# saidwivedi/InteractVLM

Hardware: AMD Instinct MI355X
Metric: images/sec end-to-end contact inference (higher is better)
Workload: dtype f16

## Files before the change

### include/ivlm_hip.h

```cpp
#ifndef IVLM_HIP_H
#define IVLM_HIP_H

#include <stddef.h>
#include <stdint.h>

#ifdef __cplusplus
extern "C" {
#endif

#define IVLM_OK 0
#define IVLM_ERR_INVALID_ARG (-1)
#define IVLM_ERR_WORKSPACE (-2)
#define IVLM_ERR_LAUNCH (-3)
#define IVLM_ERR_UNSUPPORTED (-4)

#define IVLM_F32 0
#define IVLM_BF16 1
#define IVLM_BF16_SPLIT 2
#define IVLM_F16 4
#define IVLM_F16_SPLIT 5
#define IVLM_FP8 3

#define IVLM_GEMM_A_F32 1
#define IVLM_GEMM_RES_F32 2
#define IVLM_GEMM_A_SPLIT 4
#define IVLM_GEMM_OUT_SPLIT 8
#define IVLM_GEMM_F16 16
#define IVLM_GEMM_OUT_F16 32

#define IVLM_GEMM_W_PANEL 64

typedef void *ivlm_stream_t;

int ivlm_abi_version(void);
const char *ivlm_error_string(int code);
const char *ivlm_build_arch(void);
const char *ivlm_last_hip_error(void);

int ivlm_profile_launches(void *start_event, void *stop_event);


size_t ivlm_lift_plan_workspace_bytes(int V, int64_t HW, int Nv);
int ivlm_lift_plan_build(const int32_t *vid, const float *bary, int V, int64_t HW, int Nv,
                         int32_t *row_ptr, int32_t *ent_pix, float *ent_w, int64_t cap, int32_t *nnz_out,
                         void *workspace, size_t workspace_bytes, ivlm_stream_t stream);
int ivlm_lift_points_plan_build(const int32_t *pid, int V, int64_t HW, int Np, int32_t *row_ptr, int32_t *ent_pix, float *ent_w,
                                int64_t cap, int32_t *nnz_out, void *workspace, size_t workspace_bytes, ivlm_stream_t stream);
int ivlm_lift_stream_blocks_per_cu(int bpc);

int ivlm_lift_mesh_plan(const float *logits, const int32_t *row_ptr, const int32_t *ent_pix,
                        const float *ent_w, int B, int V, int64_t HW, int Nv, int mode, float param,
                        float *out, float *nviews, ivlm_stream_t stream);

int ivlm_lift_mesh_plan_lowres(const void *low, int dtype, int lh, int lw, int img, int in_h, int in_w, int oh, int ow,
                               const int32_t *row_ptr, const int32_t *ent_pix, const float *ent_w, int B, int V,
                               int Nv, int mode, float param, float *out, float *nviews, ivlm_stream_t stream);

size_t ivlm_lift_mesh_dense_workspace_bytes(int B, int V, int Nv);
int ivlm_lift_mesh_dense(const float *logits, const int32_t *vid, const float *bary, int B, int V,
                         int64_t HW, int Nv, int mode, float param, float *out, float *nviews,
                         void *workspace, size_t workspace_bytes, ivlm_stream_t stream);

size_t ivlm_lift_points_workspace_bytes(int B, int V, int Np);
int ivlm_lift_points(const float *probs, const int32_t *pid, int pid_batched, int B, int V, int64_t HW,
                     int Np, float *out, float *nviews, void *workspace, size_t workspace_bytes,
                     ivlm_stream_t stream);

int ivlm_postprocess_masks(const void *low, int dtype, int n, int h, int w, int img, int in_h, int in_w,
                           int oh, int ow, int apply_sigmoid, float *out, ivlm_stream_t stream);
int ivlm_uncertainty_mlp(const float *embeddings, int64_t rows, const void *w1, const void *b1, const void *w2, const void *b2,
                         const void *w3, const void *b3, float *out, ivlm_stream_t stream);
int ivlm_resize_bilinear(const float *src, int n, int h, int w, void *dst, int dst_dtype, int oh, int ow, ivlm_stream_t stream);

int ivlm_postprocess_masks_valid(const void *low, int dtype, int n, int h, int w, int img, int in_h, int in_w, int oh, int ow,
                                 const float *gt, float ignore_label, float *out, ivlm_stream_t stream);


int ivlm_gemm_bf16(const void *A, int64_t lda, const void *W, int64_t ldw, void *C, int64_t ldc,
                   const void *bias, const void *residual, int64_t ldr, int res_mod, int M, int N, int K,
                   int act, int out_f32, int batch, int64_t strideA, int64_t strideW, int64_t strideC,
                   int64_t strideR, const void *rms_w, float rms_eps, int flags, const int32_t *out_rows,
                   const int32_t *a_rows, ivlm_stream_t stream);

int ivlm_gemm_bf16_panel(const void *A, int64_t lda, int64_t a_kstep, const void *W, int64_t ldw, int64_t w_kstep, void *C,
                         int64_t ldc, int64_t c_panel, const void *bias, const void *residual, int64_t ldr, int M, int N, int K,
                         int act, int out_f32, int flags, const int32_t *out_rows, const int32_t *a_rows, ivlm_stream_t stream);

int ivlm_gemm_fp8(const void *A, int64_t lda, const void *W, int64_t ldw, void *C, int64_t ldc, const void *bias,
                  const void *residual, int64_t ldr, int M, int N, int K, int act, int out_kind, const float *scale_a,
                  const float *scale_w, const float *scale_out, int flags, const int32_t *out_rows, const int32_t *a_rows,
                  ivlm_stream_t stream);

int ivlm_gemv_fp8w(const float *x, const void *Wq, int64_t ldw, const float *scale_w, void *C, const void *bias,
                   const void *residual, int N, int K, int act, int out_f32, const void *rms_w, float rms_eps, int flags,
                   ivlm_stream_t stream);

size_t ivlm_gemm_splitk_workspace_bytes(int M, int N, int splits);
int ivlm_gemm_bf16_splitk(const void *A, int64_t lda, const void *W, int64_t ldw, void *C, int64_t ldc,
                          const void *bias, const void *residual, int64_t ldr, int res_mod, int M, int N, int K,
                          int act, int out_f32, int splits, void *workspace, size_t workspace_bytes, int flags,
                          ivlm_stream_t stream);
#define IVLM_SPLITK_COUNTERS 4096
int ivlm_gemm_bf16_splitk_fused(const void *A, int64_t lda, const void *W, int64_t ldw, void *C, int64_t ldc,
                                const void *bias, const void *residual, int64_t ldr, int res_mod, int M, int N, int K,
                                int act, int out_f32, int splits, void *workspace, size_t workspace_bytes, int32_t *counters,
                                int flags, ivlm_stream_t stream);
int ivlm_gemv_tuning(int max_blocks_per_cu, int rows2_min_n);
void ivlm_gemv1_tuning(int ksplit);
void ivlm_gemv1_lds_floor(int bytes);
int ivlm_gemv_mfma_min_m(int min_m);
void ivlm_skinny_tuning(int tiles_per_block);

int ivlm_gemm_nsplit(int on);
int ivlm_gemm_tile_override(int tile);
int ivlm_gemm_tile320(int on);
int ivlm_gemm_route_query(int entry, int M, int N, int K, int64_t lda, int64_t ldw, int64_t ldc, int64_t ldr, int64_t a_kstep,
                          int64_t w_kstep, int64_t c_panel, int act, int out_kind, int has_bias, int has_residual, int res_mod,
                          int batch, int flags, int has_out_rows, int has_a_rows, int splits, int32_t *records, int max_records);

int ivlm_layernorm(const void *x, int x_dtype, const void *w, const void *b, void *y, int y_dtype, int64_t rows, int cols,
                   float eps, int gelu_after, const int32_t *out_rows, const float *fp8_scale, ivlm_stream_t stream);
int ivlm_rmsnorm(const void *x, int x_dtype, const void *w, void *y, int y_dtype, int64_t rows, int cols, float eps,
                 ivlm_stream_t stream);

int ivlm_rmsnorm_fp8(const void *x, int x_dtype, const void *w, void *y, int64_t rows, int cols, float eps, const float *fp8_scale,
                     ivlm_stream_t stream);

int ivlm_attention_bf16(const void *q, const void *k, const void *v, void *o, const int64_t *strides_host, int B,
                        int H, int Sq, int Sk, int D, float scale, int causal, int q_pos0, const float *rel_h,
                        const float *rel_w, int rel_kh, int rel_kw, int kv_batch_div, int prescale_q,
                        ivlm_stream_t stream);
int ivlm_attention_f16(const void *q, const void *k, const void *v, void *o, const int64_t *strides_host, int B,
                       int H, int Sq, int Sk, int D, float scale, int causal, int q_pos0, const float *rel_h,
                       const float *rel_w, int rel_kh, int rel_kw, int kv_batch_div, int prescale_q,
                       ivlm_stream_t stream);
int ivlm_attention_f16_qsplit(const void *q, const void *q_lo, const void *k, const void *v, void *o, const int64_t *strides_host,
                              int B, int H, int Sq, int Sk, int D, float scale, const float *rel_h, const float *rel_w, int rel_kh,
                              int rel_kw, int level, ivlm_stream_t stream);
int ivlm_attention_bf16_split(const void *q, const void *q_lo, const void *k, const void *k_lo, const void *v, const void *v_lo,
                              void *o, void *o_lo, const int64_t *strides_host, int B, int H, int Sq, int Sk, int D, float scale,
                              int causal, int q_pos0, const float *rel_h, const float *rel_w, int rel_kh, int rel_kw,
                              int kv_batch_div, int prescale_q, ivlm_stream_t stream);
int ivlm_attention_f32(const float *q, const float *k, const float *v, float *o, const int64_t *strides_host, int B, int H,
                       int Sq, int Sk, int D, float scale, int kv_batch_div, ivlm_stream_t stream);
int ivlm_attention_pingpong(int mode);
int ivlm_attention_xcd_map(int on);
int ivlm_attention_window_kernel(int v2);

int ivlm_relpos_bias(const void *q, int64_t q_bs, int64_t q_hs, int64_t q_rs, const void *tab_h, const void *tab_w,
                     int B, int H, int SH, int SW, int D, float *rel_h, float *rel_w, ivlm_stream_t stream);
int ivlm_relpos_bias_split(const void *q, const void *q_lo, int64_t q_bs, int64_t q_hs, int64_t q_rs, const void *tab_h,
                           const void *tab_w, int B, int H, int SH, int SW, int D, float *rel_h, float *rel_w,
                           ivlm_stream_t stream);
int ivlm_relpos_gather(const void *G, int64_t g_head_stride, int npad, int B, int H, int SH, int SW, float *rel_h,
                       float *rel_w, ivlm_stream_t stream);
int ivlm_relpos_gather_f32(const void *G, int64_t g_head_stride, int npad, int B, int H, int SH, int SW, float *rel_h,
                           float *rel_w, ivlm_stream_t stream);

int ivlm_relpos_bias_f16(const void *q, const void *q_lo, int64_t q_bs, int64_t q_hs, int64_t q_rs, const void *cat16, int npad, int B,
                         int H, int SH, int SW, int D, float *G_ws, size_t g_bytes, float *rel_h, float *rel_w, ivlm_stream_t stream);

int ivlm_llama_decode_attn(const void *qkv, int io_dtype, void *kcache, void *vcache, int tmax, void *o, int H, int D, int pos,
                           const int32_t *pos_dev, float theta, float scale, const float *cos_tab, const float *sin_tab,
                           ivlm_stream_t stream);
int ivlm_llama_decode_attn_f16(const void *qkv, void *kcache, void *vcache, int tmax, void *o, int H, int D, int pos,
                               const int32_t *pos_dev, float theta, float scale, const float *cos_tab, const float *sin_tab,
                               ivlm_stream_t stream);
size_t ivlm_llama_decode_attn_splitkv_scratch_bytes(int H, int D);
int ivlm_llama_decode_attn_splitkv(const float *qkv, int cache_dtype, void *kcache, void *vcache, int tmax, float *o, int H, int D,
// ... 115 lines not shown
int ivlm_sam_encode_parity_f16mlp(const ivlm_sam_cfg *cfg, const ivlm_sam_head *head, const ivlm_sam_block *blocks_host,
                                  const ivlm_sam_mlp_f16 *mlp16_host, const void *images, int V, float *embeddings_out,
                                  void *workspace, size_t workspace_bytes, ivlm_stream_t stream);
typedef struct {
    const void *qkv_w16, *proj_w16, *lin1_w16, *lin2_w16, *qkv_b16, *rel_cat16;
} ivlm_sam_block_f16;
size_t ivlm_sam_encode_f16_workspace_bytes(const ivlm_sam_cfg *cfg, int V);
int ivlm_sam_encode_f16(const ivlm_sam_cfg *cfg, const ivlm_sam_head *head, const ivlm_sam_block *blocks_host,
                        const ivlm_sam_block_f16 *blocks16_host, const void *images, int V, float *embeddings_out, void *workspace,
                        size_t workspace_bytes, ivlm_stream_t stream);
int ivlm_bf16_to_f16(const void *src_bf16, void *dst_f16, int64_t n, ivlm_stream_t stream);

typedef struct {
    const void *w2, *b;
    int n, k;
} ivlm_lin;
typedef struct {
    ivlm_lin q, k, v, o;
} ivlm_dec_attn;
typedef struct {
    ivlm_dec_attn self_attn, t2i, i2t;
    const void *norm1_w, *norm1_b, *norm2_w, *norm2_b, *norm3_w, *norm3_b, *norm4_w, *norm4_b;
    ivlm_lin lin1, lin2;
} ivlm_dec_layer;
typedef struct {
    int C, heads, depth;
    const void *no_mask, *key_pe, *out_tokens;
    ivlm_dec_layer layers[4];
    ivlm_dec_attn final_attn;
    const void *norm_final_w, *norm_final_b, *up_ln_w, *up_ln_b;
    ivlm_lin up0, up1, hyper[3], iou[3];
} ivlm_sam_dec;
size_t ivlm_sam_decode_workspace_bytes(int V, int grid, int C, int n_text, int mlp_dim);
int ivlm_sam_decode(const ivlm_sam_dec *weights, int V, int grid, int n_text, const float *image_embeddings,
                    const float *text_embeds, float *low_res_out, float *iou_out, void *workspace, size_t workspace_bytes,
                    ivlm_stream_t stream);

int ivlm_gemm_splitk_choice(int M, int N, int K, int act, int has_rms);
int ivlm_stages_splitk_fused(int on);

int ivlm_gemv1_bf12(const float *x, const void *P, int64_t ldp, const void *E, int64_t lde, const int32_t *ebase,
                    const int32_t *patch_ptr, const int32_t *patch_col, const void *patch_val, void *C, const void *bias,
                    const void *residual, int N, int K, int act, int out_f32, const void *rms_w, float rms_eps, int flags,
                    ivlm_stream_t stream);
int ivlm_gemv1_bf12m(const float *x, const void *Pf, const void *Ef, const int32_t *ebase, const int32_t *patch_ptr,
                     const int32_t *patch_col, const void *patch_val, void *C, const void *bias, const void *residual, int N, int K,
                     int act, int out_f32, const void *rms_w, float rms_eps, int flags, ivlm_stream_t stream);
int ivlm_llama_decode_attn_parts(const float *qkv, int cache_dtype, void *kcache, void *vcache, int tmax, float *parts, int H, int D,
                                 int pos, const int32_t *pos_dev, float theta, float scale, const float *cos_tab, const float *sin_tab,
                                 ivlm_stream_t stream);
int ivlm_gemv1_bf12m_parts(const float *parts, int D, const void *Pf, const void *Ef, const int32_t *ebase, const int32_t *patch_ptr,
                           const int32_t *patch_col, const void *patch_val, void *C, const void *bias, const void *residual, int N, int K,
                           int act, int out_f32, int flags, ivlm_stream_t stream);
int ivlm_pack_bf12m_count(const void *w, int N_valid, int n_rows, int K, int32_t *ebase, int32_t *patch_ptr, ivlm_stream_t stream);
int ivlm_pack_bf12m_fill(const void *w, int N_valid, int n_rows, int K, const int32_t *ebase, const int32_t *patch_ptr, void *Pf, void *Ef,
                         int32_t *patch_col, void *patch_val, ivlm_stream_t stream);
int ivlm_gemv16_bf12m(const float *x, int64_t lda, int M, const void *Pf, const void *Ef, const int32_t *ebase,
                      const int32_t *patch_ptr, const int32_t *patch_col, const void *patch_val, void *C, int64_t ldc, const void *bias,
                      const void *residual, int64_t ldr, int N, int K, int act, int out_f32, const void *rms_w, float rms_eps, int flags,
                      ivlm_stream_t stream);
void ivlm_gemv16_bf12m_tuning(int tiles_per_block);
int ivlm_decode_parts_tuning(int ranges);
void ivlm_gemv1_bf12m_tuning(int wide_max_blocks);
int ivlm_gemv1_bf12m_staging(int form);
int ivlm_unpack_bf12(const void *P, int64_t ldp, const void *E, int64_t lde, const int32_t *ebase, const int32_t *patch_ptr,
                     const int32_t *patch_col, const void *patch_val, int N, int K, void *w_out, ivlm_stream_t stream);

int ivlm_argmax_f32(const float *x, int rows, int cols, int32_t *out, ivlm_stream_t stream);
int ivlm_argmax_f32_bump(const float *x, int rows, int cols, int32_t *out, int32_t *bump, ivlm_stream_t stream);

int ivlm_im2col_nchw(const void *x, void *out, int B, int C, int H, int W, int ks, int stride, int Kpad,
                     ivlm_stream_t stream);
int ivlm_im2col3x3_nhwc(const void *x, void *out, int B, int H, int W, int C, ivlm_stream_t stream);
int ivlm_im2col3x3_nhwc_strided(const void *x, int64_t ldx, void *out, int64_t ldo, int B, int H, int W, int C,
                                ivlm_stream_t stream);
int ivlm_gather_rows(void *dst, int dst_kind, int64_t ldd, const void *src, int src_dtype, int64_t lds, const int32_t *idx,
                     const void *add, int add_dtype, int64_t lda, int64_t rows, int cols, const float *fp8_scale,
                     ivlm_stream_t stream);
int ivlm_amax(const void *x, int dtype, int64_t n, float *out, ivlm_stream_t stream);
int ivlm_add_rows(void *out, int out_kind, const void *a, int a_dtype, const void *b, int b_dtype, int64_t rows, int cols,
                  int64_t b_rows, int op, ivlm_stream_t stream);
int ivlm_fill_rows(void *dst, int64_t ldd, const int32_t *idx, int64_t n_idx, const void *row, int cols,
                   ivlm_stream_t stream);
int ivlm_dense_pe(const void *gauss, void *pe, int pe_dtype, int h, int w, int F, ivlm_stream_t stream);
int ivlm_rope_kv(void *qkv, int64_t ld, int T, int H, int D, int pos0, float theta, void *kcache, void *vcache,
                 const float *cos_tab, const float *sin_tab, ivlm_stream_t stream);
int ivlm_rope_kv_f16(void *qkv, int64_t ld, int T, int H, int D, int pos0, float theta, void *kcache, void *vcache,
                     const float *cos_tab, const float *sin_tab, ivlm_stream_t stream);
int ivlm_rope_kv_split(void *qkv, int64_t ld, int T, int H, int D, int pos0, void *kcache, void *kcache_lo, void *vcache,
                       void *vcache_lo, const float *cos_tab, const float *sin_tab, ivlm_stream_t stream);
int ivlm_llama_attn_oproj(const float *qkv, void *kcache, void *vcache, int tmax, float *attn_scratch, const void *wo,
                          const float *x, float *x_out, int H, int D, float theta, float scale, const float *cos_tab,
                          const float *sin_tab, const int32_t *pos_dev, const int32_t *step_dev, int32_t *counter,
                          int32_t *status, ivlm_stream_t stream);
int ivlm_rope_table(float *cos_tab, float *sin_tab, int T, int D, float theta, ivlm_stream_t stream);
int ivlm_normalize_pad_u8(const uint8_t *src, int H, int W, int y0, int x0, int ch, int cw, const float *mean3_host,
                          const float *std3_host, void *out, int out_bf16, int OH, int OW, ivlm_stream_t stream);
int ivlm_mask_dot(const void *up, const void *hyper, int dtype, float *low, int B, int gh, int gw, int C,
                  ivlm_stream_t stream);
int ivlm_mask_dot_multi(const void *up, const void *hyper, int dtype, float *low, int B, int M, int gh, int gw, int C,
                        ivlm_stream_t stream);
int ivlm_prompt_embed(const float *coords, const int32_t *labels, const float *gauss, const float *table, float *out, int64_t R,
                      int F, int H, int W, ivlm_stream_t stream);
int ivlm_mask_downscale(const float *mask, const float *w0, const float *b0, const float *ln1_w, const float *ln1_b, const float *w3,
                        const float *b3, const float *ln2_w, const float *ln2_b, const float *w6, const float *b6, float *dense, int B,
                        int gh, int gw, int C, int mask_in_chans, float eps, ivlm_stream_t stream);

size_t ivlm_h_geo_workspace_bytes(int n);
int ivlm_h_geo_metric(const float *dist, const float *pred, const float *gt, int B, int n, float *out, void *workspace,
                      size_t workspace_bytes, ivlm_stream_t stream);
int ivlm_contact_prf(const float *gt, const float *pred, int B, int n, float thr, float *out, ivlm_stream_t stream);
int ivlm_spmv_csr(const int32_t *row_ptr, const int32_t *col, const float *val, const float *x, int B, int rows,
                  int cols, float *y, ivlm_stream_t stream);

int ivlm_contact_band_census(const float *p, int64_t ld, int B, int Nv, const float *thr, int J, float margin, int32_t *counts,
                             float *mindist, ivlm_stream_t stream);
size_t ivlm_mask_band_census_workspace_bytes(void);
int ivlm_mask_band_census(const float *logits, int V, int64_t HW, const int32_t *ent_pix, const int32_t *row_ptr, int n_rows,
                          float thr_p, float margin_p, int32_t *counts, void *workspace, size_t workspace_bytes,
                          ivlm_stream_t stream);

#define IVLM_SEG_GT_U8 0
#define IVLM_SEG_GT_I32 1
#define IVLM_SEG_GT_F32 2
size_t ivlm_seg_iou_workspace_bytes(int V);
int ivlm_seg_iou_counts(const float *pred, const void *gt, int gt_dtype, int V, int H, int W, int ignore_label, int32_t *out,
                        void *workspace, size_t workspace_bytes, ivlm_stream_t stream);
#define IVLM_AFFORD_MAX_N 4096
#define IVLM_AFFORD_MAX_T 64
int ivlm_afford_metrics(const float *gt, const float *pred, int B, int n, const float *thresholds, int T, float mae_div,
                        float *out, int32_t *valid, ivlm_stream_t stream);

#define IVLM_CONTACT_PAIR_CHAIN 512
size_t ivlm_contact_pair_workspace_bytes(int B, int N_o, int N_h);
int ivlm_contact_pair(const float *o, const float *h, const void *p, const void *q, int p_dtype, int B, int N_o, int N_h,
                      int64_t o_batch_stride, int64_t h_batch_stride, float *value_out, float *grad_o, float *grad_h,
                      void *workspace, size_t workspace_bytes, ivlm_stream_t stream);

#define IVLM_ICP_ESTIMATE_SCALE 1
#define IVLM_ICP_ALLOW_REFLECTION 2
#define IVLM_ICP_REQUERY 4
size_t ivlm_contact_icp_workspace_bytes(int B, int N_o);
int ivlm_contact_icp(const float *x, const float *y, const float *xn, const float *yn, const float *w, const float *init_R,
                     const float *init_T, const float *init_s, int B, int N_o, int N_h, int64_t x_batch_stride, int64_t y_batch_stride,
                     int64_t xn_batch_stride, int64_t yn_batch_stride, int64_t w_batch_stride, int max_iterations, float relative_rmse_thr,
                     int flags, float *R_out, float *T_out, float *s_out, float *rmse_out, int32_t *converged_out, int32_t *iterations_out,
                     int32_t *nn_idx_out, float *hist_R, float *hist_T, float *hist_s, void *workspace, size_t workspace_bytes,
                     ivlm_stream_t stream);

int ivlm_points_align(const float *X, const float *Y, const float *w, int B, int N, int64_t x_batch_stride, int64_t y_batch_stride,
                      int64_t w_batch_stride, int flags, float *R_out, float *T_out, float *s_out, void *workspace, size_t workspace_bytes,
                      ivlm_stream_t stream);

int ivlm_contact_nearest(const float *q, const float *t, int D, int B, int N_o, int N_h, int64_t q_batch_stride, int64_t t_batch_stride,
                         int32_t *idx_out, float *d2_out, ivlm_stream_t stream);

int ivlm_contact_normal_filter(const float *obj_normals, const float *human_normals, int N_o, int N_h, float c_pos, float c_neg,
                               int has_neg, uint8_t *keep_out, ivlm_stream_t stream);

#define IVLM_SILHOUETTE_CHAIN 32
#define IVLM_SILHOUETTE_POS_ULPS 12
#define IVLM_SILHOUETTE_REL_ULPS 6
#define IVLM_SILHOUETTE_EXP_ULPS 3
#define IVLM_SILHOUETTE_T_ULPS 8
size_t ivlm_soft_silhouette_workspace_bytes(int B, int N, int F, int H, int W);
int ivlm_soft_silhouette_forward(const float *verts, const int32_t *faces, int B, int N, int F, int H, int W, float fx, float fy,
// ... 140 lines not shown
```

### interactvlm_amd/csrc/elementwise.hip

```cpp
#include "kernels.h"

namespace ivlm {
namespace {

constexpr int kT = 256;

inline int grid_for(int64_t work_items, int max_blocks = 8192) {
    int64_t b = (work_items + kT - 1) / kT;
    if (b < 1) b = 1;
    return (int)(b < max_blocks ? b : max_blocks);
}

__global__ __launch_bounds__(kT) void im2col_nchw_kernel(const bf16_t* __restrict__ x, bf16_t* __restrict__ out, int B,
                                                         int C, int H, int W, int ks, int stride, int Kpad) {
    const int gh = (H - ks) / stride + 1, gw = (W - ks) / stride + 1;
    const int K = C * ks * ks;
    const int64_t total = (int64_t)B * gh * gw * (Kpad >> 3);
    for (int64_t i = (int64_t)blockIdx.x * kT + threadIdx.x; i < total; i += (int64_t)gridDim.x * kT) {
        const int c8 = (int)(i % (Kpad >> 3));
        const int64_t row = i / (Kpad >> 3);
        const int gx = (int)(row % gw), gy = (int)((row / gw) % gh), b = (int)(row / ((int64_t)gw * gh));
        bf16_t v[8];
#pragma unroll
        for (int e = 0; e < 8; ++e) {
// ... 38 lines not shown
        f[4] = __uint_as_float(u.z << 16); f[5] = __uint_as_float(u.z & 0xffff0000u);
        f[6] = __uint_as_float(u.w << 16); f[7] = __uint_as_float(u.w & 0xffff0000u);
    }
}
__device__ __forceinline__ uint2 pack_fp8x8(const float* f, float inv_scale) {
    float c[8];
#pragma unroll
    for (int j = 0; j < 8; ++j) c[j] = fminf(fmaxf(f[j] * inv_scale, -448.0f), 448.0f);
    uint32_t a = 0, b = 0;
    a = __builtin_amdgcn_cvt_pk_fp8_f32(c[0], c[1], a, false);
    a = __builtin_amdgcn_cvt_pk_fp8_f32(c[2], c[3], a, true);
    b = __builtin_amdgcn_cvt_pk_fp8_f32(c[4], c[5], b, false);
    b = __builtin_amdgcn_cvt_pk_fp8_f32(c[6], c[7], b, true);
    return make_uint2(a, b);
}

__device__ __forceinline__ void store8(void* base, int kind, int64_t elem, int cols, const float* f, float inv_scale = 1.0f) {
    if (kind == 3) {
        *reinterpret_cast<uint2*>(static_cast<uint8_t*>(base) + elem) = pack_fp8x8(f, inv_scale);
        return;
    }
    if (kind == 1) {
        float4* p = reinterpret_cast<float4*>(static_cast<float*>(base) + elem);
        p[0] = make_float4(f[0], f[1], f[2], f[3]);
        p[1] = make_float4(f[4], f[5], f[6], f[7]);
        return;
    }
    bf16_t* o = static_cast<bf16_t*>(base) + elem;
    *reinterpret_cast<uint4*>(o) = make_uint4(pack_bf16x2(f[0], f[1]), pack_bf16x2(f[2], f[3]), pack_bf16x2(f[4], f[5]),
                                              pack_bf16x2(f[6], f[7]));
    if (kind == 2) {
        float l[8];
#pragma unroll
        for (int j = 0; j < 8; ++j) l[j] = f[j] - bf16_to_f32(f32_to_bf16(f[j]));
        *reinterpret_cast<uint4*>(o + cols) = make_uint4(pack_bf16x2(l[0], l[1]), pack_bf16x2(l[2], l[3]),
                                                         pack_bf16x2(l[4], l[5]), pack_bf16x2(l[6], l[7]));
    }
}

__global__ __launch_bounds__(kT) void gather_rows_kernel(void* __restrict__ dst, int dst_kind, int64_t ldd,
                                                         const void* __restrict__ src, int src_kind, int64_t lds_,
                                                         const int32_t* __restrict__ idx, const void* __restrict__ add,
                                                         int add_kind, int64_t lda, int64_t rows, int cols,
                                                         const float* __restrict__ scale) {
    const int c8n = cols >> 3;
    const int64_t total = rows * c8n;
    const float inv_scale = scale ? 1.0f / *scale : 1.0f;
    for (int64_t i = (int64_t)blockIdx.x * kT + threadIdx.x; i < total; i += (int64_t)gridDim.x * kT) {
        const int c8 = (int)(i % c8n);
        const int64_t r = i / c8n;
        const int64_t s = idx ? (int64_t)idx[r] : r;
        float v[8] = {0.f, 0.f, 0.f, 0.f, 0.f, 0.f, 0.f, 0.f};
        if (s >= 0) load8(src, src_kind, s * lds_ + c8 * 8, v);
        if (add) {
            float a[8];
            load8(add, add_kind, r * lda + c8 * 8, a);
#pragma unroll
            for (int j = 0; j < 8; ++j) v[j] += a[j];
        }
        store8(dst, dst_kind, r * ldd + c8 * 8, cols, v, inv_scale);
    }
}

__global__ __launch_bounds__(kT) void amax_kernel(const void* __restrict__ x, int kind, int64_t n8, float* __restrict__ out) {
    float m = 0.0f;
    for (int64_t i = (int64_t)blockIdx.x * kT + threadIdx.x; i < n8; i += (int64_t)gridDim.x * kT) {
        float v[8];
        load8(x, kind, i * 8, v);
#pragma unroll
        for (int j = 0; j < 8; ++j) m = fmaxf(m, fabsf(v[j]));
    }
    m = wave_max(m);
    if ((threadIdx.x & 63) == 0) atomicMax(reinterpret_cast<unsigned int*>(out), __float_as_uint(m));
}

__global__ __launch_bounds__(kT) void fill_rows_kernel(bf16_t* __restrict__ dst, int64_t ldd, const int32_t* __restrict__ idx,
                                                       int64_t n_idx, const bf16_t* __restrict__ row, int cols) {
    const int c8n = cols >> 3;
    const int64_t total = n_idx * c8n;
    for (int64_t i = (int64_t)blockIdx.x * kT + threadIdx.x; i < total; i += (int64_t)gridDim.x * kT) {
        const int c8 = (int)(i % c8n);
        const int64_t r = idx[i / c8n];
        *reinterpret_cast<uint4*>(dst + r * ldd + c8 * 8) = *reinterpret_cast<const uint4*>(row + c8 * 8);
    }
}

__global__ __launch_bounds__(kT) void bf16_to_f16_kernel(const bf16_t* __restrict__ src, uint16_t* __restrict__ dst, int64_t n) {
    const int64_t n8 = n >> 3;
    for (int64_t i = (int64_t)blockIdx.x * kT + threadIdx.x; i < n8; i += (int64_t)gridDim.x * kT) {
        const uint4 u = *reinterpret_cast<const uint4*>(src + i * 8);
        const uint32_t w[4] = {u.x, u.y, u.z, u.w};
        uint4 o;
        uint32_t* ow = reinterpret_cast<uint32_t*>(&o);
#pragma unroll
        for (int j = 0; j < 4; ++j) ow[j] = pack_f16x2(__uint_as_float(w[j] << 16), __uint_as_float(w[j] & 0xffff0000u));
        *reinterpret_cast<uint4*>(dst + i * 8) = o;
    }
    if (blockIdx.x == 0 && threadIdx.x < (n & 7)) {
        const int64_t i = n8 * 8 + threadIdx.x;
        dst[i] = (uint16_t)(pack_f16x2(bf16_to_f32(src[i]), 0.f) & 0xffffu);
    }
}

__global__ __launch_bounds__(kT) void add_rows_kernel(void* __restrict__ out, int out_kind, const void* __restrict__ a,
                                                      int a_kind, const void* __restrict__ b, int b_kind, int64_t rows,
                                                      int cols, int64_t b_rows, int op) {
    const int c8n = cols >> 3;
    const int64_t total = rows * c8n;
    const int64_t ldo = out_kind == 2 ? 2 * (int64_t)cols : cols;
    for (int64_t i = (int64_t)blockIdx.x * kT + threadIdx.x; i < total; i += (int64_t)gridDim.x * kT) {
        const int c8 = (int)(i % c8n);
        const int64_t r = i / c8n;
        float va[8], vb[8];
        load8(a, a_kind, r * cols + c8 * 8, va);
        load8(b, b_kind, (r % b_rows) * cols + c8 * 8, vb);
#pragma unroll
        for (int j = 0; j < 8; ++j) va[j] = op ? va[j] * vb[j] : va[j] + vb[j];
        store8(out, out_kind, r * ldo + c8 * 8, cols, va);
    }
}

__global__ __launch_bounds__(kT) void dense_pe_kernel(const float* __restrict__ gauss ,
                                                      void* __restrict__ pe , int pe_f32, int h, int w, int F) {
    const int64_t total = (int64_t)h * w * 2 * F;
    for (int64_t i = (int64_t)blockIdx.x * kT + threadIdx.x; i < total; i += (int64_t)gridDim.x * kT) {
        const int c = (int)(i % (2 * F));
        const int64_t p = i / (2 * F);
        const int xx = (int)(p % w), yy = (int)(p / w);
        const int f = c < F ? c : c - F;
        const float cx = 2.0f * (((float)xx + 0.5f) / (float)w) - 1.0f;
        const float cy = 2.0f * (((float)yy + 0.5f) / (float)h) - 1.0f;
        float t = cx * gauss[f] + cy * gauss[F + f];
        t = 6.283185307179586f * t;
        const float val = c < F ? sinf(t) : cosf(t);
        if (pe_f32) static_cast<float*>(pe)[i] = val;
        else static_cast<bf16_t*>(pe)[i] = f32_to_bf16(val);
    }
}

__global__ __launch_bounds__(kT) void rope_table_kernel(float* __restrict__ ct, float* __restrict__ st, int T, int D,
                                                        float theta) {
    const int half = D >> 1;
    const int i = blockIdx.x * kT + threadIdx.x;
    if (i >= T * half) return;
    const int j = i % half, pos = i / half;
    const float ang = (float)pos * powf(theta, -(float)(2 * j) / (float)D);
    ct[i] = cosf(ang);
    st[i] = sinf(ang);
}

template <bool F16>
__global__ __launch_bounds__(kT) void rope_kv_kernel(bf16_t* __restrict__ qkv, int64_t ld, int T, int H, int D,
                                                     int pos0, float theta, bf16_t* __restrict__ kcache,
                                                     bf16_t* __restrict__ vcache, const float* __restrict__ ct,
                                                     const float* __restrict__ stab) {
    const int half = D >> 1;
    const int64_t total = (int64_t)T * H * half;
    for (int64_t i = (int64_t)blockIdx.x * kT + threadIdx.x; i < total; i += (int64_t)gridDim.x * kT) {
        const int j = (int)(i % half);
        const int h = (int)((i / half) % H);
        const int t = (int)(i / ((int64_t)half * H));
        const int pos = pos0 + t;
        float c, s;
        if (ct) {
            c = ct[pos * half + j];
            s = stab[pos * half + j];
// ... 149 lines not shown
                                                           int ch, int cw, float m0, float m1, float m2, float s0,
                                                           float s1, float s2, T* __restrict__ out, int OH, int OW) {
    const int64_t total = (int64_t)OH * OW;
    for (int64_t i = (int64_t)blockIdx.x * kT + threadIdx.x; i < total; i += (int64_t)gridDim.x * kT) {
        const int x = (int)(i % OW), y = (int)(i / OW);
        float r = 0.f, g = 0.f, b = 0.f;
        if (y < ch && x < cw) {
            const uint8_t* p = src + ((int64_t)(y0 + y) * W + (x0 + x)) * 3;
            r = ((float)p[0] - m0) / s0;
            g = ((float)p[1] - m1) / s1;
            b = ((float)p[2] - m2) / s2;
        }
        if (sizeof(T) == 2) {
            reinterpret_cast<bf16_t*>(out)[i] = f32_to_bf16(r);
            reinterpret_cast<bf16_t*>(out)[total + i] = f32_to_bf16(g);
            reinterpret_cast<bf16_t*>(out)[2 * total + i] = f32_to_bf16(b);
        } else {
            reinterpret_cast<float*>(out)[i] = r;
            reinterpret_cast<float*>(out)[total + i] = g;
            reinterpret_cast<float*>(out)[2 * total + i] = b;
        }
    }
}

}

int normalize_pad_u8(const uint8_t* src, int H, int W, int y0, int x0, int ch, int cw, const float* mean3,
                     const float* std3, void* out, int out_bf16, int OH, int OW, hipStream_t st) {
    if (!src || !out || !mean3 || !std3 || y0 < 0 || x0 < 0 || y0 + ch > H || x0 + cw > W || ch > OH || cw > OW)
        return IVLM_ERR_INVALID_ARG;
    const int grid = grid_for((int64_t)OH * OW);
    if (out_bf16)
        normalize_pad_kernel<bf16_t><<<grid, kT, 0, st>>>(src, W, y0, x0, ch, cw, mean3[0], mean3[1], mean3[2], std3[0],
                                                          std3[1], std3[2], static_cast<bf16_t*>(out), OH, OW);
    else
        normalize_pad_kernel<float><<<grid, kT, 0, st>>>(src, W, y0, x0, ch, cw, mean3[0], mean3[1], mean3[2], std3[0],
                                                         std3[1], std3[2], static_cast<float*>(out), OH, OW);
    return ivlm_launch_status();
}

int im2col_nchw(const bf16_t* x, bf16_t* out, int B, int C, int H, int W, int ks, int stride, int Kpad,
                hipStream_t st) {
    if (!x || !out || (Kpad & 7) || Kpad < C * ks * ks) return IVLM_ERR_INVALID_ARG;
    const int gh = (H - ks) / stride + 1, gw = (W - ks) / stride + 1;
    im2col_nchw_kernel<<<grid_for((int64_t)B * gh * gw * (Kpad >> 3)), kT, 0, st>>>(x, out, B, C, H, W, ks, stride, Kpad);
    return ivlm_launch_status();
}
int im2col3x3_nhwc(const bf16_t* x, bf16_t* out, int B, int H, int W, int C, hipStream_t st, int64_t ldx, int64_t ldo) {
    if (!x || !out || (C & 7)) return IVLM_ERR_INVALID_ARG;
    if (ldx == 0) ldx = C;
    if (ldo == 0) ldo = 9 * (int64_t)C;
    if (ldx < C || ldo < 9 * (int64_t)C || ((ldx | ldo) & 7)) return IVLM_ERR_INVALID_ARG;
    im2col3x3_nhwc_kernel<<<grid_for((int64_t)B * H * W * 9 * (C >> 3)), kT, 0, st>>>(x, out, B, H, W, C, ldx, ldo);
    return ivlm_launch_status();
}
int gather_rows(void* dst, int dst_kind, int64_t ldd, const void* src, int src_kind, int64_t lds_, const int32_t* idx,
                const void* add, int add_kind, int64_t lda, int64_t rows, int cols, hipStream_t st, const float* scale) {
    if (!dst || !src || rows <= 0 || (cols & 7) || (ldd & 7) || (lds_ & 7) || (lda & 7)) return IVLM_ERR_INVALID_ARG;
    if (dst_kind < 0 || dst_kind > 3 || (src_kind & ~1) || (add_kind & ~1)) return IVLM_ERR_INVALID_ARG;
    if (dst_kind == 2 && ldd < 2 * (int64_t)cols) return IVLM_ERR_INVALID_ARG;
    if (dst_kind == 3 && !scale) return IVLM_ERR_INVALID_ARG;
    gather_rows_kernel<<<grid_for(rows * (cols >> 3)), kT, 0, st>>>(dst, dst_kind, ldd, src, src_kind, lds_, idx, add,
                                                                    add_kind, lda, rows, cols, scale);
    return ivlm_launch_status();
}
int amax(const void* x, int kind, int64_t n, float* out, hipStream_t st) {
    if (!x || !out || n <= 0 || (n & 7) || (kind & ~1)) return IVLM_ERR_INVALID_ARG;
    amax_kernel<<<grid_for(n >> 3, 2048), kT, 0, st>>>(x, kind, n >> 3, out);
    return ivlm_launch_status();
}
int add_rows(void* out, int out_kind, const void* a, int a_kind, const void* b, int b_kind, int64_t rows, int cols,
             int64_t b_rows, hipStream_t st, int op) {
    if (!out || !a || !b || rows <= 0 || b_rows <= 0 || (cols & 7)) return IVLM_ERR_INVALID_ARG;
    if (out_kind < 0 || out_kind > 2 || (a_kind & ~1) || (b_kind & ~1)) return IVLM_ERR_INVALID_ARG;
    add_rows_kernel<<<grid_for(rows * (cols >> 3)), kT, 0, st>>>(out, out_kind, a, a_kind, b, b_kind, rows, cols, b_rows, op);
    return ivlm_launch_status();
}
int fill_rows(bf16_t* dst, int64_t ldd, const int32_t* idx, int64_t n_idx, const bf16_t* row, int cols, hipStream_t st) {
    if (n_idx == 0) return IVLM_OK;
    if (!dst || !idx || !row || n_idx < 0 || (cols & 7) || (ldd & 7)) return IVLM_ERR_INVALID_ARG;
    fill_rows_kernel<<<grid_for(n_idx * (cols >> 3)), kT, 0, st>>>(dst, ldd, idx, n_idx, row, cols);
    return ivlm_launch_status();
}
int dense_pe(const float* gauss, void* pe, int pe_f32, int h, int w, int F, hipStream_t st) {
    if (!gauss || !pe) return IVLM_ERR_INVALID_ARG;
    dense_pe_kernel<<<grid_for((int64_t)h * w * 2 * F), kT, 0, st>>>(gauss, pe, pe_f32, h, w, F);
    return ivlm_launch_status();
}
int rope_kv(bf16_t* qkv, int64_t ld, int T, int H, int D, int pos0, float theta, bf16_t* kcache, bf16_t* vcache,
            hipStream_t st, const float* cos_tab, const float* sin_tab, int f16) {
    if (!qkv || T <= 0 || (D & 1) || (kcache && !vcache) || (cos_tab && !sin_tab)) return IVLM_ERR_INVALID_ARG;
    if (f16)
        rope_kv_kernel<true><<<grid_for((int64_t)T * H * (D >> 1)), kT, 0, st>>>(qkv, ld, T, H, D, pos0, theta, kcache, vcache,
                                                                                 cos_tab, sin_tab);
    else
        rope_kv_kernel<false><<<grid_for((int64_t)T * H * (D >> 1)), kT, 0, st>>>(qkv, ld, T, H, D, pos0, theta, kcache, vcache,
                                                                                  cos_tab, sin_tab);
    return ivlm_launch_status();
}
int rope_kv_split(bf16_t* qkv, int64_t ld, int T, int H, int D, int pos0, bf16_t* kcache, bf16_t* kcache_lo, bf16_t* vcache,
                  bf16_t* vcache_lo, const float* cos_tab, const float* sin_tab, hipStream_t st) {
    if (!qkv || T <= 0 || (D & 1) || !cos_tab || !sin_tab || ld < 6LL * H * D) return IVLM_ERR_INVALID_ARG;
    if (kcache && (!kcache_lo || !vcache || !vcache_lo)) return IVLM_ERR_INVALID_ARG;
    rope_kv_split_kernel<<<grid_for((int64_t)T * H * (D >> 1)), kT, 0, st>>>(qkv, ld, T, H, D, pos0, kcache, kcache_lo, vcache,
                                                                             vcache_lo, cos_tab, sin_tab);
    return ivlm_launch_status();
}
int rope_table(float* cos_tab, float* sin_tab, int T, int D, float theta, hipStream_t st) {
    if (!cos_tab || !sin_tab || T <= 0 || (D & 1)) return IVLM_ERR_INVALID_ARG;
    rope_table_kernel<<<(T * (D >> 1) + kT - 1) / kT, kT, 0, st>>>(cos_tab, sin_tab, T, D, theta);
    return ivlm_launch_status();
}
int mask_dot(const void* up, const void* hyper, int kind, float* low, int B, int gh, int gw, int C, hipStream_t st) {
    if (!up || !hyper || !low || (C & 7) || (kind & ~1)) return IVLM_ERR_INVALID_ARG;
    mask_dot_kernel<<<grid_for((int64_t)B * gh * gw * 16), kT, 0, st>>>(up, hyper, kind, low, B, gh, gw, C);
    return ivlm_launch_status();
}
int mask_dot_multi(const void* up, const void* hyper, int kind, float* low, int B, int M, int gh, int gw, int C, hipStream_t st) {
    if (!up || !hyper || !low || B <= 0 || gh <= 0 || gw <= 0 || C <= 0 || (C & 7) || (kind & ~1)) return IVLM_ERR_INVALID_ARG;
    if (M < 1 || M > 4) return IVLM_ERR_UNSUPPORTED;
    const int blocks = grid_for((int64_t)B * gh * gw * 16);
    switch (M) {
        case 1: mask_dot_multi_kernel<1><<<blocks, kT, 0, st>>>(up, hyper, kind, low, B, gh, gw, C); break;
        case 2: mask_dot_multi_kernel<2><<<blocks, kT, 0, st>>>(up, hyper, kind, low, B, gh, gw, C); break;
        case 3: mask_dot_multi_kernel<3><<<blocks, kT, 0, st>>>(up, hyper, kind, low, B, gh, gw, C); break;
        default: mask_dot_multi_kernel<4><<<blocks, kT, 0, st>>>(up, hyper, kind, low, B, gh, gw, C); break;
    }
    return ivlm_launch_status();
}

}

extern "C" {
#define BF(p) static_cast<bf16_t*>(p)
#define CBF(p) static_cast<const bf16_t*>(p)
int ivlm_im2col_nchw(const void* x, void* out, int B, int C, int H, int W, int ks, int stride, int Kpad,
                     ivlm_stream_t s) {
    ivlm_enter();
    return ivlm::im2col_nchw(CBF(x), BF(out), B, C, H, W, ks, stride, Kpad, ivlm_stream(s));
}
int ivlm_im2col3x3_nhwc(const void* x, void* out, int B, int H, int W, int C, ivlm_stream_t s) {
    ivlm_enter();
    return ivlm::im2col3x3_nhwc(CBF(x), BF(out), B, H, W, C, ivlm_stream(s));
}
int ivlm_im2col3x3_nhwc_strided(const void* x, int64_t ldx, void* out, int64_t ldo, int B, int H, int W, int C, ivlm_stream_t s) {
    ivlm_enter();
    return ivlm::im2col3x3_nhwc(CBF(x), BF(out), B, H, W, C, ivlm_stream(s), ldx, ldo);
}
int ivlm_gather_rows(void* dst, int dst_kind, int64_t ldd, const void* src, int src_dtype, int64_t lds_, const int32_t* idx,
                     const void* add, int add_dtype, int64_t lda, int64_t rows, int cols, const float* fp8_scale,
                     ivlm_stream_t s) {
    ivlm_enter();
    const int k = dst_kind == IVLM_F32 ? 1 : (dst_kind == IVLM_BF16 ? 0 : (dst_kind == IVLM_BF16_SPLIT ? 2 : (dst_kind == IVLM_FP8 ? 3 : -1)));
    return ivlm::gather_rows(dst, k, ldd, src, src_dtype == IVLM_F32, lds_, idx, add, add_dtype == IVLM_F32, lda, rows, cols,
                             ivlm_stream(s), fp8_scale);
}
int ivlm_amax(const void* x, int dtype, int64_t n, float* out, ivlm_stream_t s) {
    ivlm_enter();
    return ivlm::amax(x, dtype == IVLM_F32, n, out, ivlm_stream(s));
}
int ivlm_add_rows(void* out, int out_kind, const void* a, int a_dtype, const void* b, int b_dtype, int64_t rows, int cols,
                  int64_t b_rows, int op, ivlm_stream_t s) {
    ivlm_enter();
    return ivlm::add_rows(out, out_kind == IVLM_F32 ? 1 : (out_kind == IVLM_BF16 ? 0 : (out_kind == IVLM_BF16_SPLIT ? 2 : -1)),
                          a, a_dtype == IVLM_F32, b, b_dtype == IVLM_F32, rows, cols, b_rows, ivlm_stream(s), op);
}
int ivlm_fill_rows(void* dst, int64_t ldd, const int32_t* idx, int64_t n_idx, const void* row, int cols, ivlm_stream_t s) {
    ivlm_enter();
    return ivlm::fill_rows(BF(dst), ldd, idx, n_idx, CBF(row), cols, ivlm_stream(s));
}
int ivlm_dense_pe(const void* gauss, void* pe, int pe_dtype, int h, int w, int F, ivlm_stream_t s) {
    ivlm_enter();
    return ivlm::dense_pe(static_cast<const float*>(gauss), pe, pe_dtype == IVLM_F32, h, w, F, ivlm_stream(s));
}
int ivlm_rope_kv(void* qkv, int64_t ld, int T, int H, int D, int pos0, float theta, void* kcache, void* vcache,
                 const float* cos_tab, const float* sin_tab, ivlm_stream_t s) {
    ivlm_enter();
    return ivlm::rope_kv(BF(qkv), ld, T, H, D, pos0, theta, BF(kcache), BF(vcache), ivlm_stream(s), cos_tab, sin_tab);
}
int ivlm_rope_kv_f16(void* qkv, int64_t ld, int T, int H, int D, int pos0, float theta, void* kcache, void* vcache,
                     const float* cos_tab, const float* sin_tab, ivlm_stream_t s) {
    ivlm_enter();
    return ivlm::rope_kv(BF(qkv), ld, T, H, D, pos0, theta, BF(kcache), BF(vcache), ivlm_stream(s), cos_tab, sin_tab, 1);
}
int ivlm_rope_kv_split(void* qkv, int64_t ld, int T, int H, int D, int pos0, void* kcache, void* kcache_lo, void* vcache,
                       void* vcache_lo, const float* cos_tab, const float* sin_tab, ivlm_stream_t s) {
    ivlm_enter();
    return ivlm::rope_kv_split(BF(qkv), ld, T, H, D, pos0, BF(kcache), BF(kcache_lo), BF(vcache), BF(vcache_lo), cos_tab, sin_tab,
                               ivlm_stream(s));
}
int ivlm_bf16_to_f16(const void* src, void* dst, int64_t n, ivlm_stream_t s) {
    ivlm_enter();
    if (n == 0) return IVLM_OK;
    if (!src || !dst || n < 0 || ((uintptr_t)src & 15) || ((uintptr_t)dst & 15)) return IVLM_ERR_INVALID_ARG;
    ivlm::bf16_to_f16_kernel<<<ivlm::grid_for((n >> 3) + 1), ivlm::kT, 0, ivlm_stream(s)>>>(CBF(src), static_cast<uint16_t*>(dst), n);
    return ivlm_launch_status();
}
int ivlm_rope_table(float* cos_tab, float* sin_tab, int T, int D, float theta, ivlm_stream_t s) {
    ivlm_enter();
    return ivlm::rope_table(cos_tab, sin_tab, T, D, theta, ivlm_stream(s));
}
int ivlm_mask_dot(const void* up, const void* hyper, int dtype, float* low, int B, int gh, int gw, int C, ivlm_stream_t s) {
    ivlm_enter();
    return ivlm::mask_dot(up, hyper, dtype == IVLM_F32, low, B, gh, gw, C, ivlm_stream(s));
}
int ivlm_mask_dot_multi(const void* up, const void* hyper, int dtype, float* low, int B, int M, int gh, int gw, int C,
                        ivlm_stream_t s) {
    ivlm_enter();
    return ivlm::mask_dot_multi(up, hyper, dtype == IVLM_F32, low, B, M, gh, gw, C, ivlm_stream(s));
}
int ivlm_normalize_pad_u8(const uint8_t* src, int H, int W, int y0, int x0, int ch, int cw, const float* mean3_host,
                          const float* std3_host, void* out, int out_bf16, int OH, int OW, ivlm_stream_t s) {
    ivlm_enter();
    return ivlm::normalize_pad_u8(src, H, W, y0, x0, ch, cw, mean3_host, std3_host, out, out_bf16, OH, OW,
                                  ivlm_stream(s));
}
#undef BF
#undef CBF
}
```

### interactvlm_amd/csrc/gemm.hip

```cpp
#include <algorithm>

#include "gemm_common.h"
#include "gemm_route.h"

namespace ivlm {
namespace {

constexpr int BK = 64;

template <int WM_, int WN_, int MI_, int NI_, int MINB_ = 2>
struct TileCfg {
    static constexpr int WM = WM_, WN = WN_, MI = MI_, NI = NI_;
    static constexpr int kMinBlocks = MINB_;
    static constexpr int BM = WM * MI * 16, BN = WN * NI * 16;
    static constexpr int kWaves = WM * WN, kThreads = kWaves * 64;
    static constexpr int kTileBytesA = BM * BK * 2, kTileBytesW = BN * BK * 2;
    static constexpr int kStageBytes = kTileBytesA + kTileBytesW;
    static constexpr int kLdsBytes = 2 * kStageBytes;
    static constexpr int PA = (BM / 8 + kWaves - 1) / kWaves, PW = (BN / 8 + kWaves - 1) / kWaves;
    static_assert(BM % 8 == 0 && BN % 8 == 0, "whole 8-row pieces");
};

template <int ACT, bool OUT_F32, typename CFG, int OPK = 0>
__global__ __launch_bounds__(CFG::kThreads, CFG::kMinBlocks) void gemm_bf16_kernel(GemmArgs g) {
// ... 200 lines not shown
bool tile320_runs(const GemmArgs& g) {
    if (g.fp8 || g.out_fp8 || g.a_kstep || g.w_kstep || g.c_panel || (g.act != ACT_NONE && g.act != ACT_GELU)) return false;
    return g.out_f32 ? gemm_whole_lines_ok<true>(g, g.act) : gemm_whole_lines_ok<false>(g, g.act);
}
bool tile320_fits(const GemmArgs& g) {
    if (!tile320_runs(g) || g.batch != 1 || g.rms_w || g.N % 320 || g.M < 2048) return false;
    const long tm = (g.M + 255) / 256, tiles = tm * (g.N / 320);
    if ((!g.out_f32 || g.out_split) && !(g.f16 && tiles % 256 == 0 && tiles <= 512)) return false;
    const double q = (double)tiles / (double)(((tiles + 255) / 256) * 256);
    return tiles >= 256 && q >= 0.85 && (double)(tm * 256) / (double)g.M < 1.1;
}

int auto_tile(const GemmArgs& g, const GemmSwitches& sw) {
    if (sw.tile320 && tile320_fits(g)) return 320;
    if (g.M > 128 && g.M <= 352 && g.N >= 8192 && g.batch <= 2 && (g.act == ACT_NONE || g.act == ACT_SWIGLU)) return 176;
    const long t128 = (long)((g.M + 127) / 128) * ((g.N + 127) / 128) * g.batch;
    if (t128 < 400) return 64;
    const long t256 = (long)((g.M + 255) / 256) * ((g.N + 255) / 256) * g.batch;
    const double q = (double)t256 / (double)(((t256 + 255) / 256) * 256);
    const double edge = (double)(((g.M + 255) / 256) * 256) * (((g.N + 255) / 256) * 256) / ((double)g.M * g.N);
    if (t256 >= 512 && q >= 0.85 && edge < 1.1) return 512;
    const int keff = g.a_split ? 2 * g.K : g.K;
    if (t256 >= 256 && keff >= 2048 && edge < 1.1) return 512;
    return 128;
}

struct RouteLog {
    int32_t* rec;
    int cap, n;
};
thread_local RouteLog* t_route_log = nullptr;
bool route_logged(int family, int bm, int bn, int opk, int out_f32, int act, int grid_x, int grid_z, int lds) {
    RouteLog* log = t_route_log;
    if (!log) return false;
    if (log->n < log->cap) {
        const int32_t v[9] = {family, bm, bn, opk, out_f32, act, grid_x, grid_z, lds};
        std::copy(v, v + 9, log->rec + 9 * log->n);
    }
    ++log->n;
    return true;
}

}

GemmSwitches g_gemm_switches;

GemmRoute gemm_route(const GemmArgs& g, const GemmSwitches& sw) {
    GemmRoute r;
    r.opk = g.fp8 ? 1 : (g.f16 ? 2 : 0);
    r.out_f32 = g.out_f32 ? 1 : 0;
    r.act = g.act;
    if (!g.fp8 && (g.act < ACT_NONE || g.act > ACT_SIGMOID)) r.rc = IVLM_ERR_INVALID_ARG;
    else if (r.opk != 0 && !gemm_tower_act(g.act)) r.rc = IVLM_ERR_UNSUPPORTED;
    if (r.rc != IVLM_OK) return r;

    int t = tile_code_ok(g.tile) ? g.tile : (sw.tile_override ? sw.tile_override : auto_tile(g, sw));
    if (g.sk.count && (t == 512 || t == 256 || t == 320)) t = 128;
    r.bm = 128, r.bn = 128;
    switch (t) {
        case 320:
            if (tile320_runs(g)) r.family = GEMM_320, r.bm = 256, r.bn = 320;
            break;
        case 512: r.family = GEMM_256P; break;
        case 256: r.family = r.opk == 0 ? GEMM_TILE : GEMM_256P, r.bm = r.bn = 256; break;
        case 64: r.bn = 64; break;
        case 96:
            if (r.opk != 1) r.bn = r.opk == 0 ? 96 : 64;
            break;
        case 176:
            if (gemm_instantiated(GEMM_TILE, 176, 128, r.opk, g.act)) r.bm = 176;
            else if (r.opk != 1) r.bn = 64;
            break;
        default: break;
    }
    if (r.family == GEMM_256P) r.bm = r.bn = 256;
    r.grid_x = ((g.M + r.bm - 1) / r.bm) * ((g.N + r.bn - 1) / r.bn);
    r.grid_z = g.batch;
    r.lds = r.family == GEMM_256P ? kGemm256LdsBytes : (r.family == GEMM_320 ? kGemm320LdsBytes : 256 * (r.bm + r.bn));
    return r;
}

static int nsplit_cols(const GemmArgs& g, const GemmSwitches& sw) {
    if (!sw.nsplit || g.tile != 0 || sw.tile_override != 0 || g.batch != 1 || g.act == ACT_SWIGLU || g.M < 4096 || (g.N & 255)) return 0;
    if (auto_tile(g, sw) == 320) return 0;
    const long tm = (g.M + 255) / 256, tn = g.N / 256;
    const long tiles = tm * tn;
    const double q = (double)tiles / (double)(((tiles + 255) / 256) * 256);
    if (q >= 0.8 || tn < 2 || (g.a_split ? 2 * g.K : g.K) < 2048) return 0;
    for (long c = tn - 1; c >= tn / 2; --c)
        if ((tm * c) % 256 == 0 || (double)(tm * c) / (double)(((tm * c + 255) / 256) * 256) >= 0.97) return (int)(c * 256);
    return 0;
}

int gemm_bf16(const GemmArgs& g, hipStream_t st) {
    if (!g.A || !g.W || !g.C || g.M <= 0 || g.N <= 0 || g.K <= 0 || g.batch <= 0) return IVLM_ERR_INVALID_ARG;
    if (const int n1 = nsplit_cols(g, g_gemm_switches)) {
        GemmArgs a = g, b = g;
        a.N = n1;
        a.tile = 512;
        int rc = gemm_bf16(a, st);
        if (rc != IVLM_OK) return rc;
        b.N = g.N - n1;
        b.tile = 64;
        b.W = g.W + (int64_t)n1 * (g.w_kstep ? 64 : g.ldw);
        b.C = g.c_panel ? static_cast<char*>(g.C) + (size_t)(n1 / 64) * g.c_panel * 2
                        : static_cast<char*>(g.C) + (size_t)n1 * (g.out_fp8 ? 1 : ((g.out_f32 && !g.out_split) ? 4 : 2));
        if (g.bias) b.bias = g.bias + n1;
        if (g.residual) b.residual = g.residual + (g.res_f32 ? 2 * n1 : n1);
        return gemm_bf16(b, st);
    }
    if (g.K % 8 != 0) return IVLM_ERR_UNSUPPORTED;
    if ((g.lda & 7) || (g.ldw & 7)) return IVLM_ERR_UNSUPPORTED;
    if (g.act == ACT_SWIGLU && ((g.N & 3) || g.residual)) return IVLM_ERR_UNSUPPORTED;
    if ((reinterpret_cast<uintptr_t>(g.A) | reinterpret_cast<uintptr_t>(g.W)) & 15) return IVLM_ERR_INVALID_ARG;
    if (g.a_f32) return IVLM_ERR_UNSUPPORTED;
    if (g.f16 || g.out_f16) {
        if (g.fp8 || g.out_fp8 || g.a_f32 || (g.out_f16 && g.out_f32 && !g.out_split) || (g.a_split && !g.f16)) return IVLM_ERR_UNSUPPORTED;
    }
    if (g.a_split || g.out_split) {
        if (g.fp8 || g.out_fp8 || g.a_kstep || g.w_kstep || g.c_panel) return IVLM_ERR_UNSUPPORTED;
        if (g.a_split && ((g.a_lo & 7) || g.a_lo < g.K)) return IVLM_ERR_INVALID_ARG;
        if (g.out_split && (!g.out_f32 || (g.c_lo & 1) || g.c_lo <= 0)) return IVLM_ERR_INVALID_ARG;
    }
    if (g.a_kstep || g.w_kstep || g.c_panel) {
        if (g.fp8 || g.out_fp8 || (g.K & 63)) return IVLM_ERR_UNSUPPORTED;
        if ((g.a_kstep || g.c_panel) && (g.batch != 1 || g.act == ACT_SWIGLU)) return IVLM_ERR_UNSUPPORTED;
        if ((g.a_kstep && (g.a_kstep < (int64_t)64 * g.M || (g.a_kstep & 7) || g.a_rows)) || (g.w_kstep && (g.w_kstep < (int64_t)64 * g.N || (g.w_kstep & 7))))
            return IVLM_ERR_INVALID_ARG;
        if (g.c_panel && (g.out_f32 || (g.N & 63) || g.c_panel < (int64_t)64 * g.M || g.out_rows)) return IVLM_ERR_UNSUPPORTED;
    }
    if (g.fp8 && (!g.scale_a || !g.scale_w || (g.out_fp8 && (!g.scale_out || g.out_f32 || (g.ldc & 3))))) return IVLM_ERR_INVALID_ARG;
    if (g.out_fp8 && !g.fp8) return IVLM_ERR_UNSUPPORTED;
    if (g.out_fp8 && (g.N & 3)) return IVLM_ERR_UNSUPPORTED;
    const GemmRoute r = gemm_route(g, g_gemm_switches);
    if (r.rc != IVLM_OK) return r.rc;
    if (route_logged(r.family, r.bm, r.bn, r.opk, r.out_f32, r.act, r.grid_x, r.grid_z, r.lds)) return IVLM_OK;
    switch (r.family) {
        case GEMM_256P: return gemm256_launch(r, g, st);
        case GEMM_320: return gemm320_launch(r, g, st);
        default: return gemm_dispatch(r, GoTile{r, g, st});
    }
}

namespace {
template <bool OUT_F32>
__global__ __launch_bounds__(256) void splitk_reduce_kernel(const float* __restrict__ part, int splits, GemmArgs g) {
    const int n4 = g.N >> 2;
    const int64_t total = (int64_t)g.M * n4;
    for (int64_t i = (int64_t)blockIdx.x * 256 + threadIdx.x; i < total; i += (int64_t)gridDim.x * 256) {
        const int m = (int)(i / n4), n = (int)(i - (int64_t)m * n4) * 4;
        splitk_finish4<OUT_F32>(g, part, splits, m, n);
    }
}
}

int gemm_bf16_splitk(const GemmArgs& g, int splits, float* workspace, size_t ws_bytes, hipStream_t st, int32_t* counters) {
    if (splits < 2 || g.batch != 1 || g.act == ACT_SWIGLU || g.rms_w || g.out_rows || g.a_rows || !workspace) return IVLM_ERR_INVALID_ARG;
    if (g.K % (splits * 8) != 0 || (g.N & 3) || (g.ldc & 3)) return IVLM_ERR_UNSUPPORTED;
    if (ws_bytes < (size_t)splits * g.M * g.N * sizeof(float)) return IVLM_ERR_WORKSPACE;
    GemmArgs p = g;
    p.K = g.K / splits;
    p.batch = splits;
    p.strideA = p.K;
    p.strideW = g.w_kstep ? (int64_t)(p.K / 64) * g.w_kstep : p.K;
    p.strideC = (int64_t)g.M * g.N;
    p.strideR = 0;
    p.C = workspace;
    p.ldc = g.N;
    p.out_f32 = 1;
    p.out_f16 = 0;
    p.out_split = 0;
    p.bias = nullptr;
    p.residual = nullptr;
    p.act = ACT_NONE;
    if (counters && !g.fp8 && (g.N & 3) == 0) {
        const long tiles = (long)((g.M + 127) / 128) * ((g.N + 63) / 64);
        if (tiles <= kSplitKCounters) {
            p.sk.count = counters;
            p.sk.C = g.C; p.sk.bias = g.bias; p.sk.residual = g.residual;
            p.sk.ldc = g.ldc; p.sk.ldr = g.ldr; p.sk.c_lo = g.c_lo;
            p.sk.res_mod = g.res_mod; p.sk.act = g.act; p.sk.out_f32 = g.out_f32; p.sk.out_f16 = g.out_f16; p.sk.out_split = g.out_split;
            p.sk.res_f32 = g.res_f32;
            const int rc = gemm_bf16(p, st);
            if (rc == IVLM_OK) route_logged(4, 0, 0, 0, g.out_f32, g.act, 0, 0, 0);
            return rc;
        }
    }
    const int rc = gemm_bf16(p, st);
    if (rc != IVLM_OK) return rc;
    const int64_t total = (int64_t)g.M * (g.N >> 2);
    const int blocks = (int)std::min<int64_t>((total + 255) / 256, 2048);
    if (route_logged(3, 0, 0, 0, g.out_f32, g.act, blocks, 1, 0)) return IVLM_OK;
    if (g.out_f32) ivlm_launch(splitk_reduce_kernel<true>, dim3(blocks), dim3(256), 0, st, (const float*)workspace, splits, g);
    else ivlm_launch(splitk_reduce_kernel<false>, dim3(blocks), dim3(256), 0, st, (const float*)workspace, splits, g);
    return ivlm_launch_status();
}

int linear_bf16(const GemmArgs& g, hipStream_t st) {
    if (g.batch == 1 && g.M <= 16 && g.K >= 1024 && g.N >= 1024 && !(g.K & 7) && !(g.lda & 7) && !(g.ldw & 7) &&
        !(g.act == ACT_SWIGLU && ((g.N & 1) || g.residual))) {
        const int min_m = g_gemm_switches.skinny_min_m;
        const bool skinny = min_m > 0 ? g.M >= min_m : (g.M >= 5 || (g.M >= 3 && (size_t)g.M * g.K * 2 > 48 * 1024));
        if (!g.out_rows && !g.a_rows && (skinny || (g.a_f32 && g.M >= 2))) return gemv_mfma_bf16(g, st);
    }
    if (g.M <= 8 && g.batch == 1 && !g.out_rows && !g.a_rows) return gemv_bf16(g, st);
    if (g.a_f32 && g.M <= 16 && g.batch == 1 && !g.out_rows && !g.a_rows) {
        for (int m0 = 0; m0 < g.M; m0 += 8) {
            GemmArgs c = g;
            c.M = g.M - m0 < 8 ? g.M - m0 : 8;
            c.A = reinterpret_cast<const bf16_t*>(reinterpret_cast<const float*>(g.A) + (int64_t)m0 * g.lda);
            c.C = static_cast<char*>(g.C) + (size_t)m0 * g.ldc * (g.out_f32 ? 4 : 2);
            if (g.residual && g.res_mod <= 0) c.residual = g.residual + (int64_t)m0 * g.ldr * (g.res_f32 ? 2 : 1);
            if (g.residual && g.res_mod > 0) return IVLM_ERR_UNSUPPORTED;
            const int rc = gemv_bf16(c, st);
            if (rc != IVLM_OK) return rc;
        }
        return IVLM_OK;
    }
    if (g.a_f32) return IVLM_ERR_UNSUPPORTED;
    if (g.rms_w) return IVLM_ERR_UNSUPPORTED;
    return gemm_bf16(g, st);
}

int gemm_splitk_choice(int M, int N, int K, int act, int has_rms) {
    if (M <= 8 || M > 1024 || act == ACT_SWIGLU || has_rms || (N & 3) || (K & 63)) return 1;
    if (M <= 16 && N >= 1024 && K >= 1024) return 1;
    if (M > 128 && M <= 352 && N >= 8192) {
        const long t176 = (long)((M + 175) / 176) * ((N + 127) / 128);
        return (t176 < 256 && (K / 64) % 2 == 0 && K / 2 >= 512) ? 2 : 1;
    }
    const long tiles = (long)((M + 127) / 128) * ((N + 63) / 64);
    if (tiles >= 256) return 1;
    int best = 1;
    const int k64 = K / 64;
    for (int sp = 2; sp <= std::min<long>(8, 1024 / tiles); ++sp)
        if (k64 % sp == 0 && K / sp >= 512) best = sp;
    return best;
}

GemmArgs gemm_args(const void* A, int64_t lda, const void* W, int64_t ldw, void* C, int64_t ldc, const void* bias, const void* residual,
                   int64_t ldr, int res_mod, int M, int N, int K, int act, int out_f32, int flags, const int32_t* out_rows,
                   const int32_t* a_rows) {
    GemmArgs g;
    g.A = static_cast<const bf16_t*>(A);
    g.W = static_cast<const bf16_t*>(W);
    g.C = C;
    g.bias = static_cast<const bf16_t*>(bias);
    g.residual = static_cast<const bf16_t*>(residual);
    g.lda = lda; g.ldw = ldw; g.ldc = ldc; g.ldr = ldr;
    g.res_mod = res_mod;
    g.M = M; g.N = N; g.K = K;
    g.act = act;
    g.out_rows = out_rows;
    g.a_rows = a_rows;
    g.a_f32 = (flags & IVLM_GEMM_A_F32) ? 1 : 0;
    g.res_f32 = (flags & IVLM_GEMM_RES_F32) ? 1 : 0;
    g.f16 = (flags & IVLM_GEMM_F16) ? 1 : 0;
    g.out_f16 = (flags & IVLM_GEMM_OUT_F16) ? 1 : 0;
    if (flags & IVLM_GEMM_A_SPLIT) { g.a_split = 1; g.a_lo = K; }
    if (flags & IVLM_GEMM_OUT_SPLIT) { g.out_split = 1; g.c_lo = act == ACT_SWIGLU ? N / 2 : N; out_f32 = 1; }
    g.out_f32 = out_f32;
    if (flags & IVLM_GEMM_W_PANEL) { g.w_kstep = (int64_t)64 * N; g.ldw = 64; }
    return g;
}

}

using ivlm::g_gemm_switches;

extern "C" int ivlm_gemv_mfma_min_m(int min_m) {
    g_gemm_switches.skinny_min_m = min_m;
    return 0;
}

extern "C" int ivlm_gemm_nsplit(int on) {
    g_gemm_switches.nsplit = on;
    return 0;
}

extern "C" int ivlm_gemm_tile320(int on) {
    const int prev = g_gemm_switches.tile320;
    g_gemm_switches.tile320 = on ? 1 : 0;
    return prev;
}

extern "C" int ivlm_gemm_tile_override(int tile) {
    const int prev = g_gemm_switches.tile_override;
    if (tile == 0 || ivlm::tile_code_ok(tile)) g_gemm_switches.tile_override = tile;
    return prev;
}

extern "C" int ivlm_gemm_splitk_choice(int M, int N, int K, int act, int has_rms) {
    return ivlm::gemm_splitk_choice(M, N, K, act, has_rms);
}

extern "C" int ivlm_gemm_bf16(const void* A, int64_t lda, const void* W, int64_t ldw, void* C, int64_t ldc,
                              const void* bias, const void* residual, int64_t ldr, int res_mod, int M, int N, int K,
                              int act, int out_f32, int batch, int64_t strideA, int64_t strideW, int64_t strideC,
                              int64_t strideR, const void* rms_w, float rms_eps, int flags, const int32_t* out_rows,
                              const int32_t* a_rows, ivlm_stream_t stream) {
    ivlm_enter();
    ivlm::GemmArgs g = ivlm::gemm_args(A, lda, W, ldw, C, ldc, bias, residual, ldr, res_mod, M, N, K, act, out_f32, flags, out_rows, a_rows);
    if (g.w_kstep && ((K & 63) || batch > 1)) return IVLM_ERR_UNSUPPORTED;
    if ((g.a_split || g.out_split || g.f16 || g.out_f16 || g.w_kstep) && M <= 16) return IVLM_ERR_UNSUPPORTED;
    g.rms_w = static_cast<const bf16_t*>(rms_w);
    g.rms_eps = rms_eps;
    g.batch = batch < 1 ? 1 : batch;
    g.strideA = strideA; g.strideW = strideW; g.strideC = strideC; g.strideR = strideR;
    return ivlm::linear_bf16(g, ivlm_stream(stream));
}

extern "C" int ivlm_gemm_bf16_panel(const void* A, int64_t lda, int64_t a_kstep, const void* W, int64_t ldw, int64_t w_kstep, void* C,
                                    int64_t ldc, int64_t c_panel, const void* bias, const void* residual, int64_t ldr, int M, int N,
                                    int K, int act, int out_f32, int flags, const int32_t* out_rows, const int32_t* a_rows,
                                    ivlm_stream_t stream) {
    ivlm_enter();
    if (M <= 16 || (flags & IVLM_GEMM_A_F32)) return IVLM_ERR_UNSUPPORTED;
    ivlm::GemmArgs g = ivlm::gemm_args(A, a_kstep ? 64 : lda, W, w_kstep ? 64 : ldw, C, ldc, bias, residual, ldr, 0, M, N, K, act, out_f32,
                                       flags & IVLM_GEMM_RES_F32, out_rows, a_rows);
    g.a_kstep = a_kstep; g.w_kstep = w_kstep; g.c_panel = c_panel;
    return ivlm::gemm_bf16(g, ivlm_stream(stream));
}

extern "C" int ivlm_gemm_fp8(const void* A, int64_t lda, const void* W, int64_t ldw, void* C, int64_t ldc, const void* bias,
                             const void* residual, int64_t ldr, int M, int N, int K, int act, int out_kind, const float* scale_a,
                             const float* scale_w, const float* scale_out, int flags, const int32_t* out_rows,
                             const int32_t* a_rows, ivlm_stream_t stream) {
    ivlm_enter();
    if ((K & 15) || (lda & 15) || (ldw & 15) || M <= 16) return IVLM_ERR_UNSUPPORTED;
    ivlm::GemmArgs g = ivlm::gemm_args(A, lda / 2, W, ldw / 2, C, ldc, bias, residual, ldr, 0, M, N, K / 2, act, out_kind == IVLM_F32,
                                       flags & IVLM_GEMM_RES_F32, out_rows, a_rows);
    g.fp8 = 1;
    g.out_fp8 = out_kind == 2 ? 1 : 0;
    g.scale_a = scale_a; g.scale_w = scale_w; g.scale_out = scale_out;
    return ivlm::gemm_bf16(g, ivlm_stream(stream));
}

extern "C" size_t ivlm_gemm_splitk_workspace_bytes(int M, int N, int splits) {
    return (size_t)(splits < 1 ? 1 : splits) * (size_t)M * (size_t)N * sizeof(float);
}

static int splitk_entry(const void* A, int64_t lda, const void* W, int64_t ldw, void* C, int64_t ldc,
                                     const void* bias, const void* residual, int64_t ldr, int res_mod, int M, int N,
                                     int K, int act, int out_f32, int splits, void* workspace, size_t workspace_bytes,
                                     int flags, ivlm_stream_t stream, int32_t* counters) {
    ivlm_enter();
    if (flags & IVLM_GEMM_A_F32) return IVLM_ERR_UNSUPPORTED;
    if ((flags & IVLM_GEMM_OUT_F16) && out_f32 && !(flags & IVLM_GEMM_OUT_SPLIT)) return IVLM_ERR_INVALID_ARG;
    if ((flags & IVLM_GEMM_W_PANEL) && K % (splits * 64) != 0) return IVLM_ERR_UNSUPPORTED;
    const ivlm::GemmArgs g = ivlm::gemm_args(A, lda, W, ldw, C, ldc, bias, residual, ldr, res_mod, M, N, K, act, out_f32, flags, nullptr, nullptr);
    return ivlm::gemm_bf16_splitk(g, splits, static_cast<float*>(workspace), workspace_bytes, ivlm_stream(stream), counters);
}

extern "C" int ivlm_gemm_bf16_splitk(const void* A, int64_t lda, const void* W, int64_t ldw, void* C, int64_t ldc,
                                     const void* bias, const void* residual, int64_t ldr, int res_mod, int M, int N,
                                     int K, int act, int out_f32, int splits, void* workspace, size_t workspace_bytes,
                                     int flags, ivlm_stream_t stream) {
    return splitk_entry(A, lda, W, ldw, C, ldc, bias, residual, ldr, res_mod, M, N, K, act, out_f32, splits, workspace, workspace_bytes,
                        flags, stream, nullptr);
}

extern "C" int ivlm_gemm_bf16_splitk_fused(const void* A, int64_t lda, const void* W, int64_t ldw, void* C, int64_t ldc,
                                           const void* bias, const void* residual, int64_t ldr, int res_mod, int M, int N,
                                           int K, int act, int out_f32, int splits, void* workspace, size_t workspace_bytes,
                                           int32_t* counters, int flags, ivlm_stream_t stream) {
    if (!counters) return IVLM_ERR_INVALID_ARG;
    return splitk_entry(A, lda, W, ldw, C, ldc, bias, residual, ldr, res_mod, M, N, K, act, out_f32, splits, workspace, workspace_bytes,
                        flags, stream, counters);
}

extern "C" int ivlm_gemm_route_query(int entry, int M, int N, int K, int64_t lda, int64_t ldw, int64_t ldc, int64_t ldr, int64_t a_kstep,
                                     int64_t w_kstep, int64_t c_panel, int act, int out_kind, int has_bias, int has_residual,
                                     int res_mod, int batch, int flags, int has_out_rows, int has_a_rows, int splits,
                                     int32_t* records, int max_records) {
    if (!records || max_records < 1 || M <= 16) return IVLM_ERR_INVALID_ARG;
    const auto dummy = [](int present, uintptr_t at) { return present ? reinterpret_cast<void*>(at << 16) : nullptr; };
    const void *A = dummy(1, 1), *W = dummy(1, 2), *bias = dummy(has_bias, 4), *res = dummy(has_residual, 5);
    void *C = dummy(1, 3), *ws = dummy(1, 8);
    const int32_t *orow = static_cast<int32_t*>(dummy(has_out_rows, 6)), *arow = static_cast<int32_t*>(dummy(has_a_rows, 7));
    const float* sc = static_cast<float*>(dummy(1, 9));
    ivlm::RouteLog log{records, max_records, 0};
    ivlm::t_route_log = &log;
    int rc = IVLM_ERR_INVALID_ARG;
    switch (entry) {
        case 0: rc = ivlm_gemm_bf16(A, lda, W, ldw, C, ldc, bias, res, ldr, res_mod, M, N, K, act, out_kind, batch, 0, 0, 0, 0, nullptr, 0.f, flags, orow, arow, nullptr); break;
        case 1: rc = ivlm_gemm_bf16_panel(A, lda, a_kstep, W, ldw, w_kstep, C, ldc, c_panel, bias, res, ldr, M, N, K, act, out_kind, flags, orow, arow, nullptr); break;
        case 2: rc = ivlm_gemm_fp8(A, lda, W, ldw, C, ldc, bias, res, ldr, M, N, K, act, out_kind, sc, sc, sc, flags, orow, arow, nullptr); break;
        case 3: rc = ivlm_gemm_bf16_splitk(A, lda, W, ldw, C, ldc, bias, res, ldr, res_mod, M, N, K, act, out_kind, splits, ws, SIZE_MAX, flags, nullptr); break;
        case 4: rc = ivlm_gemm_bf16_splitk_fused(A, lda, W, ldw, C, ldc, bias, res, ldr, res_mod, M, N, K, act, out_kind, splits, ws, SIZE_MAX, static_cast<int32_t*>(dummy(1, 10)), flags, nullptr); break;
        default: break;
    }
    if (rc != IVLM_OK) ivlm::route_logged(-1, rc, 0, 0, 0, 0, 0, 0, 0);
    ivlm::t_route_log = nullptr;
    return log.n <= max_records ? log.n : IVLM_ERR_WORKSPACE;
}
```

### interactvlm_amd/csrc/gemm_common.h

```cpp
#pragma once
#include "kernels.h"

namespace ivlm {

typedef __attribute__((ext_vector_type(8))) __bf16 bf16x8_t;
typedef __attribute__((ext_vector_type(4))) float f32x4_t;
typedef __attribute__((ext_vector_type(8))) int i32x8_t;
typedef __attribute__((ext_vector_type(8))) _Float16 f16x8_t;

__device__ __forceinline__ f32x4_t mfma_fp8_128(const bf16x8_t& a0, const bf16x8_t& a1, const bf16x8_t& b0, const bf16x8_t& b1,
                                                const f32x4_t& c) {
    struct P { bf16x8_t lo, hi; };
    const P pa{a0, a1}, pb{b0, b1};
    return __builtin_amdgcn_mfma_scale_f32_16x16x128_f8f6f4(__builtin_bit_cast(i32x8_t, pa), __builtin_bit_cast(i32x8_t, pb), c,
                                                            0, 0, 0, 0x7f7f7f7f, 0, 0x7f7f7f7f);
}

__device__ __forceinline__ float gelu_erf_fast(float x) {
    const float z = fabsf(x) * 0.70710678118654752f;
    const float t = __builtin_amdgcn_rcpf(fmaf(0.3275911f, z, 1.0f));
    float p = fmaf(1.061405429f, t, -1.453152027f);
    p = fmaf(p, t, 1.421413741f);
    p = fmaf(p, t, -0.284496736f);
    p = fmaf(p, t, 0.254829592f);
    const float a = 0.5f * p * t, e = __expf(-z * z);
    const float q = a * e;
    return x * (x < 0.0f ? q : fmaf(-a, e, 1.0f));
}

typedef float __attribute__((ext_vector_type(2))) f32x2_t;
__device__ __forceinline__ f32x2_t gelu_erf_fast2(f32x2_t x) {
    const f32x2_t ax = {fabsf(x.x), fabsf(x.y)};
    const f32x2_t z = ax * 0.70710678118654752f;
    const f32x2_t d = __builtin_elementwise_fma(f32x2_t{0.3275911f, 0.3275911f}, z, f32x2_t{1.0f, 1.0f});
    const f32x2_t t = {__builtin_amdgcn_rcpf(d.x), __builtin_amdgcn_rcpf(d.y)};
    f32x2_t p = __builtin_elementwise_fma(f32x2_t{1.061405429f, 1.061405429f}, t, f32x2_t{-1.453152027f, -1.453152027f});
    p = __builtin_elementwise_fma(p, t, f32x2_t{1.421413741f, 1.421413741f});
    p = __builtin_elementwise_fma(p, t, f32x2_t{-0.284496736f, -0.284496736f});
    p = __builtin_elementwise_fma(p, t, f32x2_t{0.254829592f, 0.254829592f});
    const f32x2_t a = (p * 0.5f) * t;
    const f32x2_t nzz = -z * z;
    const f32x2_t e = {__expf(nzz.x), __expf(nzz.y)};
    const f32x2_t q = a * e;
    const f32x2_t omq = __builtin_elementwise_fma(-a, e, f32x2_t{1.0f, 1.0f});
    return f32x2_t{x.x * (x.x < 0.0f ? q.x : omq.x), x.y * (x.y < 0.0f ? q.y : omq.y)};
}

__device__ __forceinline__ float gemm_act(float x, int act) {
    switch (act) {
        case ACT_GELU: return gelu_erf_fast(x);
        case ACT_QUICK_GELU: return x / (1.0f + __expf(-1.702f * x));
        case ACT_RELU: return x < 0.0f ? 0.0f : x;
        case ACT_SILU: return x / (1.0f + __expf(-x));
        case ACT_SIGMOID: return 1.0f / (1.0f + __expf(-x));
        default: return x;
    }
}

__device__ __attribute__((aligned(16))) const uint32_t kGemmZeroChunk[4] = {0u, 0u, 0u, 0u};

__device__ __forceinline__ void glds16(const void* gsrc, void* lds_dst) {
#ifndef IVLM_ABL_NODMA
    __builtin_amdgcn_global_load_lds(gsrc, (__attribute__((address_space(3))) void*)lds_dst, 16, 0, 0);
#endif
}
__device__ __forceinline__ bf16x8_t gemm_frag_read(const unsigned char* p) {
#ifdef IVLM_ABL_NOLDS
    uint32_t v = (uint32_t)(uintptr_t)p * 0x9e3779b1u | 0x3c003c00u;
    asm volatile("" : "+v"(v));
    typedef __attribute__((ext_vector_type(4))) uint32_t u4_t;
    return __builtin_bit_cast(bf16x8_t, u4_t{v, v, v, v});
#else
    return *reinterpret_cast<const bf16x8_t*>(p);
#endif
}
#ifdef IVLM_ABL_NOMFMA
#define IVLM_ABL_MFMA_USE(a, b)                                                          \
    do {                                                                                 \
        auto a_ = (a);                                                                   \
        auto b_ = (b);                                                                   \
        asm volatile("" ::"v"(a_), "v"(b_));                                             \
    } while (0)
#endif

__device__ __forceinline__ void gemm_tile_origin(const GemmArgs& g, int BM, int BN, int& m0, int& n0) {
    const int tiles_n = (g.N + BN - 1) / BN;
    const int tiles_m = (g.M + BM - 1) / BM;
    const int nwg = tiles_m * tiles_n;
    constexpr int kXcd = 8, kGroupM = 8;
    const int bid = blockIdx.x;
    const int xcd = bid % kXcd, loc = bid / kXcd;
    const int q = nwg / kXcd, r = nwg % kXcd;
    const int lin = (xcd < r ? xcd * (q + 1) : r * (q + 1) + (xcd - r) * q) + loc;
    const int per_group = kGroupM * tiles_n;
    const int first_m = (lin / per_group) * kGroupM;
    const int gsz = tiles_m - first_m < kGroupM ? tiles_m - first_m : kGroupM;
    const int in_group = lin % per_group;
    m0 = (first_m + in_group % gsz) * BM;
    n0 = (in_group / gsz) * BN;
}

__device__ __forceinline__ float gemm_residual_at(const GemmArgs& g, const bf16_t* R, int64_t idx) {
    return g.res_f32 ? reinterpret_cast<const float*>(R)[idx] : bf16_to_f32(R[idx]);
}

template <bool OUT_F32>
__device__ __forceinline__ void splitk_finish4(const GemmArgs& g, const float* __restrict__ part, int splits, int m, int n) {
    const int64_t slice = (int64_t)g.M * g.N;
    const float* p = part + (int64_t)m * g.N + n;
    float4 acc = *reinterpret_cast<const float4*>(p);
    for (int sidx = 1; sidx < splits; ++sidx) {
        const float4 t = *reinterpret_cast<const float4*>(p + sidx * slice);
        acc.x += t.x; acc.y += t.y; acc.z += t.z; acc.w += t.w;
    }
    float v[4] = {acc.x, acc.y, acc.z, acc.w};
#pragma unroll
    for (int j = 0; j < 4; ++j) {
        if (g.bias) v[j] += bf16_to_f32(g.bias[n + j]);
        v[j] = gemm_act(v[j], g.act);
        if (g.residual) {
            const int64_t rrow = g.res_mod > 0 ? (m % g.res_mod) : m;
            v[j] += gemm_residual_at(g, g.residual, rrow * g.ldr + n + j);
        }
    }
    const int64_t o = (int64_t)m * g.ldc + n;
    if (OUT_F32 && g.out_split) {
        uint32_t h0, l0, h1, l1;
        split_16x2(v[0], v[1], h0, l0, g.out_f16);
        split_16x2(v[2], v[3], h1, l1, g.out_f16);
        *reinterpret_cast<uint2*>(static_cast<bf16_t*>(g.C) + o) = make_uint2(h0, h1);
        *reinterpret_cast<uint2*>(static_cast<bf16_t*>(g.C) + o + g.c_lo) = make_uint2(l0, l1);
    } else if (OUT_F32) *reinterpret_cast<float4*>(static_cast<float*>(g.C) + o) = make_float4(v[0], v[1], v[2], v[3]);
    else *reinterpret_cast<uint2*>(static_cast<bf16_t*>(g.C) + o) = make_uint2(pack_16x2(v[0], v[1], g.out_f16), pack_16x2(v[2], v[3], g.out_f16));
}

template <int BM, int BN, int THREADS>
__device__ __forceinline__ void splitk_fixup(const GemmArgs& g, int m0, int n0) {
    __shared__ int s_last;
    __threadfence();
    __syncthreads();
    if (threadIdx.x == 0) {
        const int old = atomicAdd(g.sk.count + blockIdx.x, 1);
        const int last = old == g.batch - 1;
        if (last) g.sk.count[blockIdx.x] = 0;
        s_last = last;
    }
    __syncthreads();
    if (!s_last) return;
    __threadfence();
    GemmArgs f = g;
    f.C = g.sk.C; f.bias = g.sk.bias; f.residual = g.sk.residual;
    f.ldc = g.sk.ldc; f.ldr = g.sk.ldr; f.c_lo = g.sk.c_lo;
    f.res_mod = g.sk.res_mod; f.act = g.sk.act; f.out_f32 = g.sk.out_f32; f.out_f16 = g.sk.out_f16; f.out_split = g.sk.out_split;
    f.res_f32 = g.sk.res_f32;
    const float* part = static_cast<const float*>(g.C);
    constexpr int kQ = BN / 4;
    for (int i = threadIdx.x; i < BM * kQ; i += THREADS) {
        const int m = m0 + i / kQ, n = n0 + (i % kQ) * 4;
        if (m >= g.M || n >= g.N) continue;
        if (f.out_f32) splitk_finish4<true>(f, part, g.batch, m, n);
        else splitk_finish4<false>(f, part, g.batch, m, n);
    }
}

template <int ACT>
__device__ __forceinline__ void gemm_value4(const GemmArgs& g, int n, const f32x4_t& acc, float (&v)[4]) {
    v[0] = acc[0]; v[1] = acc[1]; v[2] = acc[2]; v[3] = acc[3];
    if (g.fp8) {
        const float alpha = (*g.scale_a) * (*g.scale_w);
#pragma unroll
        for (int j = 0; j < 4; ++j) v[j] *= alpha;
    }
    if (g.bias) {
        const uint2 b2 = *reinterpret_cast<const uint2*>(g.bias + n);
        v[0] += bf16_to_f32((bf16_t)(b2.x & 0xffff));
        v[1] += bf16_to_f32((bf16_t)(b2.x >> 16));
        v[2] += bf16_to_f32((bf16_t)(b2.y & 0xffff));
        v[3] += bf16_to_f32((bf16_t)(b2.y >> 16));
    }
#pragma unroll
    for (int j = 0; j < 4; ++j) v[j] = gemm_act(v[j], ACT);
}

template <bool OUT_F32>
__host__ __device__ __forceinline__ bool gemm_whole_lines_ok(const GemmArgs& g, int act) {
    return act != ACT_SWIGLU && !g.out_fp8 && g.batch == 1 && (reinterpret_cast<uintptr_t>(g.C) & 15) == 0 &&
           (OUT_F32 ? ((g.N & 3) == 0 && (g.ldc & 3) == 0 && (!g.residual || (g.ldr & 3) == 0) && (!g.out_split || (g.c_lo & 3) == 0))
                    : ((g.N & 7) == 0 && !g.residual && (g.c_panel ? (g.c_panel & 7) == 0 : (g.ldc & 7) == 0)));
}

template <int ACT, bool OUT_F32, int MI, int NI, int PASS_MI, int NI_ALL = NI, int NI0 = 0>
__device__ __forceinline__ void gemm_store_lines(const GemmArgs& g, unsigned char* wbuf, int mw, int nw, int lane,
                                                 const f32x4_t (&acc)[NI_ALL][MI]) {
    constexpr int ES = OUT_F32 ? 4 : 2;
    constexpr int RB = NI * 16 * ES;
    constexpr int CH = RB / 16;
    static_assert(CH == 8 || CH == 16, "rows of 128 or 256 bytes");
    static_assert(MI % PASS_MI == 0, "whole passes");
    constexpr int RPI = 64 / CH;
    constexpr int ROWS = PASS_MI * 16;
    const int cc = lane % CH, n = nw + cc * (16 / ES);
#pragma unroll
    for (int p = 0; p < MI / PASS_MI; ++p) {
#pragma unroll
        for (int mi = 0; mi < PASS_MI; ++mi) {
            const int r = mi * 16 + (lane & 15);
            const int sw = CH == 8 ? ((r >> 1) & 7) : (r & 15);
#pragma unroll
            for (int ni = 0; ni < NI; ++ni) {
                const int nl = ni * 16 + (lane >> 4) * 4;
                float v[4] = {0.f, 0.f, 0.f, 0.f};
                if (nw + nl < g.N) gemm_value4<ACT>(g, nw + nl, acc[NI0 + ni][p * PASS_MI + mi], v);
                unsigned char* dst = wbuf + r * RB + ((((nl * ES) >> 4) ^ sw) << 4) + ((nl * ES) & 15);
                if (OUT_F32) *reinterpret_cast<float4*>(dst) = make_float4(v[0], v[1], v[2], v[3]);
                else *reinterpret_cast<uint2*>(dst) = make_uint2(pack_16x2(v[0], v[1], g.out_f16), pack_16x2(v[2], v[3], g.out_f16));
            }
        }
        asm volatile("s_waitcnt lgkmcnt(0)" ::: "memory");
        __builtin_amdgcn_wave_barrier();
#pragma unroll
        for (int it = 0; it < ROWS / RPI; ++it) {
            const int rr = it * RPI + lane / CH;
            const int sw = CH == 8 ? ((rr >> 1) & 7) : (rr & 15);
            const unsigned char* src = wbuf + rr * RB + ((cc ^ sw) << 4);
            int m = mw + p * ROWS + rr;
            if (m >= g.M || n >= g.N) continue;
            if (g.out_rows) {
                m = g.out_rows[m];
                if (m < 0) continue;
            }
            if (OUT_F32) {
                float4 q = *reinterpret_cast<const float4*>(src);
                if (g.residual) {
                    const int64_t rrow = g.res_mod > 0 ? (m % g.res_mod) : m;
                    if (g.res_f32) {
                        const float4 r4 = *reinterpret_cast<const float4*>(reinterpret_cast<const float*>(g.residual) + rrow * g.ldr + n);
                        q.x += r4.x; q.y += r4.y; q.z += r4.z; q.w += r4.w;
                    } else {
                        const uint2 r2 = *reinterpret_cast<const uint2*>(g.residual + rrow * g.ldr + n);
                        q.x += bf16_to_f32((bf16_t)(r2.x & 0xffff));
                        q.y += bf16_to_f32((bf16_t)(r2.x >> 16));
                        q.z += bf16_to_f32((bf16_t)(r2.y & 0xffff));
                        q.w += bf16_to_f32((bf16_t)(r2.y >> 16));
                    }
                }
                if (g.out_split) {
                    uint32_t h0, l0, h1, l1;
                    split_16x2(q.x, q.y, h0, l0, g.out_f16);
                    split_16x2(q.z, q.w, h1, l1, g.out_f16);
                    bf16_t* cb = static_cast<bf16_t*>(g.C) + (int64_t)m * g.ldc + n;
                    *reinterpret_cast<uint2*>(cb) = make_uint2(h0, h1);
                    *reinterpret_cast<uint2*>(cb + g.c_lo) = make_uint2(l0, l1);
                } else {
                    *reinterpret_cast<float4*>(static_cast<float*>(g.C) + (int64_t)m * g.ldc + n) = q;
                }
            } else {
                const int64_t o = g.c_panel ? (int64_t)(n >> 6) * g.c_panel + (int64_t)m * 64 + (n & 63) : (int64_t)m * g.ldc + n;
                *reinterpret_cast<uint4*>(static_cast<bf16_t*>(g.C) + o) = *reinterpret_cast<const uint4*>(src);
            }
        }
        asm volatile("s_waitcnt lgkmcnt(0)" ::: "memory");
        __builtin_amdgcn_wave_barrier();
    }
}

template <int ACT, bool OUT_F32, int MI, int NI_ALL>
__device__ __forceinline__ void gemm_stage_strip(const GemmArgs& g, unsigned char* tile, int cl, int n_global, int lane,
                                                 const f32x4_t (&acc)[NI_ALL][MI], int ni_src) {
    constexpr int ES = OUT_F32 ? 4 : 2;
    constexpr int RB = 64 * ES, CH = RB / 16;
    const int nl = cl + (lane >> 4) * 4;
#pragma unroll
    for (int mi = 0; mi < MI; ++mi) {
        const int r = mi * 16 + (lane & 15);
        const int sw = CH == 8 ? ((r >> 1) & 7) : (r & 15);
        float v[4] = {0.f, 0.f, 0.f, 0.f};
        if (n_global + (lane >> 4) * 4 < g.N) gemm_value4<ACT>(g, n_global + (lane >> 4) * 4, acc[ni_src][mi], v);
        unsigned char* dst = tile + r * RB + ((((nl * ES) >> 4) ^ sw) << 4) + ((nl * ES) & 15);
        if (OUT_F32) *reinterpret_cast<float4*>(dst) = make_float4(v[0], v[1], v[2], v[3]);
        else *reinterpret_cast<uint2*>(dst) = make_uint2(pack_16x2(v[0], v[1], g.out_f16), pack_16x2(v[2], v[3], g.out_f16));
    }
}

template <bool OUT_F32>
__device__ __forceinline__ void gemm_store_strip_rows(const GemmArgs& g, const unsigned char* tile, int row0, int nrows, int m_base, int n_base,
                                                      int lane) {
    constexpr int ES = OUT_F32 ? 4 : 2;
    constexpr int RB = 64 * ES, CH = RB / 16, RPI = 64 / CH;
    const int cc = lane % CH, n = n_base + cc * (16 / ES);
    for (int it = 0; it < nrows / RPI; ++it) {
        const int rr = row0 + it * RPI + lane / CH;
        const int sw = CH == 8 ? ((rr >> 1) & 7) : (rr & 15);
        const unsigned char* src = tile + rr * RB + ((cc ^ sw) << 4);
        int m = m_base + rr;
        if (m >= g.M || n >= g.N) continue;
        if (g.out_rows) {
            m = g.out_rows[m];
            if (m < 0) continue;
        }
        if (OUT_F32) {
            float4 q = *reinterpret_cast<const float4*>(src);
            if (g.residual) {
                const int64_t rrow = g.res_mod > 0 ? (m % g.res_mod) : m;
                if (g.res_f32) {
                    const float4 r4 = *reinterpret_cast<const float4*>(reinterpret_cast<const float*>(g.residual) + rrow * g.ldr + n);
                    q.x += r4.x; q.y += r4.y; q.z += r4.z; q.w += r4.w;
                } else {
                    const uint2 r2 = *reinterpret_cast<const uint2*>(g.residual + rrow * g.ldr + n);
                    q.x += bf16_to_f32((bf16_t)(r2.x & 0xffff));
                    q.y += bf16_to_f32((bf16_t)(r2.x >> 16));
                    q.z += bf16_to_f32((bf16_t)(r2.y & 0xffff));
                    q.w += bf16_to_f32((bf16_t)(r2.y >> 16));
                }
            }
            if (g.out_split) {
                uint32_t h0, l0, h1, l1;
                split_16x2(q.x, q.y, h0, l0, g.out_f16);
                split_16x2(q.z, q.w, h1, l1, g.out_f16);
                bf16_t* cb = static_cast<bf16_t*>(g.C) + (int64_t)m * g.ldc + n;
                *reinterpret_cast<uint2*>(cb) = make_uint2(h0, h1);
                *reinterpret_cast<uint2*>(cb + g.c_lo) = make_uint2(l0, l1);
            } else {
                *reinterpret_cast<float4*>(static_cast<float*>(g.C) + (int64_t)m * g.ldc + n) = q;
            }
        } else {
            *reinterpret_cast<uint4*>(static_cast<bf16_t*>(g.C) + (int64_t)m * g.ldc + n) = *reinterpret_cast<const uint4*>(src);
        }
    }
}

template <int ACT, bool OUT_F32>
__device__ __forceinline__ void gemm_epilogue4(const GemmArgs& g, int bz, int m, int n, const f32x4_t& acc) {
    if (m >= g.M || n >= g.N) return;
    if (g.out_rows) {
        m = g.out_rows[m];
        if (m < 0) return;
    }
    const bf16_t* __restrict__ bias = g.bias;
    const bf16_t* __restrict__ R = g.residual ? g.residual + (int64_t)bz * g.strideR * (g.res_f32 ? 2 : 1) : nullptr;
    const int64_t rrow = g.res_mod > 0 ? (m % g.res_mod) : m;
    float v[4] = {acc[0], acc[1], acc[2], acc[3]};
    if (g.fp8) {
        const float alpha = (*g.scale_a) * (*g.scale_w);
#pragma unroll
        for (int j = 0; j < 4; ++j) v[j] *= alpha;
    }
    if ((g.N & 3) == 0) {
        if (bias) {
            const uint2 b2 = *reinterpret_cast<const uint2*>(bias + n);
            v[0] += bf16_to_f32((bf16_t)(b2.x & 0xffff));
            v[1] += bf16_to_f32((bf16_t)(b2.x >> 16));
            v[2] += bf16_to_f32((bf16_t)(b2.y & 0xffff));
            v[3] += bf16_to_f32((bf16_t)(b2.y >> 16));
        }
        if (ACT == ACT_SWIGLU) {
            const float o0 = (v[0] / (1.0f + __expf(-v[0]))) * v[1];
            const float o1 = (v[2] / (1.0f + __expf(-v[2]))) * v[3];
            const int64_t o = (int64_t)m * g.ldc + (n >> 1);
            if (g.out_fp8) {
                const float inv = 1.0f / (*g.scale_out);
                const uint32_t wq = __builtin_amdgcn_cvt_pk_fp8_f32(fminf(fmaxf(o0 * inv, -448.0f), 448.0f),
                                                                    fminf(fmaxf(o1 * inv, -448.0f), 448.0f), 0u, false);
                *reinterpret_cast<uint16_t*>(static_cast<uint8_t*>(g.C) + (int64_t)bz * g.strideC + o) = (uint16_t)(wq & 0xffffu);
                return;
            }
            if (OUT_F32 && g.out_split) {
                bf16_t* C = static_cast<bf16_t*>(g.C) + (int64_t)bz * g.strideC;
                uint32_t hi, lo;
                split_16x2(o0, o1, hi, lo, g.out_f16);
                *reinterpret_cast<uint32_t*>(C + o) = hi;
                *reinterpret_cast<uint32_t*>(C + o + g.c_lo) = lo;
            } else if (OUT_F32) {
                float* C = static_cast<float*>(g.C) + (int64_t)bz * g.strideC;
                *reinterpret_cast<float2*>(C + o) = make_float2(o0, o1);
            } else {
                bf16_t* C = static_cast<bf16_t*>(g.C) + (int64_t)bz * g.strideC;
                *reinterpret_cast<uint32_t*>(C + o) = pack_16x2(o0, o1, g.out_f16);
            }
            return;
        }
#pragma unroll
        for (int j = 0; j < 4; ++j) v[j] = gemm_act(v[j], ACT);
        if (R) {
            if (g.res_f32) {
                const float4 r4 = *reinterpret_cast<const float4*>(reinterpret_cast<const float*>(R) + rrow * g.ldr + n);
                v[0] += r4.x; v[1] += r4.y; v[2] += r4.z; v[3] += r4.w;
            } else {
                const uint2 r2 = *reinterpret_cast<const uint2*>(R + rrow * g.ldr + n);
                v[0] += bf16_to_f32((bf16_t)(r2.x & 0xffff));
                v[1] += bf16_to_f32((bf16_t)(r2.x >> 16));
                v[2] += bf16_to_f32((bf16_t)(r2.y & 0xffff));
                v[3] += bf16_to_f32((bf16_t)(r2.y >> 16));
            }
        }
        const int64_t o = g.c_panel ? (int64_t)(n >> 6) * g.c_panel + (int64_t)m * 64 + (n & 63) : (int64_t)m * g.ldc + n;
        if (g.out_fp8) {
            const float inv = 1.0f / (*g.scale_out);
            float c4[4];
#pragma unroll
            for (int j = 0; j < 4; ++j) c4[j] = fminf(fmaxf(v[j] * inv, -448.0f), 448.0f);
            uint32_t w = 0;
            w = __builtin_amdgcn_cvt_pk_fp8_f32(c4[0], c4[1], w, false);
            w = __builtin_amdgcn_cvt_pk_fp8_f32(c4[2], c4[3], w, true);
            *reinterpret_cast<uint32_t*>(static_cast<uint8_t*>(g.C) + (int64_t)bz * g.strideC + o) = w;
        } else if (OUT_F32 && g.out_split) {
            bf16_t* C = static_cast<bf16_t*>(g.C) + (int64_t)bz * g.strideC;
            uint32_t h0, l0, h1, l1;
            split_16x2(v[0], v[1], h0, l0, g.out_f16);
            split_16x2(v[2], v[3], h1, l1, g.out_f16);
            *reinterpret_cast<uint2*>(C + o) = make_uint2(h0, h1);
            *reinterpret_cast<uint2*>(C + o + g.c_lo) = make_uint2(l0, l1);
        } else if (OUT_F32) {
            float* C = static_cast<float*>(g.C) + (int64_t)bz * g.strideC;
            *reinterpret_cast<float4*>(C + o) = make_float4(v[0], v[1], v[2], v[3]);
        } else {
            bf16_t* C = static_cast<bf16_t*>(g.C) + (int64_t)bz * g.strideC;
            *reinterpret_cast<uint2*>(C + o) = make_uint2(pack_16x2(v[0], v[1], g.out_f16), pack_16x2(v[2], v[3], g.out_f16));
        }
    } else {
#pragma unroll
        for (int j = 0; j < 4; ++j) {
            if (n + j >= g.N) break;
            float x = v[j] + (bias ? bf16_to_f32(bias[n + j]) : 0.0f);
            x = gemm_act(x, ACT);
            if (R) x += gemm_residual_at(g, R, rrow * g.ldr + n + j);
            const int64_t o = (int64_t)m * g.ldc + n + j;
            if (OUT_F32 && g.out_split) {
                bf16_t* C = static_cast<bf16_t*>(g.C) + (int64_t)bz * g.strideC;
                uint32_t h2, l2;
                split_16x2(x, 0.0f, h2, l2, g.out_f16);
                C[o] = (bf16_t)(h2 & 0xffffu);
                C[o + g.c_lo] = (bf16_t)(l2 & 0xffffu);
            } else if (OUT_F32)
                (static_cast<float*>(g.C) + (int64_t)bz * g.strideC)[o] = x;
            else
                (static_cast<bf16_t*>(g.C) + (int64_t)bz * g.strideC)[o] = g.out_f16 ? f32_to_h16<true>(x) : f32_to_bf16(x);
        }
    }
}

}
```

### interactvlm_amd/csrc/kernels.h

```cpp
#pragma once
#include "ivlm_common.h"

namespace ivlm {

enum Act : int { ACT_NONE = 0, ACT_GELU = 1, ACT_QUICK_GELU = 2, ACT_RELU = 3, ACT_SILU = 4, ACT_SWIGLU = 5, ACT_SIGMOID = 6 };

struct SplitKFused {
    int32_t* count = nullptr;
    void* C = nullptr;
    const bf16_t* bias = nullptr;
    const bf16_t* residual = nullptr;
    int64_t ldc = 0, ldr = 0, c_lo = 0;
    int res_mod = 0, act = 0, out_f32 = 0, out_f16 = 0, out_split = 0, res_f32 = 0;
};
constexpr int kSplitKCounters = 4096;

struct GemmArgs {
    const bf16_t* A = nullptr;
    const bf16_t* W = nullptr;
    void* C = nullptr;
    const bf16_t* bias = nullptr;
    const bf16_t* residual = nullptr;
    int64_t lda = 0, ldw = 0, ldc = 0, ldr = 0;
    int res_mod = 0;
    int M = 0, N = 0, K = 0;
    int act = ACT_NONE;
    int out_f32 = 0;
    const int32_t* out_rows = nullptr;
    const int32_t* a_rows = nullptr;
    int64_t a_kstep = 0, w_kstep = 0;
    int64_t c_panel = 0;
    int fp8 = 0, out_fp8 = 0;
    const float *scale_a = nullptr, *scale_w = nullptr, *scale_out = nullptr;
    int a_f32 = 0;
    int a_split = 0;
    int64_t a_lo = 0;
    int out_split = 0;
    int64_t c_lo = 0;
    int f16 = 0, out_f16 = 0;
    int res_f32 = 0;
    int batch = 1;
    int64_t strideA = 0, strideW = 0, strideC = 0, strideR = 0;
    int tile = 0;
    const bf16_t* rms_w = nullptr;
    float rms_eps = 0.0f;
    SplitKFused sk;
};

GemmArgs gemm_args(const void* A, int64_t lda, const void* W, int64_t ldw, void* C, int64_t ldc, const void* bias, const void* residual,
                   int64_t ldr, int res_mod, int M, int N, int K, int act, int out_f32, int flags, const int32_t* out_rows = nullptr,
                   const int32_t* a_rows = nullptr);
int gemm_bf16(const GemmArgs& g, hipStream_t st);
int gemm_splitk_choice(int M, int N, int K, int act, int has_rms);
int gemm_bf16_splitk(const GemmArgs& g, int splits, float* workspace, size_t ws_bytes, hipStream_t st, int32_t* counters = nullptr);
int linear_bf16(const GemmArgs& g, hipStream_t st);

int layernorm(const void* x, int x_f32, const bf16_t* w, const bf16_t* b, void* y, int y_f32, int64_t rows, int cols, float eps,
              hipStream_t st, int gelu = 0, const int32_t* out_rows = nullptr, const float* fp8_scale = nullptr);
int rmsnorm(const void* x, int x_f32, const bf16_t* w, void* y, int y_f32, int64_t rows, int cols, float eps, hipStream_t st,
            const float* fp8_scale = nullptr);

struct AttnArgs {
    const bf16_t *q, *k, *v;
    bf16_t* o;
    int64_t q_bs, q_hs, q_rs;
    int64_t k_bs, k_hs, k_rs;
    int64_t v_bs, v_hs, v_rs;
    int64_t o_bs, o_hs, o_rs;
    int B, H, Sq, Sk, D;
    float scale;
    int causal;
    int q_pos0;
    const float* rel_h;
    const float* rel_w;
    int rel_kh, rel_kw;
    int kv_batch_div;
    int prescale_q;
    const bf16_t *q_lo = nullptr, *k_lo = nullptr, *v_lo = nullptr;
    bf16_t* o_lo = nullptr;
    int xcd_map = 1;
    int q_lo_level = 0;
    int f16 = 0;
};

int attention_bf16(const AttnArgs& a, hipStream_t st);
int attention_f32(const float* q, const float* k, const float* v, float* o, const int64_t* st12, int B, int H, int Sq, int Sk,
                  int D, float scale, int kv_div, hipStream_t st);
int relpos_bias(const bf16_t* q, int64_t q_bs, int64_t q_hs, int64_t q_rs, const bf16_t* tab_h, const bf16_t* tab_w,
                int B, int H, int SH, int SW, int D, float* rel_h, float* rel_w, hipStream_t st, const bf16_t* q_lo = nullptr);

int im2col_nchw(const bf16_t* x, bf16_t* out, int B, int C, int H, int W, int ks, int stride, int Kpad, hipStream_t st);
int im2col3x3_nhwc(const bf16_t* x, bf16_t* out, int B, int H, int W, int C, hipStream_t st, int64_t ldx = 0, int64_t ldo = 0);
int rope_kv_split(bf16_t* qkv, int64_t ld, int T, int H, int D, int pos0, bf16_t* kcache, bf16_t* kcache_lo, bf16_t* vcache,
                  bf16_t* vcache_lo, const float* cos_tab, const float* sin_tab, hipStream_t st);
int gather_rows(void* dst, int dst_kind, int64_t ldd, const void* src, int src_kind, int64_t lds_, const int32_t* idx,
                const void* add, int add_kind, int64_t lda, int64_t rows, int cols, hipStream_t st, const float* scale = nullptr);
int amax(const void* x, int kind, int64_t n, float* out, hipStream_t st);
int add_rows(void* out, int out_kind, const void* a, int a_kind, const void* b, int b_kind, int64_t rows, int cols,
             int64_t b_rows, hipStream_t st, int op = 0);
int fill_rows(bf16_t* dst, int64_t ldd, const int32_t* idx, int64_t n_idx, const bf16_t* row, int cols, hipStream_t st);
int dense_pe(const float* gauss, void* pe, int pe_f32, int h, int w, int F, hipStream_t st);
int rope_kv(bf16_t* qkv, int64_t ld, int T, int H, int D, int pos0, float theta, bf16_t* kcache, bf16_t* vcache,
            hipStream_t st, const float* cos_tab = nullptr, const float* sin_tab = nullptr, int f16 = 0);
int rope_table(float* cos_tab, float* sin_tab, int T, int D, float theta, hipStream_t st);
int normalize_pad_u8(const uint8_t* src, int H, int W, int y0, int x0, int ch, int cw, const float* mean3,
                     const float* std3, void* out, int out_bf16, int OH, int OW, hipStream_t st);
int mask_dot(const void* up, const void* hyper, int kind, float* low, int B, int gh, int gw, int C, hipStream_t st);
int mask_dot_multi(const void* up, const void* hyper, int kind, float* low, int B, int M, int gh, int gw, int C, hipStream_t st);

int contact_prf(const float* gt, const float* pred, int B, int n, float thr, float* out, hipStream_t st);
int spmv_csr(const int32_t* row_ptr, const int32_t* col, const float* val, const float* x, int B, int rows, int cols,
             float* y, hipStream_t st);

int contact_band_census(const float* p, int64_t ld, int B, int nv, const float* thr, int J, float margin, int32_t* counts,
                        float* mindist, hipStream_t st);
size_t mask_band_census_workspace_bytes();
int mask_band_census(const float* logits, int V, int64_t HW, const int32_t* ent_pix, const int32_t* row_ptr, int n_rows,
                     float thr_p, float margin_p, int32_t* counts, void* ws, size_t ws_bytes, hipStream_t st);

size_t seg_iou_workspace_bytes(int V);
int seg_iou_counts(const float* pred, const void* gt, int gt_dtype, int V, int H, int W, int ignore_label, int32_t* out, void* ws,
                   size_t ws_bytes, hipStream_t st);
int afford_metrics(const float* gt, const float* pred, int B, int n, const float* thresholds, int T, float mae_div, float* out,
                   int32_t* valid, hipStream_t st);

size_t mesh_sdf_plan_bytes(int n_verts, int n_faces);
int mesh_sdf_prepare(const float* verts, const int32_t* faces, int n_verts, int n_faces, void* plan, size_t plan_bytes, hipStream_t st);
size_t mesh_sdf_workspace_bytes(int B, int N, int n_faces);
int mesh_sdf_query(const void* plan, const float* points, int B, int N, float* sdf, float* closest, int32_t* face, float* winding,
                   void* ws, size_t ws_bytes, hipStream_t st);
int mesh_sdf_penetration(const void* plan, const float* points, int B, int N, float* value, float* grad, void* ws, size_t ws_bytes,
                         hipStream_t st);
size_t mesh_sdf_intrusion_workspace_bytes(int B, int N, int n_faces);
int mesh_sdf_intrusion(const void* plan, const float* points, const float* rot6d, const float* trans, const float* scale, int B, int N,
                       float* value, float* grad_r6, float* grad_t, float* grad_s, void* ws, size_t ws_bytes, hipStream_t st);

size_t contact_pair_workspace_bytes(int B, int n_o, int n_h);
int contact_pair(const float* o, const float* h, const void* p, const void* q, int p_dtype, int B, int n_o, int n_h,
                 int64_t o_bstride, int64_t h_bstride, float* value, float* grad_o, float* grad_h, void* ws, size_t ws_bytes,
                 hipStream_t st);

size_t soft_silhouette_workspace_bytes(int B, int N, int F, int H, int W);
int soft_silhouette_forward(const float* verts, const int32_t* faces, int B, int N, int F, int H, int W, float fx, float fy, float px,
                            float py, float sigma, float blur, float* alpha, void* ws, size_t ws_bytes, hipStream_t st);
int soft_silhouette_backward(const float* verts, const int32_t* vf_off, const int32_t* vf_list, const float* galpha, int B, int N, int F,
                             int H, int W, float fx, float fy, float px, float py, float sigma, float blur, float* gverts, void* ws,
                             size_t ws_bytes, hipStream_t st);
int silhouette_terms(const float* alpha, const float* target, int64_t t_bstride, int B, int H, int W, float* loss, float* centroid,
                     double* sums, const float* g_loss, const float* g_centroid, float* galpha, void* ws, size_t ws_bytes,
                     hipStream_t st);

size_t pose_transform_workspace_bytes(int B, int N);
int pose_transform_forward(const float* verts, const float* rot6d, const float* trans, const float* scale, int B, int N, float* out,
                           hipStream_t st);
int pose_transform_backward(const float* verts, const float* rot6d, const float* scale, const float* grad_out, int B, int N,
                            float* grad_r6, float* grad_t, float* grad_s, void* ws, size_t ws_bytes, hipStream_t st);

size_t contact_icp_workspace_bytes(int B, int n_o);
int contact_icp(const float* x, const float* y, const float* xn, const float* yn, const float* w, const float* init_R, const float* init_T,
                const float* init_s, int B, int n_o, int n_h, int64_t x_bs, int64_t y_bs, int64_t xn_bs, int64_t yn_bs, int64_t w_bs,
                int max_iterations, float relative_rmse_thr, int flags, float* R, float* T, float* s, float* rmse, int32_t* converged,
                int32_t* iterations, int32_t* nn_idx, float* hist_R, float* hist_T, float* hist_s, void* ws, size_t ws_bytes,
                hipStream_t st);
int points_align(const float* X, const float* Y, const float* w, int B, int n, int64_t x_bs, int64_t y_bs, int64_t w_bs, int flags,
                 float* R, float* T, float* s, void* ws, size_t ws_bytes, hipStream_t st);
int contact_nearest(const float* q, const float* t, int D, int B, int n_o, int n_h, int64_t q_bs, int64_t t_bs, int32_t* idx, float* d2,
                    hipStream_t st);
int contact_normal_filter(const float* on, const float* hn, int n_o, int n_h, float c_pos, float c_neg, int has_neg, uint8_t* keep,
                          hipStream_t st);

size_t raster_workspace_bytes(int n_prims_verts, int H, int W);
int rasterize_mesh(const float* verts, int nv, const int32_t* faces, int nf, const float* cam12_host, float fov_deg,
                   int H, int W, int32_t* p2v, float* bary, int32_t* pix_to_face, void* ws, size_t ws_bytes,
                   hipStream_t st);
int rasterize_points(const float* pts, int np, const float* cam12_host, float fov_deg, float radius, int H, int W,
                     int32_t* map, void* ws, size_t ws_bytes, hipStream_t st);

int phong_shade(const int32_t* p2v, const float* bary, const float* verts, const float* normals, const float* colors, int npix,
                const float* light3_host, const float* cam3_host, float ambient, float diffuse, float specular, float shininess,
                const float* bg3_host, uint8_t* out, hipStream_t st);

enum DecodeAttnForm : int {
    DA_ONE_BLOCK = 0,
// ... 55 lines not shown
```

### interactvlm_amd/csrc/stages.hip

```cpp
#include <algorithm>
#include <cstdlib>
#include <type_traits>

#include "kernels.h"

namespace ivlm {

namespace {

inline size_t al(size_t b) { return (b + 255) & ~(size_t)255; }

struct Carver {
    char* base = nullptr;
    size_t room = SIZE_MAX, used = 0;
    bool ok = true;
    void* take(size_t bytes) {
        bytes = al(bytes);
        if (bytes > room - used) {
            ok = false;
            return nullptr;
        }
        used += bytes;
        return base ? base + (used - bytes) : nullptr;
    }
// ... 211 lines not shown
    for (int l = 0; l < c->layers; ++l) {
        const Layer& L = layers_host[l];
        at.kcache = static_cast<bf16_t*>(kcache) + l * cache_layer;
        at.vcache = static_cast<bf16_t*>(vcache) + l * cache_layer;
        if ((rc = dec_linear(c, x, L.qkv, b.qkv, nullptr, 3 * Hd, Hd, ACT_NONE, L.ln1, stream))) return rc;
        float* x1 = (x == b.xa) ? b.xb : b.xa;
        if (fused) {
            if constexpr (!packed) {
                at.scratch = b.scratch + (size_t)l * Hd; at.wo = static_cast<const bf16_t*>(L.o); at.x = x; at.x_out = x1;
                at.counter = b.counters + l * 32;
                rc = decode_attn(DA_FUSED, at, st);
            }
        } else if (split_kv) {
            if constexpr (packed) {
                rc = decode_attn(DA_PARTS, at, st);
                if (!rc)
                    rc = ivlm_gemv1_bf12m_parts(b.parts, D, L.o.Pf, L.o.Ef, L.o.ebase, L.o.patch_ptr, L.o.patch_col, L.o.patch_val, x1,
                                                nullptr, x, Hd, Hd, ACT_NONE, 1, IVLM_GEMM_RES_F32, stream);
            }
        } else {
            rc = decode_attn(DA_ONE_BLOCK, at, st);
            if (!rc) rc = dec_linear(c, b.att, L.o, x1, x, Hd, Hd, ACT_NONE, nullptr, stream);
        }
        if (rc) return rc;
        if ((rc = dec_linear(c, x1, L.gu, b.hh, nullptr, 2 * I, Hd, ACT_SWIGLU, L.ln2, stream))) return rc;
        float* x2 = (x1 == b.xa) ? b.xb : b.xa;
        if ((rc = dec_linear(c, b.hh, L.down, x2, x1, Hd, I, ACT_NONE, nullptr, stream))) return rc;
        x = x2;
    }
    if ((rc = rmsnorm(x, 1, static_cast<const bf16_t*>(final_norm), hidden_out, 1, 1, Hd, c->eps, st))) return rc;
    bump_kernel<<<1, 1, 0, st>>>(fused ? b.words + 1 : nullptr, advance ? pos_dev : nullptr);
    return ivlm_launch_status();
}

}

extern "C" size_t ivlm_llama_decode_workspace_bytes(const ivlm_llama_cfg* c) {
    return cfg_ok(c) ? carved_bytes(carve_decode, c) : 0;
}

extern "C" int ivlm_llama_decode_step(const ivlm_llama_cfg* c, const ivlm_llama_layer* layers_host, const void* final_norm,
                                      void* kcache, void* vcache, const float* cos_tab, const float* sin_tab, const float* x_in,
                                      int32_t* pos_dev, int advance, float* hidden_out, void* workspace, size_t workspace_bytes,
                                      ivlm_stream_t stream) {
    return decode_step(c, layers_host, final_norm, kcache, vcache, 0, cos_tab, sin_tab, x_in, pos_dev, advance, hidden_out, workspace,
                       workspace_bytes, stream);
}

extern "C" int ivlm_llama_decode_step_f16kv(const ivlm_llama_cfg* c, const ivlm_llama_layer* layers_host, const void* final_norm,
                                            void* kcache16, void* vcache16, const float* cos_tab, const float* sin_tab,
                                            const float* x_in, int32_t* pos_dev, int advance, float* hidden_out, void* workspace,
                                            size_t workspace_bytes, ivlm_stream_t stream) {
    return decode_step(c, layers_host, final_norm, kcache16, vcache16, 1, cos_tab, sin_tab, x_in, pos_dev, advance, hidden_out,
                       workspace, workspace_bytes, stream);
}

extern "C" int ivlm_llama_decode_step_bf12(const ivlm_llama_cfg* c, const ivlm_llama_layer_bf12* layers_host, const void* final_norm,
                                           void* kcache, void* vcache, int cache_dtype, const float* cos_tab, const float* sin_tab,
                                           const float* x_in, int32_t* pos_dev, int advance, float* hidden_out, void* workspace,
                                           size_t workspace_bytes, ivlm_stream_t stream) {
    if (cache_dtype != IVLM_BF16 && cache_dtype != IVLM_F16) return IVLM_ERR_INVALID_ARG;
    return decode_step(c, layers_host, final_norm, kcache, vcache, cache_dtype == IVLM_F16, cos_tab, sin_tab, x_in, pos_dev, advance,
                       hidden_out, workspace, workspace_bytes, stream);
}

namespace ivlm {
namespace {

__global__ void sam_window_maps_kernel(int V, int g, int ws, int nw, int32_t* __restrict__ part, int32_t* __restrict__ unpart) {
    const int S = ws * ws;
    const int64_t total = (int64_t)V * nw * nw * S;
    for (int64_t i = (int64_t)blockIdx.x * blockDim.x + threadIdx.x; i < total; i += (int64_t)gridDim.x * blockDim.x) {
        const int ix = (int)(i % ws), iy = (int)((i / ws) % ws);
        const int wx = (int)((i / S) % nw), wy = (int)((i / ((int64_t)S * nw)) % nw), v = (int)(i / ((int64_t)S * nw * nw));
        const int y = wy * ws + iy, x = wx * ws + ix;
        const bool ok = y < g && x < g;
        const int src = (v * g + y) * g + x;
        part[i] = ok ? src : -1;
        if (ok) unpart[src] = (int32_t)i;
    }
}

__global__ void fill_pad_rows_kernel(bf16_t* __restrict__ dst, int64_t ldd, const int32_t* __restrict__ part, int64_t rows,
                                     const bf16_t* __restrict__ row, int cols) {
    const int c8n = cols >> 3;
    const int64_t total = rows * c8n;
    for (int64_t i = (int64_t)blockIdx.x * blockDim.x + threadIdx.x; i < total; i += (int64_t)gridDim.x * blockDim.x) {
        const int64_t r = i / c8n;
        if (part[r] >= 0) continue;
        const int c8 = (int)(i % c8n);
        *reinterpret_cast<uint4*>(dst + r * ldd + c8 * 8) = *reinterpret_cast<const uint4*>(row + c8 * 8);
    }
}

int gemm(const void* A, int64_t lda, const void* W, int64_t ldw, void* C, int out_f32, int64_t ldc, const void* bias,
         const void* res, int res_f32, int64_t ldr, int res_mod, int M, int N, int K, int act, const int32_t* out_rows,
         const int32_t* a_rows, const SkRegion& sk, hipStream_t st, int flags = 0) {
    const GemmArgs g = gemm_args(A, lda, W, ldw, C, ldc, bias, res, ldr, res_mod, M, N, K, act, out_f32,
                                 flags | (res_f32 ? IVLM_GEMM_RES_F32 : 0), out_rows, a_rows);
    const int sp = (out_rows || a_rows) ? 1 : gemm_splitk_choice(M, N, K, act, 0);
    if (sp > 1 && (ldc & 3) == 0 && sk.ws && sk.bytes >= (size_t)sp * M * N * 4)
        return sk_gemm(g, sp, sk, st);
    return linear_bf16(g, st);
}

int attend(const bf16_t* q, const bf16_t* q_lo, const bf16_t* k, const bf16_t* k_lo, const bf16_t* v, const bf16_t* v_lo, int64_t rs,
           bf16_t* o, int64_t o_rs, int f16, int B, int H, int S, int D, const void* rel_h, const float* rel_w, int side,
           hipStream_t st) {
    AttnArgs a{};
    a.f16 = f16;
    a.q = q; a.k = k; a.v = v; a.o = o;
    a.q_lo = q_lo; a.k_lo = k_lo; a.v_lo = v_lo; a.o_lo = k_lo ? o + H * D : nullptr;
    a.q_lo_level = (f16 && q_lo) ? 1 : 0;
    a.q_bs = a.k_bs = a.v_bs = (int64_t)S * rs;
    a.q_hs = a.k_hs = a.v_hs = a.o_hs = D;
    a.q_rs = a.k_rs = a.v_rs = rs;
    a.o_bs = (int64_t)S * o_rs; a.o_rs = o_rs;
    a.B = B; a.H = H; a.Sq = S; a.Sk = S; a.D = D;
    a.scale = 1.0f / sqrtf((float)D);
    a.rel_h = static_cast<const float*>(rel_h); a.rel_w = rel_w; a.rel_kh = side; a.rel_kw = side;
    a.kv_batch_div = 1; a.prescale_q = 1;
    return attention_bf16(a, st);
}

struct ClipBufs { bf16_t* cols; float *xa, *xb; bf16_t *y, *qkv, *att, *hh; float* sk; size_t skb; };
ClipBufs carve_clip(const ivlm_clip_cfg* c, int B, Carver& cv) {
    const size_t T = c->tokens, h = c->hidden, in = c->inter, R = B * T, skb = 8 * R * std::max(3 * h, in) * 4;
    return {cv.get<bf16_t>(B * (T - 1) * c->kpad), cv.get<float>(R * h), cv.get<float>(R * h), cv.get<bf16_t>(R * h),
            cv.get<bf16_t>(R * 3 * h), cv.get<bf16_t>(R * h), cv.get<bf16_t>(R * in), cv.get<float>(skb / 4), skb};
}

}
}

extern "C" size_t ivlm_clip_encode_workspace_bytes(const ivlm_clip_cfg* c, int B) {
    return c && B > 0 ? carved_bytes(carve_clip, c, B) : 0;
}

static int clip_encode(const ivlm_clip_cfg* c, const ivlm_clip_head* hd, const ivlm_clip_layer* layers_host, const void* images, int B,
                       void* features_out, void* workspace, size_t workspace_bytes, ivlm_stream_t stream, const int f16) {
    ivlm_enter();
    if (!c || !hd || !layers_host || !images || !features_out || !workspace || B <= 0) return IVLM_ERR_INVALID_ARG;
    Carver cv{static_cast<char*>(workspace), workspace_bytes};
    auto [cols, xa, xb, y, qkv, att, hh, skw, skb] = carve_clip(c, B, cv);
    if (!cv.ok) return IVLM_ERR_WORKSPACE;
    const SkRegion sk{skw, skb, sk_fused_on()};
    hipStream_t st = ivlm_stream(stream);
    const int T = c->tokens, Hd = c->hidden, H = c->heads, D = Hd / H, I = c->inter, R = B * T;
    if (int rc0 = sk_counters_zero(sk, st)) return rc0;
    int rc;
    if ((rc = im2col_nchw(static_cast<const bf16_t*>(images), cols, B, 3, c->image_size, c->image_size, c->patch, c->patch, c->kpad, st))) return rc;
    for (int b = 0; b < B; ++b) {
        float* xrow = xa + (size_t)b * T * Hd;
        if ((rc = gemm(cols + (size_t)b * (T - 1) * c->kpad, c->kpad, hd->patch_w, c->kpad, xrow + Hd, 1, Hd, nullptr,
                       static_cast<const bf16_t*>(hd->pos) + Hd, 0, Hd, 0, T - 1, Hd, c->kpad, ACT_NONE, nullptr, nullptr, sk, st)))
            return rc;
        if ((rc = gather_rows(xrow, 1, Hd, hd->cls_row, 1, Hd, nullptr, nullptr, 0, 0, 1, Hd, st))) return rc;
    }
    if ((rc = layernorm(xa, 1, static_cast<const bf16_t*>(hd->pre_ln_w), static_cast<const bf16_t*>(hd->pre_ln_b), xb, 1, R, Hd, c->eps, st))) return rc;
    float* x = xb;
    const int k16 = f16 ? 4 : 0;
    const int in16 = f16 ? IVLM_GEMM_F16 : 0, io16 = f16 ? IVLM_GEMM_F16 | IVLM_GEMM_OUT_F16 : 0;
    for (int l = 0; l < c->layers_run; ++l) {
        const ivlm_clip_layer& L = layers_host[l];
        if ((rc = layernorm(x, 1, static_cast<const bf16_t*>(L.ln1_w), static_cast<const bf16_t*>(L.ln1_b), y, k16, R, Hd, c->eps, st))) return rc;
        if ((rc = gemm(y, Hd, L.qkv_w, Hd, qkv, 0, 3 * Hd, L.qkv_b, nullptr, 0, 0, 0, R, 3 * Hd, Hd, ACT_NONE, nullptr, nullptr, sk, st, io16))) return rc;
        if ((rc = attend(qkv, nullptr, qkv + Hd, nullptr, qkv + 2 * Hd, nullptr, 3 * Hd, att, Hd, f16, B, H, T, D, nullptr, nullptr, 0, st))) return rc;
        float* x1 = (x == xa) ? xb : xa;
        if ((rc = gemm(att, Hd, L.out_w, Hd, x1, 1, Hd, L.out_b, x, 1, Hd, 0, R, Hd, Hd, ACT_NONE, nullptr, nullptr, sk, st, in16))) return rc;
        if ((rc = layernorm(x1, 1, static_cast<const bf16_t*>(L.ln2_w), static_cast<const bf16_t*>(L.ln2_b), y, k16, R, Hd, c->eps, st))) return rc;
        if ((rc = gemm(y, Hd, L.fc1_w, Hd, hh, 0, I, L.fc1_b, nullptr, 0, 0, 0, R, I, Hd, ACT_QUICK_GELU, nullptr, nullptr, sk, st, io16))) return rc;
        float* x2 = (x1 == xa) ? xb : xa;
        if ((rc = gemm(hh, I, L.fc2_w, I, x2, 1, Hd, L.fc2_b, x1, 1, Hd, 0, R, Hd, I, ACT_NONE, nullptr, nullptr, sk, st, in16))) return rc;
        x = x2;
    }
    const int fw = f16 ? 2 * Hd : Hd;
    for (int b = 0; b < B; ++b)
        if ((rc = gather_rows(static_cast<bf16_t*>(features_out) + (size_t)b * (T - 1) * fw, f16 ? 2 : 0, fw, x + ((size_t)b * T + 1) * Hd, 1, Hd,
                              nullptr, nullptr, 0, 0, T - 1, Hd, st)))
            return rc;
    return IVLM_OK;
}

extern "C" int ivlm_clip_encode(const ivlm_clip_cfg* c, const ivlm_clip_head* hd, const ivlm_clip_layer* layers_host,
                                const void* images, int B, void* features_out, void* workspace, size_t workspace_bytes,
                                ivlm_stream_t stream) {
    return clip_encode(c, hd, layers_host, images, B, features_out, workspace, workspace_bytes, stream, 0);
}

extern "C" int ivlm_clip_encode_f16(const ivlm_clip_cfg* c, const ivlm_clip_head* hd, const ivlm_clip_layer* layers16_host,
                                    const void* images, int B, void* features_split_out, void* workspace, size_t workspace_bytes,
                                    ivlm_stream_t stream) {
    return clip_encode(c, hd, layers16_host, images, B, features_split_out, workspace, workspace_bytes, stream, 1);
}

namespace ivlm {
namespace {

enum SamAttn {
    ATT_BF16,
    ATT_F16Q,
    ATT_SPLIT,
};
constexpr int kSplitA = IVLM_GEMM_A_SPLIT, kSplitAO = IVLM_GEMM_A_SPLIT | IVLM_GEMM_OUT_SPLIT, kF16 = IVLM_GEMM_F16,
              kF16O = IVLM_GEMM_F16 | IVLM_GEMM_OUT_F16;
struct SamMode {
    int n1, qkv;
    SamAttn attn;
    int proj, n2, lin1, lin2;
    bool split_neck;
};
constexpr SamMode kSamDefault{0, 0, ATT_BF16, 0, 0, 0, 0, false};
constexpr SamMode kSamF16q{5, kSplitAO | kF16O, ATT_F16Q, kF16, 4, kF16O, kF16, true};
constexpr SamMode kSamParityFast{2, kSplitAO, ATT_SPLIT, kSplitA, 4, kF16O, kF16, true};
constexpr SamMode kSamParity{2, kSplitAO, ATT_SPLIT, kSplitA, 2, kSplitAO, kSplitA, true};

struct SamDims {
    int g, D, H, hdim, wsz, OC, MD, Kp, nw, g2, R, nwin, WR, npad;
    SamDims(const ivlm_sam_cfg* c, int V)
        : g(c->grid), D(c->embed_dim), H(c->heads), hdim(D / H), wsz(c->window), OC(c->out_chans), MD(c->mlp_dim),
          Kp(3 * c->patch * c->patch), nw((g + wsz - 1) / wsz), g2(g * g), R(V * g2), nwin(V * nw * nw), WR(nwin * wsz * wsz),
          npad((2 * (2 * g - 1) + 7) / 8 * 8) {}
};

struct SamBufs {
    float* x;
    bf16_t *cols, *xn, *q, *kv, *att, *hh;
    float *relh_g, *relw_g, *relh_w, *relw_w;
    bf16_t *G, *brow;
    int32_t *part, *unpart;
    void* n0;
    bf16_t *n1, *c3;
};
SamBufs carve_sam(const SamDims& d, int V, const SamMode& m, Carver& cv) {
    const size_t R = d.R, WR = d.WR, D = d.D, qrows = std::max(R, WR), w = m.attn == ATT_SPLIT ? 2 : 1, nk = m.split_neck ? 2 : 1;
    SamBufs b{};
    b.cols = cv.get<bf16_t>(R * d.Kp), b.x = cv.get<float>(R * D);
    b.xn = cv.get<bf16_t>(R * D * (m.attn == ATT_BF16 ? 1 : 2));
    b.q = cv.get<bf16_t>(qrows * D * (m.attn == ATT_F16Q ? 2 : 3 * w));
    if (m.attn == ATT_F16Q) b.kv = cv.get<bf16_t>(qrows * 2 * D);
    b.att = cv.get<bf16_t>(qrows * D * w), b.hh = cv.get<bf16_t>(R * d.MD * w);
    const size_t rel_g = (size_t)V * d.H * d.g2 * d.g, rel_w = WR * d.H * d.wsz;
    if (m.attn != ATT_F16Q)
        b.relh_g = cv.get<float>(rel_g), b.relw_g = cv.get<float>(rel_g), b.relh_w = cv.get<float>(rel_w), b.relw_w = cv.get<float>(rel_w);
    if (m.attn == ATT_BF16) b.G = cv.get<bf16_t>((size_t)d.H * R * d.npad);
    b.part = cv.get<int32_t>(WR), b.unpart = cv.get<int32_t>(R);
    if (m.attn != ATT_BF16) b.brow = cv.get<bf16_t>(D * (m.attn == ATT_F16Q ? 2 : 6));
    b.n0 = cv.take(R * d.OC * 2 * nk), b.n1 = cv.get<bf16_t>(R * d.OC * nk), b.c3 = cv.get<bf16_t>(R * 9 * d.OC * nk);
    return b;
}
size_t sam_workspace_bytes(const ivlm_sam_cfg* c, int V, const SamMode& m) {
    return c && V > 0 ? carved_bytes(carve_sam, SamDims(c, V), V, m) : 0;
}

template <class W16>
int sam_encode(const ivlm_sam_cfg* c, const ivlm_sam_head* hd, const ivlm_sam_block* blocks_host, W16 w16, const SamMode& m,
               const void* images, int V, float* embeddings_out, void* workspace, size_t workspace_bytes, ivlm_stream_t stream) {
    ivlm_enter();
    if (!c || !hd || !blocks_host || !images || !embeddings_out || !workspace || V <= 0) return IVLM_ERR_INVALID_ARG;
    const SamDims d(c, V);
    Carver cv{static_cast<char*>(workspace), workspace_bytes};
    const SamBufs b = carve_sam(d, V, m, cv);
    if (!cv.ok) return IVLM_ERR_WORKSPACE;
    const int g = d.g, D = d.D, H = d.H, hdim = d.hdim, wsz = d.wsz, OC = d.OC, MD = d.MD, Kp = d.Kp, R = d.R, WR = d.WR;
    if (m.attn != ATT_BF16 && hdim != 80) return IVLM_ERR_UNSUPPORTED;
    if (m.attn == ATT_F16Q && (g != 64 || 2 * wsz > 32)) return IVLM_ERR_UNSUPPORTED;
    for (int l = 0; l < c->depth; ++l) {
        const ivlm_sam_block& Bk = blocks_host[l];
        const ivlm_sam_block_f16 B16 = w16(l);
        if (m.attn == ATT_BF16 && (!Bk.rel_cat || !Bk.rel_h || !Bk.rel_w)) return IVLM_ERR_INVALID_ARG;
        if (m.attn == ATT_F16Q && (!B16.qkv_w16 || !B16.qkv_b16 || !B16.rel_cat16)) return IVLM_ERR_INVALID_ARG;
        if (((m.proj & kF16) && !B16.proj_w16) || ((m.lin1 & kF16) && !B16.lin1_w16) || ((m.lin2 & kF16) && !B16.lin2_w16))
            return IVLM_ERR_INVALID_ARG;
    }
    hipStream_t st = ivlm_stream(stream);
    auto ln = [&](const void* x, int x_f32, const void* w, const void* bias, void* y, int kind, int cols) {
        return layernorm(x, x_f32, static_cast<const bf16_t*>(w), static_cast<const bf16_t*>(bias), y, kind, R, cols, 1e-6f, st);
    };
    auto mm = [&](const void* A, int64_t lda, const void* W, void* C, int64_t ldc, const void* bias, float* res, int N, int K, int act,
                  const int32_t* out_rows, const int32_t* a_rows, int flags) {
        return gemm(A, lda, W, K, C, res != nullptr, ldc, bias, res, res != nullptr, res ? D : 0, 0, R, N, K, act, out_rows, a_rows,
                    SkRegion{}, st, flags);
    };
    auto wide = [](int flags, int split_flag, int n) { return (flags & split_flag) ? 2 * n : n; };
    auto fill_pad_rows = [&](bf16_t* dst, int width, const void* bias, int bias_cols) {
        if (width > bias_cols) {
            IVLM_HIP_TRY(hipMemsetAsync(b.brow, 0, (size_t)width * 2, st));
            IVLM_HIP_TRY(hipMemcpyAsync(b.brow, bias, (size_t)bias_cols * 2, hipMemcpyDeviceToDevice, st));
            bias = b.brow;
        }
        fill_pad_rows_kernel<<<2048, 256, 0, st>>>(dst, width, b.part, WR, static_cast<const bf16_t*>(bias), width);
        return ivlm_launch_status();
    };
    int rc;
    sam_window_maps_kernel<<<256, 256, 0, st>>>(V, g, wsz, d.nw, b.part, b.unpart);
    if ((rc = ivlm_launch_status())) return rc;
    if ((rc = im2col_nchw(static_cast<const bf16_t*>(images), b.cols, V, 3, c->img_size, c->img_size, c->patch, c->patch, Kp, st))) return rc;
    if ((rc = gemm(b.cols, Kp, hd->patch_w, Kp, b.x, 1, D, hd->patch_b, hd->pos_embed, 0, D, d.g2, R, D, Kp, ACT_NONE, nullptr, nullptr, SkRegion{}, st))) return rc;
    float* x = b.x;
    const int64_t lx = m.attn == ATT_BF16 ? D : 2 * D;
    for (int l = 0; l < c->depth; ++l) {
        const ivlm_sam_block& Bk = blocks_host[l];
        const ivlm_sam_block_f16 B16 = w16(l);
        const bool glob = Bk.global_attn;
        const int side = glob ? g : wsz, S = side * side, nb = glob ? V : d.nwin;
        const int32_t* wmap = glob ? nullptr : b.unpart;
        if ((rc = ln(x, 1, Bk.norm1_w, Bk.norm1_b, b.xn, m.n1, D))) return rc;
        const bf16_t *q = b.q, *k, *v, *q_lo = nullptr, *k_lo = nullptr, *v_lo = nullptr;
        int64_t rs;
        if (m.attn == ATT_F16Q) {
            const bf16_t *wq = static_cast<const bf16_t*>(B16.qkv_w16), *bq = static_cast<const bf16_t*>(Bk.qkv_b),
                         *bq16 = static_cast<const bf16_t*>(B16.qkv_b16);
            rs = 2 * D; q_lo = q + D; k = b.kv; v = b.kv + D;
            if ((rc = mm(b.xn, lx, wq, b.q, rs, bq, nullptr, D, D, ACT_NONE, wmap, nullptr, m.qkv))) return rc;
            if ((rc = mm(b.xn, lx, wq + (size_t)D * D, b.kv, rs, bq + D, nullptr, 2 * D, D, ACT_NONE, wmap, nullptr, kF16O))) return rc;
            if (!glob && ((rc = fill_pad_rows(b.q, 2 * D, bq16, D)) || (rc = fill_pad_rows(b.kv, 2 * D, bq16 + D, 2 * D)))) return rc;
        } else {
            rs = wide(m.qkv, IVLM_GEMM_OUT_SPLIT, 3 * D); k = q + D; v = q + 2 * D;
            if (m.attn == ATT_SPLIT) { q_lo = q + 3 * D; k_lo = q + 4 * D; v_lo = q + 5 * D; }
            if ((rc = mm(b.xn, lx, Bk.qkv_w, b.q, rs, Bk.qkv_b, nullptr, 3 * D, D, ACT_NONE, wmap, nullptr, m.qkv))) return rc;
            if (!glob && (rc = fill_pad_rows(b.q, rs, Bk.qkv_b, 3 * D))) return rc;
        }
        const void* rh;
        float* rw = nullptr;
        if (m.attn == ATT_F16Q) {
            rh = B16.rel_cat16;
        } else if (m.attn == ATT_BF16 && hdim == 80 &&
                   ((side == 64 && 2 * (2 * side - 1) <= d.npad) || (2 * side <= 32 && 2 * (2 * side - 1) <= 64))) {
            rh = Bk.rel_cat;
        } else if (m.attn == ATT_BF16 && side >= 32) {
            rh = b.relh_g; rw = b.relw_g;
            const int M = nb * S;
            GemmArgs gg = gemm_args(q, rs, Bk.rel_cat, hdim, b.G, d.npad, nullptr, nullptr, 0, 0, M, d.npad, hdim, ACT_NONE, 0, 0);
            gg.batch = H; gg.strideA = hdim; gg.strideW = 0; gg.strideC = (int64_t)M * d.npad;
            if ((rc = linear_bf16(gg, st))) return rc;
            if ((rc = ivlm_relpos_gather(b.G, (int64_t)M * d.npad, d.npad, nb, H, side, side, b.relh_g, rw, stream))) return rc;
        } else {
            const bool big = glob && m.attn == ATT_SPLIT;
            float* rhf = big ? b.relh_g : b.relh_w;
            rh = rhf; rw = big ? b.relw_g : b.relw_w;
            if ((rc = relpos_bias(q, (int64_t)S * rs, hdim, rs, static_cast<const bf16_t*>(Bk.rel_h), static_cast<const bf16_t*>(Bk.rel_w),
                                  nb, H, side, side, hdim, rhf, rw, st, q_lo)))
                return rc;
        }
        const int64_t la = wide(m.proj, IVLM_GEMM_A_SPLIT, D);
        if ((rc = attend(q, q_lo, k, k_lo, v, v_lo, rs, b.att, la, m.attn == ATT_F16Q, nb, H, S, hdim, rh, rw, side, st))) return rc;
        if ((rc = mm(b.att, la, (m.proj & kF16) ? B16.proj_w16 : Bk.proj_w, x, D, Bk.proj_b, x, D, D, ACT_NONE, nullptr, wmap, m.proj))) return rc;
        if ((rc = ln(x, 1, Bk.norm2_w, Bk.norm2_b, b.xn, m.n2, D))) return rc;
        const int64_t lh = wide(m.lin1, IVLM_GEMM_OUT_SPLIT, MD);
        if ((rc = mm(b.xn, wide(m.lin1, IVLM_GEMM_A_SPLIT, D), (m.lin1 & kF16) ? B16.lin1_w16 : Bk.lin1_w, b.hh, lh, Bk.lin1_b, nullptr, MD,
                     D, ACT_GELU, nullptr, nullptr, m.lin1)))
            return rc;
        if ((rc = mm(b.hh, lh, (m.lin2 & kF16) ? B16.lin2_w16 : Bk.lin2_w, x, D, Bk.lin2_b, x, D, MD, ACT_NONE, nullptr, nullptr, m.lin2))) return rc;
    }
    const int sp = m.split_neck ? 1 : 0, nf = sp ? kSplitA : 0, nw_ = sp ? 2 * OC : OC;
    if ((rc = gather_rows(b.xn, sp ? 2 : 0, sp ? 2 * D : D, x, 1, D, nullptr, nullptr, 0, 0, R, D, st))) return rc;
    if ((rc = gemm(b.xn, sp ? 2 * D : D, hd->neck0_w, D, b.n0, sp, OC, nullptr, nullptr, 0, 0, 0, R, OC, D, ACT_NONE, nullptr, nullptr, SkRegion{}, st, nf))) return rc;
    if ((rc = ln(b.n0, sp, hd->neck1_w, hd->neck1_b, b.n1, sp ? 2 : 0, OC))) return rc;
    for (int half = 0; half <= sp; ++half)
        if ((rc = im2col3x3_nhwc(b.n1 + half * OC, b.c3 + half * 9 * OC, V, g, g, OC, st, nw_, 9 * nw_))) return rc;
    if ((rc = gemm(b.c3, 9 * nw_, hd->neck2_w, 9 * OC, b.n0, sp, OC, nullptr, nullptr, 0, 0, 0, R, OC, 9 * OC, ACT_NONE, nullptr, nullptr, SkRegion{}, st, nf))) return rc;
    return ln(b.n0, sp, hd->neck3_w, hd->neck3_b, embeddings_out, 1, OC);
}

constexpr auto kNoF16 = [](int) { return ivlm_sam_block_f16{}; };

}
}

extern "C" size_t ivlm_sam_encode_workspace_bytes(const ivlm_sam_cfg* c, int V) { return sam_workspace_bytes(c, V, kSamDefault); }
extern "C" size_t ivlm_sam_encode_parity_workspace_bytes(const ivlm_sam_cfg* c, int V) { return sam_workspace_bytes(c, V, kSamParity); }
extern "C" size_t ivlm_sam_encode_f16_workspace_bytes(const ivlm_sam_cfg* c, int V) { return sam_workspace_bytes(c, V, kSamF16q); }

extern "C" int ivlm_sam_encode(const ivlm_sam_cfg* c, const ivlm_sam_head* hd, const ivlm_sam_block* blocks_host, const void* images,
                               int V, float* embeddings_out, void* workspace, size_t workspace_bytes, ivlm_stream_t stream) {
    return sam_encode(c, hd, blocks_host, kNoF16, kSamDefault, images, V, embeddings_out, workspace, workspace_bytes, stream);
}

extern "C" int ivlm_sam_encode_parity(const ivlm_sam_cfg* c, const ivlm_sam_head* hd, const ivlm_sam_block* blocks_host,
                                      const void* images, int V, float* embeddings_out, void* workspace, size_t workspace_bytes,
                                      ivlm_stream_t stream) {
    return sam_encode(c, hd, blocks_host, kNoF16, kSamParity, images, V, embeddings_out, workspace, workspace_bytes, stream);
}

extern "C" int ivlm_sam_encode_parity_f16mlp(const ivlm_sam_cfg* c, const ivlm_sam_head* hd, const ivlm_sam_block* blocks_host,
                                             const ivlm_sam_mlp_f16* mlp16_host, const void* images, int V, float* embeddings_out,
                                             void* workspace, size_t workspace_bytes, ivlm_stream_t stream) {
    if (!mlp16_host) return IVLM_ERR_INVALID_ARG;
    auto w16 = [=](int l) { return ivlm_sam_block_f16{nullptr, nullptr, mlp16_host[l].lin1_w16, mlp16_host[l].lin2_w16, nullptr, nullptr}; };
    return sam_encode(c, hd, blocks_host, w16, kSamParityFast, images, V, embeddings_out, workspace, workspace_bytes, stream);
}

extern "C" int ivlm_sam_encode_f16(const ivlm_sam_cfg* c, const ivlm_sam_head* hd, const ivlm_sam_block* blocks_host,
                                   const ivlm_sam_block_f16* blocks16_host, const void* images, int V, float* embeddings_out,
                                   void* workspace, size_t workspace_bytes, ivlm_stream_t stream) {
    if (!blocks16_host) return IVLM_ERR_INVALID_ARG;
    return sam_encode(c, hd, blocks_host, [=](int l) { return blocks16_host[l]; }, kSamF16q, images, V, embeddings_out, workspace,
                      workspace_bytes, stream);
}

namespace ivlm {
namespace {

struct DecCtx {
    hipStream_t st;
    ivlm_stream_t stream;
    Carver* cv;
    SkRegion sk;
    int rc = 0;
    void* take(size_t b) {
        void* p = cv->take(b);
        if (!p && !rc) rc = IVLM_ERR_WORKSPACE;
        return p;
    }
    bf16_t* split(const float* x, int64_t rows, int cols) {
        bf16_t* o = static_cast<bf16_t*>(take((size_t)rows * 2 * cols * 2));
        if (o && !rc) rc = gather_rows(o, 2, 2 * cols, x, 1, cols, nullptr, nullptr, 0, 0, rows, cols, st);
        return o;
    }
    void* add(const float* a, const float* b, int64_t rows, int cols, int64_t b_rows, bool as_split) {
        void* o = take((size_t)rows * cols * 4);
        if (o && !rc) rc = add_rows(o, as_split ? 2 : 1, a, 1, b, 1, rows, cols, b_rows, st, 0);
        return o;
    }
    float* lin(const bf16_t* xs, const ivlm_lin& L, int M, int act, const float* res, float* dst = nullptr) {
        float* o = dst ? dst : static_cast<float*>(take((size_t)M * L.n * 4));
        if (o && !rc) rc = gemm(xs, 2 * L.k, L.w2, 2 * L.k, o, 1, L.n, L.b, res, 1, L.n, 0, M, L.n, 2 * L.k, act, nullptr, nullptr, sk, st);
        return o;
    }
// ... 107 lines not shown
```

### interactvlm_amd/ops.py

```python
from __future__ import annotations

import functools
import os

import torch

from . import _lib
from ._lib import IvlmError, check

IVLM_F32, IVLM_BF16 = 0, 1


def _stream() -> int:
    return torch.cuda.current_stream().cuda_stream


class KernelTimer:

    def __init__(self):
        self.enabled = False
        self.records = {}
        self._hip = None

    def _rt(self):
# ... 207 lines not shown
    B, V = probs.shape[0], probs.shape[1]
    HW = probs[0, 0].numel()
    batched = 1 if pid.dim() == probs.dim() else 0
    n = int(num_points)
    ws = _workspace(lib.ivlm_lift_points_workspace_bytes(B, V, n), probs.device)
    return _lift_call("lift_points", probs, B, n, want_nviews, lambda out, nviews, stream: lib.ivlm_lift_points(
        probs.data_ptr(), pid.data_ptr(), batched, B, V, HW, n, out, nviews, ws.data_ptr(), ws.numel(), stream))


def lift_points_plan(probs, plan: LiftPlan, want_nviews=False):
    return lift_mesh_plan(probs, plan, mode=2, param=0.0, want_nviews=want_nviews)


def postprocess_masks(low_res, input_size, original_size, img_size: int = 1024, apply_sigmoid: bool = False, sigmoid_gt=None,
                      ignore_label: float = -1.0):
    lib = _lib.load()
    low_res = _req(low_res, None, "low_res")
    lead = tuple(low_res.shape[:-2])
    h, w = low_res.shape[-2:]
    n = 1
    for s in lead:
        n *= s
    oh, ow = int(original_size[0]), int(original_size[1])
    out = torch.empty(lead + (oh, ow), dtype=torch.float32, device=low_res.device)
    if sigmoid_gt is not None:
        gt = _req(sigmoid_gt, torch.float32, "sigmoid_gt")
        assert gt.numel() == out.numel()
        check(lib.ivlm_postprocess_masks_valid(low_res.data_ptr(), _dt(low_res), n, h, w, int(img_size), int(input_size[0]),
                                               int(input_size[1]), oh, ow, gt.data_ptr(), float(ignore_label), out.data_ptr(),
                                               _stream()), "postprocess_masks_valid")
        return out
    check(lib.ivlm_postprocess_masks(low_res.data_ptr(), _dt(low_res), n, h, w, int(img_size), int(input_size[0]),
                                     int(input_size[1]), oh, ow, 1 if apply_sigmoid else 0, out.data_ptr(),
                                     _stream()), "postprocess_masks")
    return out


ACT = {"none": 0, "gelu": 1, "quick_gelu": 2, "relu": 3, "silu": 4, "swiglu": 5, "sigmoid": 6}
BF16 = torch.bfloat16


SPLITK = os.environ.get("IVLM_SPLITK", "1") != "0"
SPLITK_FUSED = os.environ.get("IVLM_SPLITK_FUSED", "0") == "1"
_SPLITK_CNT = {}
_SPLITK_CNT_CAPTURE = None


def _splitk_counters(device):
    cnts = _SPLITK_CNT
    if torch.cuda.is_current_stream_capturing():
        if _SPLITK_CNT_CAPTURE is None:
            raise IvlmError("fused split-K GEMM captured outside graphs.capture (its counters need a capture scope)")
        cnts = _SPLITK_CNT_CAPTURE
    key = (device.index, _stream())
    c = cnts.get(key)
    if c is None:
        c = cnts[key] = torch.zeros(4096, dtype=torch.int32, device=device)
    return c


def _splitk_choice(M, N, K, act, rms):
    if not SPLITK:
        return 1
    return _splitk_rule(M, N, K, ACT[act], 0 if rms is None else 1)


@functools.lru_cache(maxsize=None)
def _splitk_rule(M, N, K, act, has_rms):
    return _lib.load().ivlm_gemm_splitk_choice(M, N, K, act, has_rms)


GEMM_A_F32, GEMM_RES_F32, GEMM_A_SPLIT, GEMM_OUT_SPLIT, GEMM_F16, GEMM_OUT_F16, GEMM_W_PANEL = 1, 2, 4, 8, 16, 32, 64


def panel_weight(w):
    N, K = w.shape
    assert K % 64 == 0
    return w.view(N, K // 64, 64).permute(1, 0, 2).contiguous()
F16 = torch.float16
F32 = torch.float32


def linear(x, weight, bias=None, act="none", residual=None, res_mod=0, out=None, out_f32=False, rms=None, out_rows=None,
           a_rows=None, a_split=False, out_split=False, out_f16=False):
    lib = _lib.load()
    w_panel = weight.dim() == 3
    if w_panel:
        assert weight.shape[2] == 64 and weight.is_contiguous()
        N, K = weight.shape[1], weight.shape[0] * 64
    else:
        N = weight.shape[0]
        K = weight.shape[1]
    f16 = weight.dtype == F16
    assert x.shape[-1] == (2 * K if a_split else K) and x.dtype in (BF16, F32, F16) and weight.dtype in (BF16, F16)
    assert (x.dtype == F16) == f16
    x2 = x.reshape(-1, x.shape[-1])
    if x2.stride(-1) != 1:
        x2 = x2.contiguous()
    M = x2.shape[0] if a_rows is None else a_rows.numel()
    flags = 0
    if x.dtype == F32:
        if M > 16:
            raise IvlmError("linear: fp32 activations only on the M <= 16 weight-streaming paths (use split_rows + a_split)")
        flags |= GEMM_A_F32
    if a_split:
        assert x.dtype in (BF16, F16)
        flags |= GEMM_A_SPLIT
    if f16:
        flags |= GEMM_F16
    if out is not None and out.dtype == F16:
        out_f16 = True
    if out_f16:
        assert not out_f32 or out_split
        flags |= GEMM_OUT_F16
    if w_panel:
        if M <= 16 or out_rows is not None or a_split or out_split:
            raise IvlmError("linear: K-panel weights serve the plain tile GEMMs (M > 16) only")
        flags |= GEMM_W_PANEL
    n_out = N // 2 if act == "swiglu" else N
    if out_split:
        flags |= GEMM_OUT_SPLIT
    n_cols = 2 * n_out if out_split else n_out
    if out is None:
        lead = x.shape[:-1] if a_rows is None else (M,)
        out = torch.empty(tuple(lead) + (n_cols,), dtype=F32 if (out_f32 and not out_split) else (F16 if out_f16 else BF16),
                          device=x.device)
    assert not out_split or out.dtype == (F16 if out_f16 else BF16)
    o2 = out.reshape(-1, n_cols)
    assert o2.stride(-1) == 1 and weight.stride(-1) == 1
    ldw = 64 if w_panel else weight.stride(0)
    r2, ldr = None, 0
    if residual is not None:
        r2 = residual.reshape(-1, N)
        assert r2.dtype in (BF16, F32) and r2.stride(-1) == 1
        ldr = r2.stride(0)
        if r2.dtype == F32:
            flags |= GEMM_RES_F32
    if bias is not None:
        assert bias.dtype == BF16 and bias.is_contiguous()
    call = lambda: check(lib.ivlm_gemm_bf16(
        x2.data_ptr(), x2.stride(0), weight.data_ptr(), ldw, o2.data_ptr(), o2.stride(0), _p(bias),
        _p(r2), ldr, int(res_mod), M, N, K, ACT[act], 1 if out.dtype == F32 else 0, 1, 0, 0, 0, 0,
        _p(rms[0]) if rms else 0, float(rms[1]) if rms else 0.0, flags, _p(out_rows), _p(a_rows), _stream()), "gemm_bf16")
    splits = _splitk_choice(M, N, K, act, rms) if (x.dtype in (BF16, F16) and out_rows is None and a_rows is None) else 1
    if splits > 1 and o2.stride(0) % 4 == 0:
        ws = torch.empty(splits * M * N, dtype=F32, device=x.device)
        if SPLITK_FUSED:
            cnt = _splitk_counters(x.device)
            call = lambda: check(lib.ivlm_gemm_bf16_splitk_fused(
                x2.data_ptr(), x2.stride(0), weight.data_ptr(), ldw, o2.data_ptr(), o2.stride(0), _p(bias),
                _p(r2), ldr, int(res_mod), M, N, K, ACT[act], 1 if out.dtype == F32 else 0, splits, ws.data_ptr(),
                ws.numel() * 4, cnt.data_ptr(), flags, _stream()), "gemm_bf16_splitk_fused")
        else:
            call = lambda: check(lib.ivlm_gemm_bf16_splitk(
                x2.data_ptr(), x2.stride(0), weight.data_ptr(), ldw, o2.data_ptr(), o2.stride(0), _p(bias),
                _p(r2), ldr, int(res_mod), M, N, K, ACT[act], 1 if out.dtype == F32 else 0, splits, ws.data_ptr(),
                ws.numel() * 4, flags, _stream()), "gemm_bf16_splitk")
    if TIMER.enabled:
        if M > 16:
            TIMER.time("gemm_bf16_mfma", 2.0 * M * N * K, call, tag=(M, N, K, act, "split" if a_split else ""))
        else:
            TIMER.time("gemv_bf16", 2.0 * N * K, call, tag=(M, N, K, act))
    else:
        call()
    return out


def _dtc(t):
    return IVLM_F32 if t.dtype == F32 else IVLM_BF16


IVLM_FP8 = 3
U8 = torch.uint8


def layernorm(x, weight, bias, eps=1e-5, gelu=False, out=None, out_f32=False, out_rows=None, fp8_scale=None, out_split=False,
              out_f16=False):
    lib = _lib.load()
    x = _req(x, None, "x")
    cols = x.shape[-1]
    if out is None:
        if out_split:
            out = torch.empty(x.shape[:-1] + (2 * cols,), dtype=F16 if out_f16 else BF16, device=x.device)
        elif out_f16:
            out = torch.empty(x.shape, dtype=F16, device=x.device)
        else:
            out = torch.empty(x.shape, dtype=U8 if fp8_scale is not None else (F32 if out_f32 else BF16), device=x.device)
    y = out
    ydt = IVLM_FP8 if fp8_scale is not None else ((5 if out_f16 else 2) if out_split else (4 if out_f16 else _dtc(y)))
    check(lib.ivlm_layernorm(x.data_ptr(), _dtc(x), weight.data_ptr(), bias.data_ptr(), y.data_ptr(), ydt,
                             x.numel() // cols, cols, float(eps), 1 if gelu else 0, _p(out_rows), _p(fp8_scale), _stream()),
          "layernorm")
    return y


def amax(x, out=None):
    lib = _lib.load()
    x = _req(x, None, "x")
    assert x.numel() % 8 == 0
    if out is None:
        out = torch.zeros(1, dtype=F32, device=x.device)
    check(lib.ivlm_amax(x.data_ptr(), _dtc(x), x.numel(), out.data_ptr(), _stream()), "amax")
    return out


# ... 392 lines not shown
    logits = _req(logits, torch.float32, "logits")
    rows, cols = logits.shape
    out = torch.empty(rows, dtype=torch.int32, device=logits.device)
    if bump is not None:
        assert bump.dtype == torch.int32 and bump.is_cuda and bump.numel() == rows and bump.is_contiguous()
        check(lib.ivlm_argmax_f32_bump(logits.data_ptr(), rows, cols, out.data_ptr(), bump.data_ptr(), _stream()), "argmax_bump")
        return out
    check(lib.ivlm_argmax_f32(logits.data_ptr(), rows, cols, out.data_ptr(), _stream()), "argmax")
    return out


def im2col_nchw(x, ks, stride, kpad=None):
    lib = _lib.load()
    x = _req(x, BF16, "x")
    B, C, H, W = x.shape
    K = C * ks * ks
    kpad = kpad or ((K + 63) // 64) * 64
    gh, gw = (H - ks) // stride + 1, (W - ks) // stride + 1
    out = torch.empty(B * gh * gw, kpad, dtype=BF16, device=x.device)
    check(lib.ivlm_im2col_nchw(x.data_ptr(), out.data_ptr(), B, C, H, W, ks, stride, kpad, _stream()), "im2col_nchw")
    return out


def im2col3x3_nhwc(x):
    lib = _lib.load()
    x = _req(x, BF16, "x")
    B, H, W, C = x.shape
    out = torch.empty(B * H * W, 9 * C, dtype=BF16, device=x.device)
    check(lib.ivlm_im2col3x3_nhwc(x.data_ptr(), out.data_ptr(), B, H, W, C, _stream()), "im2col3x3")
    return out


def im2col3x3_nhwc_split(x_split, B, H, W, C):
    lib = _lib.load()
    x_split = _req(x_split, BF16, "x_split")
    assert x_split.shape == (B * H * W, 2 * C)
    out = torch.empty(B * H * W, 18 * C, dtype=BF16, device=x_split.device)
    for half in range(2):
        check(lib.ivlm_im2col3x3_nhwc_strided(x_split.data_ptr() + half * C * 2, 2 * C, out.data_ptr() + half * 9 * C * 2,
                                              18 * C, B, H, W, C, _stream()), "im2col3x3_strided")
    return out


_KIND = {"bf16": IVLM_BF16, "f32": IVLM_F32, "split": 2, "fp8": 3}


def gather_rows(src, idx=None, add=None, out=None, out_kind=None, scale=None):
    lib = _lib.load()
    assert src.dtype in (BF16, F32) and src.stride(-1) == 1
    cols = src.shape[-1]
    if idx is not None:
        assert idx.dtype == torch.int32 and idx.is_contiguous()
        rows = idx.numel()
    else:
        src = src.reshape(-1, cols)
        rows = src.shape[0]
    if out_kind is None:
        ref = out if out is not None else (add if add is not None else src)
        out_kind = "f32" if ref.dtype == F32 else "bf16"
    if out is None:
        out = (torch.empty(rows, 2 * cols, dtype=BF16, device=src.device) if out_kind == "split"
               else torch.empty(rows, cols, dtype={"f32": F32, "fp8": torch.uint8}.get(out_kind, BF16), device=src.device))
    assert out.stride(-1) == 1 and out.dtype == {"f32": F32, "fp8": torch.uint8}.get(out_kind, BF16)
    assert (out_kind == "fp8") == (scale is not None)
    lda = 0
    if add is not None:
        assert add.dtype in (BF16, F32) and add.stride(-1) == 1
        lda = add.stride(0)
    check(lib.ivlm_gather_rows(out.data_ptr(), _KIND[out_kind], out.stride(0), src.data_ptr(), _dtc(src), src.stride(0),
                               _p(idx), _p(add), _dtc(add) if add is not None else 0, lda, rows, cols, _p(scale), _stream()),
          "gather_rows")
    return out


def fill_rows(dst, idx, row):
    lib = _lib.load()
    assert dst.dtype in (BF16, F16) and row.dtype == dst.dtype and dst.stride(-1) == 1 and row.is_contiguous()
    assert idx.dtype == torch.int32 and idx.is_contiguous() and row.numel() == dst.shape[-1]
    check(lib.ivlm_fill_rows(dst.data_ptr(), dst.stride(0), idx.data_ptr(), idx.numel(), row.data_ptr(), dst.shape[-1],
                             _stream()), "fill_rows")
    return dst


def split_rows(x):
    C = x.shape[-1]
    return gather_rows(x.reshape(-1, C), out_kind="split").view(x.shape[:-1] + (2 * C,))


def add_rows(a, b, out=None, op="add", out_kind=None):
    lib = _lib.load()
    a = _req(a, None, "a")
    b = _req(b, None, "b")
    cols = a.shape[-1]
    if out_kind is None:
        out_kind = "f32" if (out if out is not None else a).dtype == F32 else "bf16"
    if out is None:
        out = (torch.empty(a.shape[:-1] + (2 * cols,), dtype=BF16, device=a.device) if out_kind == "split"
               else torch.empty(a.shape, dtype=F32 if out_kind == "f32" else BF16, device=a.device))
    check(lib.ivlm_add_rows(out.data_ptr(), _KIND[out_kind], a.data_ptr(), _dtc(a), b.data_ptr(), _dtc(b),
                            a.numel() // cols, cols, b.numel() // cols, 1 if op == "mul" else 0, _stream()), "add_rows")
    return out


def uncertainty_mlp(emb, w1, b1, w2, b2, w3, b3):
    emb = _req(emb, F32, "emb")
    assert emb.shape[-1] == 256 and tuple(w1.shape) == (64, 256) and tuple(w2.shape) == (16, 64) and w3.numel() == 16
    ws = [_req(t, BF16, "w") for t in (w1, b1, w2, b2, w3, b3)]
    out = torch.empty(emb.shape[:-1], dtype=F32, device=emb.device)
    check(_lib.load().ivlm_uncertainty_mlp(emb.data_ptr(), out.numel(), *[t.data_ptr() for t in ws], out.data_ptr(), _stream()),
          "uncertainty_mlp")
    return out


def resize_bilinear(src, size, dtype=torch.float32):
    src = _req(src, F32, "src")
    h, w = src.shape[-2:]
    oh, ow = int(size[0]), int(size[1])
    out = torch.empty(src.shape[:-2] + (oh, ow), dtype=dtype, device=src.device)
    n = src.numel() // (h * w)
    check(_lib.load().ivlm_resize_bilinear(src.data_ptr(), n, h, w, out.data_ptr(), _dtc(out), oh, ow, _stream()), "resize_bilinear")
    return out


def dense_pe(gauss, h, w, dtype=torch.float32):
    lib = _lib.load()
    gauss = _req(gauss, torch.float32, "gauss")
    nf = gauss.shape[1]
    pe = torch.empty(h * w, 2 * nf, dtype=dtype, device=gauss.device)
    check(lib.ivlm_dense_pe(gauss.data_ptr(), pe.data_ptr(), _dtc(pe), h, w, nf, _stream()), "dense_pe")
    return pe


def _rope_extents(qkv, width, H, D, pos0, table, caches):
    T, end = qkv.shape[0], int(pos0) + qkv.shape[0]
    assert qkv.dim() == 2 and T > 0 and int(pos0) >= 0 and qkv.shape[-1] >= width, f"qkv {tuple(qkv.shape)}: needs {width} columns"
    if table is not None:
        for t in table:
            assert t.is_cuda and t.dtype == F32 and t.is_contiguous(), "rope table: contiguous fp32 on the device"
            assert t.dim() == 2 and t.shape[1] == D // 2 and t.shape[0] >= end, f"rope table {tuple(t.shape)}: needs [>= {end}, {D // 2}]"
    for c in caches:
        if c is not None:
            assert c.is_contiguous() and c.shape[0] >= end and c.numel() >= end * H * D, f"cache {tuple(c.shape)}: needs {end} rows of {H * D}"


def rope_kv(qkv, H, D, pos0, theta, kcache=None, vcache=None, table=None):
    lib = _lib.load()
    assert qkv.dtype in (BF16, F16) and qkv.stride(-1) == 1 and (kcache is None or (kcache.dtype == qkv.dtype == vcache.dtype))
    _rope_extents(qkv, 3 * H * D, H, D, pos0, table, (kcache, vcache))
    T = qkv.shape[0]
    check((lib.ivlm_rope_kv_f16 if qkv.dtype == F16 else lib.ivlm_rope_kv)(qkv.data_ptr(), qkv.stride(0), T, H, D, int(pos0), float(theta), _p(kcache), _p(vcache),
                                                                           _p(table[0]) if table else 0, _p(table[1]) if table else 0, _stream()), "rope_kv")
    return qkv


def rope_kv_split(qkv, H, D, pos0, caches, table):
    lib = _lib.load()
    assert qkv.dtype == BF16 and qkv.stride(-1) == 1 and qkv.shape[-1] == 6 * H * D
    T = qkv.shape[0]
    kc = caches if caches is not None else (None,) * 4
    _rope_extents(qkv, 6 * H * D, H, D, pos0, table, kc)
    check(lib.ivlm_rope_kv_split(qkv.data_ptr(), qkv.stride(0), T, H, D, int(pos0), _p(kc[0]), _p(kc[1]), _p(kc[2]), _p(kc[3]),
                                 table[0].data_ptr(), table[1].data_ptr(), _stream()), "rope_kv_split")
    return qkv


def rope_table(T, D, theta, device):
# ... 364 lines not shown
```

### interactvlm_amd/sam.py

```python
from __future__ import annotations

import collections
import functools
import math

import torch

from . import graphs, ops
from .weights import SAM_PREFIX, SamEncCfg

BF16 = torch.bfloat16
F32 = torch.float32


def _dev(t, device):
    return t.to(device=device, dtype=BF16).contiguous()


class _Lin:
    def __init__(self, w, prefix, device, bias=True):
        self.w = _dev(w[prefix + ".weight"].reshape(w[prefix + ".weight"].shape[0], -1), device)
        self.b = _dev(w[prefix + ".bias"], device) if bias and (prefix + ".bias") in w else None

    def __call__(self, x, act="none", residual=None, res_mod=0, out=None, out_f32=False, out_rows=None, a_rows=None,
# ... 56 lines not shown
        return self[n + "_h"] if a.dtype == torch.float16 else self[n].w


class SamImageEncoder:

    def __init__(self, w, cfg: SamEncCfg, device, prefix=SAM_PREFIX + ".image_encoder"):
        self.cfg, self.device = cfg, device
        self._graphs = graphs.Cache()
        p = prefix
        D = cfg.embed_dim
        self.patch = _Lin(w, p + ".patch_embed.proj", device)
        self.pos_embed = _dev(w[p + ".pos_embed"].reshape(-1, D), device)
        self.blocks = []
        for i in range(cfg.depth):
            bp = f"{p}.blocks.{i}"
            self.blocks.append(_Block(
                glob=i in cfg.global_attn_indexes,
                norm1=_LN(w, bp + ".norm1", device, 1e-6), norm2=_LN(w, bp + ".norm2", device, 1e-6),
                qkv=_Lin(w, bp + ".attn.qkv", device), proj=_Lin(w, bp + ".attn.proj", device),
                rel_h=_dev(w[bp + ".attn.rel_pos_h"], device), rel_w=_dev(w[bp + ".attn.rel_pos_w"], device),
                lin1=_Lin(w, bp + ".mlp.lin1", device), lin2=_Lin(w, bp + ".mlp.lin2", device)))
        self.neck0 = _Lin(w, p + ".neck.0", device, bias=False)
        self.neck1 = _LN(w, p + ".neck.1", device, 1e-6)
        w2 = w[p + ".neck.2.weight"]
        self.neck2_w = _dev(w2.permute(0, 2, 3, 1).reshape(w2.shape[0], -1), device)
        self.neck3 = _LN(w, p + ".neck.3", device, 1e-6)
        self._maps = {}
        self._xw = {}

    def _window_maps(self, V):
        if V not in self._maps:
            g, ws = self.cfg.grid, self.cfg.window
            nw = (g + ws - 1) // ws
            gp = nw * ws
            v = torch.arange(V).view(V, 1, 1, 1, 1)
            wy = torch.arange(nw).view(1, nw, 1, 1, 1)
            wx = torch.arange(nw).view(1, 1, nw, 1, 1)
            iy = torch.arange(ws).view(1, 1, 1, ws, 1)
            ix = torch.arange(ws).view(1, 1, 1, 1, ws)
            y, x = wy * ws + iy, wx * ws + ix
            src = (v * g + y) * g + x
            part = torch.where((y < g) & (x < g), src, torch.full_like(src, -1)).reshape(-1)
            yy = torch.arange(g).view(1, g, 1)
            xx = torch.arange(g).view(1, 1, g)
            vv = torch.arange(V).view(V, 1, 1)
            unpart = (((vv * nw + yy // ws) * nw + xx // ws) * ws + yy % ws) * ws + xx % ws
            pad = (part < 0).nonzero().flatten()
            self._maps[V] = (part.to(torch.int32).to(self.device), unpart.reshape(-1).to(torch.int32).to(self.device),
                             nw, gp, pad.to(torch.int32).to(self.device))
        return self._maps[V]

    def _qkv_buffers(self, kind, V, nwin, device):
        if (kind, V) not in self._xw:
            rows, D = nwin * self.cfg.window ** 2, self.cfg.embed_dim
            shapes = {"bf16": [(3, BF16)], "f16": [(3, torch.float16)], "f16q": [(2, torch.float16)] * 2, "split": [(6, BF16)]}[kind]
            self._xw[(kind, V)] = [torch.empty(rows, n * D, dtype=dt, device=device) for n, dt in shapes]
        return self._xw[(kind, V)]

    fp8 = False
    _calibrating = False

    def enable_fp8(self, calib_images):
        dev = self.device
        for blk in self.blocks:
            for n in ("qkv", "proj", "lin1", "lin2"):
                q, sc = ops.quantize_fp8(blk[n].w)
                blk[n + "_q"], blk[n + "_s"] = q, sc
            blk["amax"] = {k: torch.zeros(1, dtype=F32, device=dev) for k in ("n1", "att", "n2", "h")}
        self._calibrating = True
        try:
            self._forward(calib_images.to(dev))
        finally:
            self._calibrating = False
        for blk in self.blocks:
            blk["s"] = {k: (v / 448.0).clamp_(min=1e-12) for k, v in blk["amax"].items()}
        self.fp8 = True
        self._graphs.clear()

    use_graph = graphs.ON

    def __call__(self, images):
        if not graphs.enabled(self.use_graph, images):
            return self._forward(images)
        key = (tuple(images.shape), self.fp8, self.precision, self.q_lo_level)
        return self._graphs.run(key, self._forward, [images], BF16)

    precision = "default"
    q_lo_level = 1

    def _attention(self, blk, xn, side, nwin, win=None, fp8=False):
        c = self.cfg
        D = c.embed_dim
        H, hd = c.num_heads, D // c.num_heads
        S = side * side
        m = _MODES[self.precision]
        b = blk["qkv"].b
        if fp8:
            gemms = [(functools.partial(ops.linear_fp8, xn, blk["qkv_q"], blk["s"]["n1"], blk["qkv_s"], b), b)]
        elif m.attn == "f16q":
            w = blk["qkv_h"]
            gemms = [(functools.partial(ops.linear, xn, w[:D], b[:D], **m.qkv), blk["q_b_split_h"]),
                     (functools.partial(ops.linear, xn[:, :D], w[D:], b[D:], out_f16=True), blk["kv_b_h"])]
        else:
            fill = blk["qkv_b_h"] if m.attn == "f16" else (blk["qkv_b_split"] if m.attn == "split" else b)
            gemms = [(functools.partial(ops.linear, xn, blk.weight("qkv", xn), b, **m.qkv), fill)]
        if win is None:
            outs = [gemm() for gemm, _ in gemms]
        else:
            unpart, pad, outs = win
            for (gemm, _), o in zip(gemms, outs):
                gemm(out=o, out_rows=unpart)
            for (_, fill), o in zip(gemms, outs):
                ops.fill_rows(o, pad, fill)
        if m.attn == "split":
            q6 = outs[0].view(nwin, S, 2, 3, H, hd)
            (q, k, v), (q_lo, k_lo, v_lo) = ([q6[:, :, j, i].permute(0, 2, 1, 3) for i in range(3)] for j in range(2))
            rel = ops.relpos_bias_split(q, q_lo, blk["rel_h"], blk["rel_w"], side, side)
            return ops.attention_split(q, q_lo, k, k_lo, v, v_lo, hd ** -0.5, rel=rel)
        if m.attn == "f16q":
            q4, kv4 = (t.view(nwin, S, 2, H, hd) for t in outs)
            q, q_lo, k, v = (t.permute(0, 2, 1, 3) for t in (q4[:, :, 0], q4[:, :, 1], kv4[:, :, 0], kv4[:, :, 1]))
            lv = self.q_lo_level
        else:
            qkv5 = outs[0].view(nwin, S, 3, H, hd)
            q, k, v = (qkv5[:, :, i].permute(0, 2, 1, 3) for i in range(3))
            q_lo, lv = None, 1
        tab = blk["rel_cat_h"] if q.dtype == torch.float16 else blk["rel_cat"]
        if hd == 80 and (2 * side <= 32 or (side == 64 and lv < 2)):
            o = ops.attention(q, k, v, hd ** -0.5, rel_tab=(tab, side), q_lo=q_lo, q_lo_level=lv)
        else:
            rel = ops.relpos_bias(q, blk["rel_h"], blk["rel_w"], side, side, cat=tab, q_lo=q_lo)
            o = ops.attention(q, k, v, hd ** -0.5, rel=rel, q_lo=q_lo if lv == 2 else None, q_lo_level=lv)
        return o.permute(0, 2, 1, 3).reshape(nwin * S, H * hd)

    def _block(self, blk, x, V, nwin, win, fp8=False):
        c = self.cfg
        glob = blk["glob"]
        side, nw_, win = (c.grid, V, None) if glob else (c.window, nwin, win)
        a_rows = None if glob else win[0]
        if fp8:
            sc = blk["s"]
            a = self._attention(blk, blk["norm1"](x, fp8_scale=sc["n1"]), side, nw_, win, fp8=True)
            aq = ops.gather_rows(a, out_kind="fp8", scale=sc["att"])
            x = ops.linear_fp8(aq, blk["proj_q"], sc["att"], blk["proj_s"], blk["proj"].b, residual=x, out=x, a_rows=a_rows)
            hq = blk["norm2"](x, fp8_scale=sc["n2"])
            h8 = ops.linear_fp8(hq, blk["lin1_q"], sc["n2"], blk["lin1_s"], blk["lin1"].b, act="gelu", out_kind="fp8",
                                scale_out=sc["h"])
            return ops.linear_fp8(h8, blk["lin2_q"], sc["h"], blk["lin2_s"], blk["lin2"].b, residual=x, out=x)
        m = _MODES[self.precision]
        cal = blk.get("amax") if self._calibrating and self.precision == "default" else None
        xn = blk["norm1"](x, **m.n1)
        if cal:
            ops.amax(xn, cal["n1"])
        a = self._attention(blk, xn, side, nw_, win)
        if cal:
            ops.amax(a, cal["att"])
        x = ops.linear(a, blk.weight("proj", a), blk["proj"].b, residual=x, out_f32=True, out=None if glob else x, a_rows=a_rows,
                       **m.proj)
        xn2 = blk["norm2"](x, **m.n2)
        h = ops.linear(xn2, blk.weight("lin1", xn2), blk["lin1"].b, act="gelu", **m.lin1)
        if cal:
            ops.amax(xn2, cal["n2"])
            ops.amax(h, cal["h"])
        return ops.linear(h, blk.weight("lin2", h), blk["lin2"].b, residual=x, out_f32=True, **m.lin2)

    def _forward(self, images):
        c = self.cfg
        V = images.shape[0]
        g = c.grid
        m = _MODES[self.precision]
        cols = ops.im2col_nchw(images.to(BF16).contiguous(), c.patch, c.patch)
        x = self.patch(cols, residual=self.pos_embed, res_mod=g * g, out_f32=True)
        part, unpart, nw, gp, pad = self._window_maps(V)
        nwin = V * nw * nw
        win = (unpart, pad, self._qkv_buffers(m.attn, V, nwin, x.device))
        fp8 = self.fp8 and self.precision == "default"
        for blk in self.blocks:
            x = self._block(blk, x, V, nwin, win, fp8)
        if m.split_neck:
            y = self.neck0(ops.gather_rows(x, out_kind="split"), out_f32=True, a_split=True)
            y = self.neck1(y, out_split=True)
            y = ops.linear(ops.im2col3x3_nhwc_split(y, V, g, g, c.out_chans), self.neck2_w, out_f32=True, a_split=True)
        else:
            y = self.neck1(self.neck0(ops.gather_rows(x, out_kind="bf16")))
            y = ops.linear(ops.im2col3x3_nhwc(y.view(V, g, g, c.out_chans)), self.neck2_w)
        return self.neck3(y, out_f32=True).view(V, g * g, c.out_chans)


class SamMaskDecoder:

    def __init__(self, w, device, grid=64, prefix=SAM_PREFIX, decoder="mask_decoder"):
        self.device, self.grid = device, grid
        self._graphs = graphs.Cache()
        pe, md = prefix + ".prompt_encoder", prefix + "." + decoder
        self.C = C = w[md + ".iou_token.weight"].shape[1]
        f32 = lambda t: t.to(device=device, dtype=BF16).to(F32).contiguous()
        self.no_mask = f32(w[pe + ".no_mask_embed.weight"].reshape(1, C))
        gauss = w[pe + ".pe_layer.positional_encoding_gaussian_matrix"].to(device=device, dtype=torch.float32).contiguous()
        self.key_pe = ops.dense_pe(gauss, grid, grid)
        self.out_tokens = f32(torch.cat([w[md + ".iou_token.weight"], w[md + ".mask_tokens.weight"]], 0))
        self.n_mask = w[md + ".mask_tokens.weight"].shape[0]
        tp = md + ".transformer"

        def attn(p):
            return dict(q=_LinF32(w, p + ".q_proj", device), k=_LinF32(w, p + ".k_proj", device),
# ... 218 lines not shown
```

Measured before the change: 10.58.

## Write QKV projection output in head-major layout for SAM attention

Adds a head-major output mode to the GEMM epilogue. Each column block of head_dim is written to its own plane with stride head_stride, so Q/K/V land as [planes, rows, hd], and matching fill_rows_heads and fill_pad_rows paths handle the window padding. The SAM attention path in both Python and the C++ stages uses this layout by default, and attention and relpos now read with a per-head stride. The aim is contiguous per-head rows for the attention kernels, in place of row-interleaved QKV with a 3*D stride. The cost is an extra integer divide per epilogue column, and split-N GEMM tiling is disabled for this mode.

New measurement: 10.56. About the same (-0.1%).

```diff
diff --git a/include/ivlm_hip.h b/include/ivlm_hip.h
--- a/include/ivlm_hip.h
+++ b/include/ivlm_hip.h
@@ -85,6 +85,10 @@
 int ivlm_gemm_bf16_panel(const void *A, int64_t lda, int64_t a_kstep, const void *W, int64_t ldw, int64_t w_kstep, void *C,
                          int64_t ldc, int64_t c_panel, const void *bias, const void *residual, int64_t ldr, int M, int N, int K,
                          int act, int out_f32, int flags, const int32_t *out_rows, const int32_t *a_rows, ivlm_stream_t stream);
+
+int ivlm_gemm_bf16_heads(const void *A, int64_t lda, const void *W, int64_t ldw, void *C, int head_dim, int64_t head_stride,
+                         int64_t c_lo, const void *bias, int M, int N, int K, int act, int flags, const int32_t *out_rows,
+                         const int32_t *a_rows, ivlm_stream_t stream);
 
 int ivlm_gemm_fp8(const void *A, int64_t lda, const void *W, int64_t ldw, void *C, int64_t ldc, const void *bias,
                   const void *residual, int64_t ldr, int M, int N, int K, int act, int out_kind, const float *scale_a,
@@ -366,6 +370,8 @@
                   int64_t b_rows, int op, ivlm_stream_t stream);
 int ivlm_fill_rows(void *dst, int64_t ldd, const int32_t *idx, int64_t n_idx, const void *row, int cols,
                    ivlm_stream_t stream);
+int ivlm_fill_rows_heads(void *dst, int head_dim, int64_t head_stride, const int32_t *idx, int64_t n_idx, const void *row, int cols,
+                         ivlm_stream_t stream);
 int ivlm_dense_pe(const void *gauss, void *pe, int pe_dtype, int h, int w, int F, ivlm_stream_t stream);
 int ivlm_rope_kv(void *qkv, int64_t ld, int T, int H, int D, int pos0, float theta, void *kcache, void *vcache,
                  const float *cos_tab, const float *sin_tab, ivlm_stream_t stream);
diff --git a/interactvlm_amd/csrc/elementwise.hip b/interactvlm_amd/csrc/elementwise.hip
--- a/interactvlm_amd/csrc/elementwise.hip
+++ b/interactvlm_amd/csrc/elementwise.hip
@@ -144,6 +144,17 @@
         const int c8 = (int)(i % c8n);
         const int64_t r = idx[i / c8n];
         *reinterpret_cast<uint4*>(dst + r * ldd + c8 * 8) = *reinterpret_cast<const uint4*>(row + c8 * 8);
+    }
+}
+
+__global__ __launch_bounds__(kT) void fill_rows_heads_kernel(bf16_t* __restrict__ dst, int hd, int64_t hs, const int32_t* __restrict__ idx,
+                                                             int64_t n_idx, const bf16_t* __restrict__ row, int cols) {
+    const int c8n = cols >> 3;
+    const int64_t total = n_idx * c8n;
+    for (int64_t i = (int64_t)blockIdx.x * kT + threadIdx.x; i < total; i += (int64_t)gridDim.x * kT) {
+        const int c = (int)(i % c8n) * 8, h = c / hd;
+        const int64_t r = idx[i / c8n];
+        *reinterpret_cast<uint4*>(dst + h * hs + r * hd + (c - h * hd)) = *reinterpret_cast<const uint4*>(row + c);
     }
 }
 
@@ -459,6 +470,12 @@
     fill_rows_kernel<<<grid_for(n_idx * (cols >> 3)), kT, 0, st>>>(dst, ldd, idx, n_idx, row, cols);
     return ivlm_launch_status();
 }
+int fill_rows_heads(bf16_t* dst, int hd, int64_t hs, const int32_t* idx, int64_t n_idx, const bf16_t* row, int cols, hipStream_t st) {
+    if (n_idx == 0) return IVLM_OK;
+    if (!dst || !idx || !row || n_idx < 0 || hd <= 0 || (hd & 7) || cols % hd || (hs & 7)) return IVLM_ERR_INVALID_ARG;
+    fill_rows_heads_kernel<<<grid_for(n_idx * (cols >> 3)), kT, 0, st>>>(dst, hd, hs, idx, n_idx, row, cols);
+    return ivlm_launch_status();
+}
 int dense_pe(const float* gauss, void* pe, int pe_f32, int h, int w, int F, hipStream_t st) {
     if (!gauss || !pe) return IVLM_ERR_INVALID_ARG;
     dense_pe_kernel<<<grid_for((int64_t)h * w * 2 * F), kT, 0, st>>>(gauss, pe, pe_f32, h, w, F);
@@ -546,6 +563,11 @@
     ivlm_enter();
     return ivlm::fill_rows(BF(dst), ldd, idx, n_idx, CBF(row), cols, ivlm_stream(s));
 }
+int ivlm_fill_rows_heads(void* dst, int head_dim, int64_t head_stride, const int32_t* idx, int64_t n_idx, const void* row, int cols,
+                         ivlm_stream_t s) {
+    ivlm_enter();
+    return ivlm::fill_rows_heads(BF(dst), head_dim, head_stride, idx, n_idx, CBF(row), cols, ivlm_stream(s));
+}
 int ivlm_dense_pe(const void* gauss, void* pe, int pe_dtype, int h, int w, int F, ivlm_stream_t s) {
     ivlm_enter();
     return ivlm::dense_pe(static_cast<const float*>(gauss), pe, pe_dtype == IVLM_F32, h, w, F, ivlm_stream(s));
diff --git a/interactvlm_amd/csrc/gemm.hip b/interactvlm_amd/csrc/gemm.hip
--- a/interactvlm_amd/csrc/gemm.hip
+++ b/interactvlm_amd/csrc/gemm.hip
@@ -306,6 +306,7 @@
 
 static int nsplit_cols(const GemmArgs& g, const GemmSwitches& sw) {
     if (!sw.nsplit || g.tile != 0 || sw.tile_override != 0 || g.batch != 1 || g.act == ACT_SWIGLU || g.M < 4096 || (g.N & 255)) return 0;
+    if (g.c_hd) return 0;
     if (auto_tile(g, sw) == 320) return 0;
     const long tm = (g.M + 255) / 256, tn = g.N / 256;
     const long tiles = tm * tn;
@@ -353,6 +354,13 @@
             return IVLM_ERR_INVALID_ARG;
         if (g.c_panel && (g.out_f32 || (g.N & 63) || g.c_panel < (int64_t)64 * g.M || g.out_rows)) return IVLM_ERR_UNSUPPORTED;
     }
+    if (g.c_hd) {
+        if (g.c_hd < 0 || (g.c_hd & 7) || g.N % g.c_hd || (g.c_hs & 7) || g.c_hs < (int64_t)g.c_hd * (g.out_rows ? 1 : g.M)) return IVLM_ERR_INVALID_ARG;
+        if (g.batch != 1 || g.c_panel || g.fp8 || g.out_fp8 || g.act == ACT_SWIGLU || g.sk.count || (g.out_f32 && !g.out_split) ||
+            (reinterpret_cast<uintptr_t>(g.C) & 15))
+            return IVLM_ERR_UNSUPPORTED;
+        if (g.out_split && ((g.c_lo & 7) || g.c_lo < (int64_t)(g.N / g.c_hd) * g.c_hs)) return IVLM_ERR_INVALID_ARG;
+    }
     if (g.fp8 && (!g.scale_a || !g.scale_w || (g.out_fp8 && (!g.scale_out || g.out_f32 || (g.ldc & 3))))) return IVLM_ERR_INVALID_ARG;
     if (g.out_fp8 && !g.fp8) return IVLM_ERR_UNSUPPORTED;
     if (g.out_fp8 && (g.N & 3)) return IVLM_ERR_UNSUPPORTED;
@@ -379,7 +387,7 @@
 }
 
 int gemm_bf16_splitk(const GemmArgs& g, int splits, float* workspace, size_t ws_bytes, hipStream_t st, int32_t* counters) {
-    if (splits < 2 || g.batch != 1 || g.act == ACT_SWIGLU || g.rms_w || g.out_rows || g.a_rows || !workspace) return IVLM_ERR_INVALID_ARG;
+    if (splits < 2 || g.batch != 1 || g.act == ACT_SWIGLU || g.rms_w || g.out_rows || g.a_rows || g.c_hd || !workspace) return IVLM_ERR_INVALID_ARG;
     if (g.K % (splits * 8) != 0 || (g.N & 3) || (g.ldc & 3)) return IVLM_ERR_UNSUPPORTED;
     if (ws_bytes < (size_t)splits * g.M * g.N * sizeof(float)) return IVLM_ERR_WORKSPACE;
     GemmArgs p = g;
@@ -526,7 +534,7 @@
     ivlm_enter();
     ivlm::GemmArgs g = ivlm::gemm_args(A, lda, W, ldw, C, ldc, bias, residual, ldr, res_mod, M, N, K, act, out_f32, flags, out_rows, a_rows);
     if (g.w_kstep && ((K & 63) || batch > 1)) return IVLM_ERR_UNSUPPORTED;
-    if ((g.a_split || g.out_split || g.f16 || g.out_f16 || g.w_kstep) && M <= 16) return IVLM_ERR_UNSUPPORTED;
+    if ((g.a_split || g.out_split || g.f16 || g.out_f16 || g.w_kstep) && M <= 16 && !out_rows && !a_rows) return IVLM_ERR_UNSUPPORTED;
     g.rms_w = static_cast<const bf16_t*>(rms_w);
     g.rms_eps = rms_eps;
     g.batch = batch < 1 ? 1 : batch;
@@ -543,6 +551,17 @@
     ivlm::GemmArgs g = ivlm::gemm_args(A, a_kstep ? 64 : lda, W, w_kstep ? 64 : ldw, C, ldc, bias, residual, ldr, 0, M, N, K, act, out_f32,
                                        flags & IVLM_GEMM_RES_F32, out_rows, a_rows);
     g.a_kstep = a_kstep; g.w_kstep = w_kstep; g.c_panel = c_panel;
+    return ivlm::gemm_bf16(g, ivlm_stream(stream));
+}
+
+extern "C" int ivlm_gemm_bf16_heads(const void* A, int64_t lda, const void* W, int64_t ldw, void* C, int head_dim, int64_t head_stride,
+                                    int64_t c_lo, const void* bias, int M, int N, int K, int act, int flags, const int32_t* out_rows,
+                                    const int32_t* a_rows, ivlm_stream_t stream) {
+    ivlm_enter();
+    if (head_dim <= 0 || (flags & (IVLM_GEMM_A_F32 | IVLM_GEMM_W_PANEL))) return IVLM_ERR_UNSUPPORTED;
+    ivlm::GemmArgs g = ivlm::gemm_args(A, lda, W, ldw, C, 0, bias, nullptr, 0, 0, M, N, K, act, 0, flags, out_rows, a_rows);
+    g.c_hd = head_dim; g.c_hs = head_stride;
+    if (g.out_split) g.c_lo = c_lo;
     return ivlm::gemm_bf16(g, ivlm_stream(stream));
 }
 
diff --git a/interactvlm_amd/csrc/gemm_common.h b/interactvlm_amd/csrc/gemm_common.h
--- a/interactvlm_amd/csrc/gemm_common.h
+++ b/interactvlm_amd/csrc/gemm_common.h
@@ -104,6 +104,15 @@
     return g.res_f32 ? reinterpret_cast<const float*>(R)[idx] : bf16_to_f32(R[idx]);
 }
 
+struct GemmCol { int64_t rs, col; };
+__device__ __forceinline__ GemmCol gemm_c_col(const GemmArgs& g, int n) {
+    if (g.c_hd) {
+        const int h = n / g.c_hd;
+        return {(int64_t)g.c_hd, (int64_t)h * g.c_hs + (n - h * g.c_hd)};
+    }
+    return {g.ldc, (int64_t)n};
+}
+
 template <bool OUT_F32>
 __device__ __forceinline__ void splitk_finish4(const GemmArgs& g, const float* __restrict__ part, int splits, int m, int n) {
     const int64_t slice = (int64_t)g.M * g.N;
@@ -184,6 +193,8 @@
 
 template <bool OUT_F32>
 __host__ __device__ __forceinline__ bool gemm_whole_lines_ok(const GemmArgs& g, int act) {
+    if (g.c_hd)
+        return act != ACT_SWIGLU && g.batch == 1 && (reinterpret_cast<uintptr_t>(g.C) & 15) == 0 && (OUT_F32 ? g.out_split != 0 : !g.residual);
     return act != ACT_SWIGLU && !g.out_fp8 && g.batch == 1 && (reinterpret_cast<uintptr_t>(g.C) & 15) == 0 &&
            (OUT_F32 ? ((g.N & 3) == 0 && (g.ldc & 3) == 0 && (!g.residual || (g.ldr & 3) == 0) && (!g.out_split || (g.c_lo & 3) == 0))
                     : ((g.N & 7) == 0 && !g.residual && (g.c_panel ? (g.c_panel & 7) == 0 : (g.ldc & 7) == 0)));
@@ -200,6 +211,7 @@
     constexpr int RPI = 64 / CH;
     constexpr int ROWS = PASS_MI * 16;
     const int cc = lane % CH, n = nw + cc * (16 / ES);
+    const GemmCol cn = gemm_c_col(g, n);
 #pragma unroll
     for (int p = 0; p < MI / PASS_MI; ++p) {
 #pragma unroll
@@ -248,14 +260,14 @@
                     uint32_t h0, l0, h1, l1;
                     split_16x2(q.x, q.y, h0, l0, g.out_f16);
                     split_16x2(q.z, q.w, h1, l1, g.out_f16);
-                    bf16_t* cb = static_cast<bf16_t*>(g.C) + (int64_t)m * g.ldc + n;
+                    bf16_t* cb = static_cast<bf16_t*>(g.C) + (int64_t)m * cn.rs + cn.col;
                     *reinterpret_cast<uint2*>(cb) = make_uint2(h0, h1);
                     *reinterpret_cast<uint2*>(cb + g.c_lo) = make_uint2(l0, l1);
                 } else {
                     *reinterpret_cast<float4*>(static_cast<float*>(g.C) + (int64_t)m * g.ldc + n) = q;
                 }
             } else {
-                const int64_t o = g.c_panel ? (int64_t)(n >> 6) * g.c_panel + (int64_t)m * 64 + (n & 63) : (int64_t)m * g.ldc + n;
+                const int64_t o = g.c_panel ? (int64_t)(n >> 6) * g.c_panel + (int64_t)m * 64 + (n & 63) : (int64_t)m * cn.rs + cn.col;
                 *reinterpret_cast<uint4*>(static_cast<bf16_t*>(g.C) + o) = *reinterpret_cast<const uint4*>(src);
             }
         }
@@ -288,6 +300,7 @@
     constexpr int ES = OUT_F32 ? 4 : 2;
     constexpr int RB = 64 * ES, CH = RB / 16, RPI = 64 / CH;
     const int cc = lane % CH, n = n_base + cc * (16 / ES);
+    const GemmCol cn = gemm_c_col(g, n);
     for (int it = 0; it < nrows / RPI; ++it) {
         const int rr = row0 + it * RPI + lane / CH;
         const int sw = CH == 8 ? ((rr >> 1) & 7) : (rr & 15);
@@ -317,14 +330,14 @@
                 uint32_t h0, l0, h1, l1;
                 split_16x2(q.x, q.y, h0, l0, g.out_f16);
                 split_16x2(q.z, q.w, h1, l1, g.out_f16);
-                bf16_t* cb = static_cast<bf16_t*>(g.C) + (int64_t)m * g.ldc + n;
+                bf16_t* cb = static_cast<bf16_t*>(g.C) + (int64_t)m * cn.rs + cn.col;
                 *reinterpret_cast<uint2*>(cb) = make_uint2(h0, h1);
                 *reinterpret_cast<uint2*>(cb + g.c_lo) = make_uint2(l0, l1);
             } else {
                 *reinterpret_cast<float4*>(static_cast<float*>(g.C) + (int64_t)m * g.ldc + n) = q;
             }
         } else {
-            *reinterpret_cast<uint4*>(static_cast<bf16_t*>(g.C) + (int64_t)m * g.ldc + n) = *reinterpret_cast<const uint4*>(src);
+            *reinterpret_cast<uint4*>(static_cast<bf16_t*>(g.C) + (int64_t)m * cn.rs + cn.col) = *reinterpret_cast<const uint4*>(src);
         }
     }
 }
@@ -393,7 +406,11 @@
                 v[3] += bf16_to_f32((bf16_t)(r2.y >> 16));
             }
         }
-        const int64_t o = g.c_panel ? (int64_t)(n >> 6) * g.c_panel + (int64_t)m * 64 + (n & 63) : (int64_t)m * g.ldc + n;
+        int64_t o = g.c_panel ? (int64_t)(n >> 6) * g.c_panel + (int64_t)m * 64 + (n & 63) : (int64_t)m * g.ldc + n;
+        if (g.c_hd) {
+            const GemmCol cn = gemm_c_col(g, n);
+            o = (int64_t)m * cn.rs + cn.col;
+        }
         if (g.out_fp8) {
             const float inv = 1.0f / (*g.scale_out);
             float c4[4];
diff --git a/interactvlm_amd/csrc/kernels.h b/interactvlm_amd/csrc/kernels.h
--- a/interactvlm_amd/csrc/kernels.h
+++ b/interactvlm_amd/csrc/kernels.h
@@ -30,6 +30,8 @@
     const int32_t* a_rows = nullptr;
     int64_t a_kstep = 0, w_kstep = 0;
     int64_t c_panel = 0;
+    int c_hd = 0;
+    int64_t c_hs = 0;
     int fp8 = 0, out_fp8 = 0;
     const float *scale_a = nullptr, *scale_w = nullptr, *scale_out = nullptr;
     int a_f32 = 0;
@@ -99,6 +101,7 @@
 int add_rows(void* out, int out_kind, const void* a, int a_kind, const void* b, int b_kind, int64_t rows, int cols,
              int64_t b_rows, hipStream_t st, int op = 0);
 int fill_rows(bf16_t* dst, int64_t ldd, const int32_t* idx, int64_t n_idx, const bf16_t* row, int cols, hipStream_t st);
+int fill_rows_heads(bf16_t* dst, int hd, int64_t hs, const int32_t* idx, int64_t n_idx, const bf16_t* row, int cols, hipStream_t st);
 int dense_pe(const float* gauss, void* pe, int pe_f32, int h, int w, int F, hipStream_t st);
 int rope_kv(bf16_t* qkv, int64_t ld, int T, int H, int D, int pos0, float theta, bf16_t* kcache, bf16_t* vcache,
             hipStream_t st, const float* cos_tab = nullptr, const float* sin_tab = nullptr, int f16 = 0);
diff --git a/interactvlm_amd/csrc/stages.hip b/interactvlm_amd/csrc/stages.hip
--- a/interactvlm_amd/csrc/stages.hip
+++ b/interactvlm_amd/csrc/stages.hip
@@ -317,14 +317,15 @@
 }
 
 __global__ void fill_pad_rows_kernel(bf16_t* __restrict__ dst, int64_t ldd, const int32_t* __restrict__ part, int64_t rows,
-                                     const bf16_t* __restrict__ row, int cols) {
+                                     const bf16_t* __restrict__ row, int cols, int hd, int64_t hs) {
     const int c8n = cols >> 3;
     const int64_t total = rows * c8n;
     for (int64_t i = (int64_t)blockIdx.x * blockDim.x + threadIdx.x; i < total; i += (int64_t)gridDim.x * blockDim.x) {
         const int64_t r = i / c8n;
         if (part[r] >= 0) continue;
-        const int c8 = (int)(i % c8n);
-        *reinterpret_cast<uint4*>(dst + r * ldd + c8 * 8) = *reinterpret_cast<const uint4*>(row + c8 * 8);
+        const int c = (int)(i % c8n) * 8, h = hd ? c / hd : 0;
+        const int64_t o = hd ? h * hs + r * hd + (c - h * hd) : r * ldd + c;
+        *reinterpret_cast<uint4*>(dst + o) = *reinterpret_cast<const uint4*>(row + c);
     }
 }
 
@@ -340,7 +341,7 @@
 }
 
 int attend(const bf16_t* q, const bf16_t* q_lo, const bf16_t* k, const bf16_t* k_lo, const bf16_t* v, const bf16_t* v_lo, int64_t rs,
-           bf16_t* o, int64_t o_rs, int f16, int B, int H, int S, int D, const void* rel_h, const float* rel_w, int side,
+           int64_t hs, bf16_t* o, int64_t o_rs, int f16, int B, int H, int S, int D, const void* rel_h, const float* rel_w, int side,
            hipStream_t st) {
     AttnArgs a{};
     a.f16 = f16;
@@ -348,7 +349,7 @@
     a.q_lo = q_lo; a.k_lo = k_lo; a.v_lo = v_lo; a.o_lo = k_lo ? o + H * D : nullptr;
     a.q_lo_level = (f16 && q_lo) ? 1 : 0;
     a.q_bs = a.k_bs = a.v_bs = (int64_t)S * rs;
-    a.q_hs = a.k_hs = a.v_hs = a.o_hs = D;
+    a.q_hs = a.k_hs = a.v_hs = hs; a.o_hs = D;
     a.q_rs = a.k_rs = a.v_rs = rs;
     a.o_bs = (int64_t)S * o_rs; a.o_rs = o_rs;
     a.B = B; a.H = H; a.Sq = S; a.Sk = S; a.D = D;
@@ -400,7 +401,7 @@
         const ivlm_clip_layer& L = layers_host[l];
         if ((rc = layernorm(x, 1, static_cast<const bf16_t*>(L.ln1_w), static_cast<const bf16_t*>(L.ln1_b), y, k16, R, Hd, c->eps, st))) return rc;
         if ((rc = gemm(y, Hd, L.qkv_w, Hd, qkv, 0, 3 * Hd, L.qkv_b, nullptr, 0, 0, 0, R, 3 * Hd, Hd, ACT_NONE, nullptr, nullptr, sk, st, io16))) return rc;
-        if ((rc = attend(qkv, nullptr, qkv + Hd, nullptr, qkv + 2 * Hd, nullptr, 3 * Hd, att, Hd, f16, B, H, T, D, nullptr, nullptr, 0, st))) return rc;
+        if ((rc = attend(qkv, nullptr, qkv + Hd, nullptr, qkv + 2 * Hd, nullptr, 3 * Hd, D, att, Hd, f16, B, H, T, D, nullptr, nullptr, 0, st))) return rc;
         float* x1 = (x == xa) ? xb : xa;
         if ((rc = gemm(att, Hd, L.out_w, Hd, x1, 1, Hd, L.out_b, x, 1, Hd, 0, R, Hd, Hd, ACT_NONE, nullptr, nullptr, sk, st, in16))) return rc;
         if ((rc = layernorm(x1, 1, static_cast<const bf16_t*>(L.ln2_w), static_cast<const bf16_t*>(L.ln2_b), y, k16, R, Hd, c->eps, st))) return rc;
@@ -517,14 +518,21 @@
         return gemm(A, lda, W, K, C, res != nullptr, ldc, bias, res, res != nullptr, res ? D : 0, 0, R, N, K, act, out_rows, a_rows,
                     SkRegion{}, st, flags);
     };
+    auto mmh = [&](const void* A, int64_t lda, const void* W, void* C, int64_t hs, int64_t c_lo, const void* bias, int N, int K,
+                   const int32_t* out_rows, int flags) {
+        GemmArgs gh = gemm_args(A, lda, W, K, C, 0, bias, nullptr, 0, 0, R, N, K, ACT_NONE, 0, flags, out_rows, nullptr);
+        gh.c_hd = hdim; gh.c_hs = hs;
+        if (gh.out_split) gh.c_lo = c_lo;
+        return gemm_bf16(gh, st);
+    };
     auto wide = [](int flags, int split_flag, int n) { return (flags & split_flag) ? 2 * n : n; };
-    auto fill_pad_rows = [&](bf16_t* dst, int width, const void* bias, int bias_cols) {
+    auto fill_pad_rows = [&](bf16_t* dst, int width, const void* bias, int bias_cols, int64_t hs = 0) {
         if (width > bias_cols) {
             IVLM_HIP_TRY(hipMemsetAsync(b.brow, 0, (size_t)width * 2, st));
             IVLM_HIP_TRY(hipMemcpyAsync(b.brow, bias, (size_t)bias_cols * 2, hipMemcpyDeviceToDevice, st));
             bias = b.brow;
         }
-        fill_pad_rows_kernel<<<2048, 256, 0, st>>>(dst, width, b.part, WR, static_cast<const bf16_t*>(bias), width);
+        fill_pad_rows_kernel<<<2048, 256, 0, st>>>(dst, width, b.part, WR, static_cast<const bf16_t*>(bias), width, hs ? hdim : 0, hs);
         return ivlm_launch_status();
     };
     int rc;
@@ -542,14 +550,19 @@
         const int32_t* wmap = glob ? nullptr : b.unpart;
         if ((rc = ln(x, 1, Bk.norm1_w, Bk.norm1_b, b.xn, m.n1, D))) return rc;
         const bf16_t *q = b.q, *k, *v, *q_lo = nullptr, *k_lo = nullptr, *v_lo = nullptr;
-        int64_t rs;
+        int64_t rs, hs = hdim;
+        const int64_t hmaj = (int64_t)nb * S * hdim, Hm = (int64_t)H * hmaj;
         if (m.attn == ATT_F16Q) {
             const bf16_t *wq = static_cast<const bf16_t*>(B16.qkv_w16), *bq = static_cast<const bf16_t*>(Bk.qkv_b),
                          *bq16 = static_cast<const bf16_t*>(B16.qkv_b16);
-            rs = 2 * D; q_lo = q + D; k = b.kv; v = b.kv + D;
-            if ((rc = mm(b.xn, lx, wq, b.q, rs, bq, nullptr, D, D, ACT_NONE, wmap, nullptr, m.qkv))) return rc;
-            if ((rc = mm(b.xn, lx, wq + (size_t)D * D, b.kv, rs, bq + D, nullptr, 2 * D, D, ACT_NONE, wmap, nullptr, kF16O))) return rc;
-            if (!glob && ((rc = fill_pad_rows(b.q, 2 * D, bq16, D)) || (rc = fill_pad_rows(b.kv, 2 * D, bq16 + D, 2 * D)))) return rc;
+            rs = hdim; hs = hmaj; q_lo = q + Hm; k = b.kv; v = b.kv + Hm;
+            if ((rc = mmh(b.xn, lx, wq, b.q, hs, Hm, bq, D, D, wmap, m.qkv))) return rc;
+            if ((rc = mmh(b.xn, lx, wq + (size_t)D * D, b.kv, hs, 0, bq + D, 2 * D, D, wmap, kF16O))) return rc;
+            if (!glob && ((rc = fill_pad_rows(b.q, 2 * D, bq16, D, hs)) || (rc = fill_pad_rows(b.kv, 2 * D, bq16 + D, 2 * D, hs)))) return rc;
+        } else if (m.attn == ATT_BF16) {
+            rs = hdim; hs = hmaj; k = q + Hm; v = q + 2 * Hm;
+            if ((rc = mmh(b.xn, lx, Bk.qkv_w, b.q, hs, 0, Bk.qkv_b, 3 * D, D, wmap, m.qkv))) return rc;
+            if (!glob && (rc = fill_pad_rows(b.q, 3 * D, Bk.qkv_b, 3 * D, hs))) return rc;
         } else {
             rs = wide(m.qkv, IVLM_GEMM_OUT_SPLIT, 3 * D); k = q + D; v = q + 2 * D;
             if (m.attn == ATT_SPLIT) { q_lo = q + 3 * D; k_lo = q + 4 * D; v_lo = q + 5 * D; }
@@ -567,19 +580,19 @@
             rh = b.relh_g; rw = b.relw_g;
             const int M = nb * S;
             GemmArgs gg = gemm_args(q, rs, Bk.rel_cat, hdim, b.G, d.npad, nullptr, nullptr, 0, 0, M, d.npad, hdim, ACT_NONE, 0, 0);
-            gg.batch = H; gg.strideA = hdim; gg.strideW = 0; gg.strideC = (int64_t)M * d.npad;
+            gg.batch = H; gg.strideA = hs; gg.strideW = 0; gg.strideC = (int64_t)M * d.npad;
             if ((rc = linear_bf16(gg, st))) return rc;
             if ((rc = ivlm_relpos_gather(b.G, (int64_t)M * d.npad, d.npad, nb, H, side, side, b.relh_g, rw, stream))) return rc;
         } else {
             const bool big = glob && m.attn == ATT_SPLIT;
             float* rhf = big ? b.relh_g : b.relh_w;
             rh = rhf; rw = big ? b.relw_g : b.relw_w;
-            if ((rc = relpos_bias(q, (int64_t)S * rs, hdim, rs, static_cast<const bf16_t*>(Bk.rel_h), static_cast<const bf16_t*>(Bk.rel_w),
+            if ((rc = relpos_bias(q, (int64_t)S * rs, hs, rs, static_cast<const bf16_t*>(Bk.rel_h), static_cast<const bf16_t*>(Bk.rel_w),
                                   nb, H, side, side, hdim, rhf, rw, st, q_lo)))
                 return rc;
         }
         const int64_t la = wide(m.proj, IVLM_GEMM_A_SPLIT, D);
-        if ((rc = attend(q, q_lo, k, k_lo, v, v_lo, rs, b.att, la, m.attn == ATT_F16Q, nb, H, S, hdim, rh, rw, side, st))) return rc;
+        if ((rc = attend(q, q_lo, k, k_lo, v, v_lo, rs, hs, b.att, la, m.attn == ATT_F16Q, nb, H, S, hdim, rh, rw, side, st))) return rc;
         if ((rc = mm(b.att, la, (m.proj & kF16) ? B16.proj_w16 : Bk.proj_w, x, D, Bk.proj_b, x, D, D, ACT_NONE, nullptr, wmap, m.proj))) return rc;
         if ((rc = ln(x, 1, Bk.norm2_w, Bk.norm2_b, b.xn, m.n2, D))) return rc;
         const int64_t lh = wide(m.lin1, IVLM_GEMM_OUT_SPLIT, MD);
diff --git a/interactvlm_amd/ops.py b/interactvlm_amd/ops.py
--- a/interactvlm_amd/ops.py
+++ b/interactvlm_amd/ops.py
@@ -313,7 +313,7 @@
 
 
 def linear(x, weight, bias=None, act="none", residual=None, res_mod=0, out=None, out_f32=False, rms=None, out_rows=None,
-           a_rows=None, a_split=False, out_split=False, out_f16=False):
+           a_rows=None, a_split=False, out_split=False, out_f16=False, head_major=0):
     lib = _lib.load()
     w_panel = weight.dim() == 3
     if w_panel:
@@ -352,6 +352,23 @@
     if out_split:
         flags |= GEMM_OUT_SPLIT
     n_cols = 2 * n_out if out_split else n_out
+    if head_major:
+        hd = int(head_major)
+        assert n_out % hd == 0 and residual is None and rms is None and not out_f32 and not w_panel and x.dtype in (BF16, F16)
+        odt = F16 if out_f16 else BF16
+        if out is None:
+            out = torch.empty(n_cols // hd, M, hd, dtype=odt, device=x.device)
+        assert out.dtype == odt and out.shape[0] == n_cols // hd and out.shape[2] == hd and out.stride(2) == 1 and out.stride(1) == hd
+        assert out_rows is not None or out.shape[1] >= M
+        hs = out.stride(0)
+        call = lambda: check(lib.ivlm_gemm_bf16_heads(
+            x2.data_ptr(), x2.stride(0), weight.data_ptr(), weight.stride(0), out.data_ptr(), hd, hs, (n_out // hd) * hs, _p(bias), M, N, K,
+            ACT[act], flags, _p(out_rows), _p(a_rows), _stream()), "gemm_bf16_heads")
+        if TIMER.enabled:
+            TIMER.time("gemm_bf16_mfma", 2.0 * M * N * K, call, tag=(M, N, K, act, "split" if a_split else ""))
+        else:
+            call()
+        return out
     if out is None:
         lead = x.shape[:-1] if a_rows is None else (M,)
         out = torch.empty(tuple(lead) + (n_cols,), dtype=F32 if (out_f32 and not out_split) else (F16 if out_f16 else BF16),
@@ -910,6 +927,16 @@
     return dst
 
 
+def fill_rows_heads(dst, idx, row):
+    lib = _lib.load()
+    P, _, hd = dst.shape
+    assert dst.dtype in (BF16, F16) and row.dtype == dst.dtype and dst.stride(2) == 1 and dst.stride(1) == hd and row.is_contiguous()
+    assert idx.dtype == torch.int32 and idx.is_contiguous() and row.numel() == P * hd
+    check(lib.ivlm_fill_rows_heads(dst.data_ptr(), hd, dst.stride(0), idx.data_ptr(), idx.numel(), row.data_ptr(), P * hd, _stream()),
+          "fill_rows_heads")
+    return dst
+
+
 def split_rows(x):
     C = x.shape[-1]
     return gather_rows(x.reshape(-1, C), out_kind="split").view(x.shape[:-1] + (2 * C,))
diff --git a/interactvlm_amd/sam.py b/interactvlm_amd/sam.py
--- a/interactvlm_amd/sam.py
+++ b/interactvlm_amd/sam.py
@@ -162,11 +162,12 @@
     def __call__(self, images):
         if not graphs.enabled(self.use_graph, images):
             return self._forward(images)
-        key = (tuple(images.shape), self.fp8, self.precision, self.q_lo_level)
+        key = (tuple(images.shape), self.fp8, self.precision, self.q_lo_level, self.qkv_head_major)
         return self._graphs.run(key, self._forward, [images], BF16)
 
     precision = "default"
     q_lo_level = 1
+    qkv_head_major = True
 
     def _attention(self, blk, xn, side, nwin, win=None, fp8=False):
         c = self.cfg
@@ -175,32 +176,43 @@
         S = side * side
         m = _MODES[self.precision]
         b = blk["qkv"].b
+        hm = self.qkv_head_major and not fp8 and m.attn != "split"
+        kw = dict(head_major=hd) if hm else {}
         if fp8:
             gemms = [(functools.partial(ops.linear_fp8, xn, blk["qkv_q"], blk["s"]["n1"], blk["qkv_s"], b), b)]
         elif m.attn == "f16q":
             w = blk["qkv_h"]
-            gemms = [(functools.partial(ops.linear, xn, w[:D], b[:D], **m.qkv), blk["q_b_split_h"]),
-                     (functools.partial(ops.linear, xn[:, :D], w[D:], b[D:], out_f16=True), blk["kv_b_h"])]
+            gemms = [(functools.partial(ops.linear, xn, w[:D], b[:D], **m.qkv, **kw), blk["q_b_split_h"]),
+                     (functools.partial(ops.linear, xn[:, :D], w[D:], b[D:], out_f16=True, **kw), blk["kv_b_h"])]
         else:
             fill = blk["qkv_b_h"] if m.attn == "f16" else (blk["qkv_b_split"] if m.attn == "split" else b)
-            gemms = [(functools.partial(ops.linear, xn, blk.weight("qkv", xn), b, **m.qkv), fill)]
+            gemms = [(functools.partial(ops.linear, xn, blk.weight("qkv", xn), b, **m.qkv, **kw), fill)]
         if win is None:
             outs = [gemm() for gemm, _ in gemms]
         else:
             unpart, pad, outs = win
+            if hm:
+                outs = [o.view(-1, o.shape[0], hd) for o in outs]
             for (gemm, _), o in zip(gemms, outs):
                 gemm(out=o, out_rows=unpart)
             for (_, fill), o in zip(gemms, outs):
-                ops.fill_rows(o, pad, fill)
+                (ops.fill_rows_heads if hm else ops.fill_rows)(o, pad, fill)
+        heads = lambda t, planes: t.view(planes, H, nwin, S, hd).permute(0, 2, 1, 3, 4)
         if m.attn == "split":
             q6 = outs[0].view(nwin, S, 2, 3, H, hd)
             (q, k, v), (q_lo, k_lo, v_lo) = ([q6[:, :, j, i].permute(0, 2, 1, 3) for i in range(3)] for j in range(2))
             rel = ops.relpos_bias_split(q, q_lo, blk["rel_h"], blk["rel_w"], side, side)
             return ops.attention_split(q, q_lo, k, k_lo, v, v_lo, hd ** -0.5, rel=rel)
         if m.attn == "f16q":
-            q4, kv4 = (t.view(nwin, S, 2, H, hd) for t in outs)
-            q, q_lo, k, v = (t.permute(0, 2, 1, 3) for t in (q4[:, :, 0], q4[:, :, 1], kv4[:, :, 0], kv4[:, :, 1]))
+            if hm:
+                (q, q_lo), (k, v) = (heads(t, 2) for t in outs)
+            else:
+                q4, kv4 = (t.view(nwin, S, 2, H, hd) for t in outs)
+                q, q_lo, k, v = (t.permute(0, 2, 1, 3) for t in (q4[:, :, 0], q4[:, :, 1], kv4[:, :, 0], kv4[:, :, 1]))
             lv = self.q_lo_level
+        elif hm:
+            q, k, v = heads(outs[0], 3)
+            q_lo, lv = None, 1
         else:
             qkv5 = outs[0].view(nwin, S, 3, H, hd)
             q, k, v = (qkv5[:, :, i].permute(0, 2, 1, 3) for i in range(3))
```
